# facebookresearch/sylph-few-shot-detection

Hardware: AMD Instinct MI355X
Metric: query images/sec, R50-FPN 5-way 5-shot 800x1333 (whole job) (higher is better)
Workload: dtype bf16

## Files before the change

### include/sylph_hip.h

```cpp
#ifndef SYLPH_HIP_H
#define SYLPH_HIP_H

#include <stdint.h>

#ifdef __cplusplus
extern "C" {
#endif

typedef struct sylph_ctx sylph_ctx;

enum { SYLPH_F32 = 0, SYLPH_BF16 = 1, SYLPH_F32S = 2 };

typedef struct sylph_config {
  int resnet_depth;
  int stride_in_1x1;
  int num_cls_convs;
  int num_box_convs;
  int nlevels;
  int strides[8];
  float pixel_mean[3];
  float pixel_std[3];
  int size_divisibility;
  int use_scale;
  int cond_use_bias;
  float pre_nms_thresh;
  int pre_nms_topk;
  float nms_thresh;
  int post_nms_topk;
  int thresh_with_ctr;
  int quality_mode;
  int cg_tower_layers;
  int cg_has_bias;
  int cg_bias_l2_norm;
  int cg_post_norm;
  int cg_conv_l2_norm;
  int cg_use_weight_scale;
  float prior_prob;
  int cand_cap;
  int cg_type;
  int tok_num_conv;
  int tok_num_fc;
  int enc_layers;
  int head_num_fc;
  int head_fc_dim;
  int cg_meta_bias;
  int cg_has_weight;
  int cg_has_scale;
  int num_share_convs;
  int tower_norm;
  int cg_tower_gn_mask;
  int cg_tower_relu_mask;
  int tower_deformable;
  int num_groups;
  int width_per_group;
  int cg_code_ksize;
} sylph_config;

void sylph_config_default(sylph_config* cfg);

int sylph_ctx_create(int device_id, int dtype, sylph_ctx** out);
void sylph_ctx_destroy(sylph_ctx* ctx);
const char* sylph_last_error(void);
int sylph_set_stream(sylph_ctx* ctx, void* hip_stream);
int sylph_set_config(sylph_ctx* ctx, const sylph_config* cfg);

int sylph_load_weight(sylph_ctx* ctx, const char* name, const float* data_host, const int64_t* shape, int ndim);
int sylph_finalize_weights(sylph_ctx* ctx);

int sylph_preprocess(sylph_ctx* ctx, int B, const float* const* images_dev, const int* heights, const int* widths,
                     int* padded_h, int* padded_w);

int sylph_preprocess_u8(sylph_ctx* ctx, int B, const unsigned char* const* images_dev, const int* heights, const int* widths,
                        const int* new_heights, const int* new_widths, int rgb_input, int* padded_h, int* padded_w);
int sylph_export_input(sylph_ctx* ctx, float* out_nchw_dev);

int sylph_backbone_fpn(sylph_ctx* ctx);

int sylph_import_pyramid(sylph_ctx* ctx, int B, int padded_h, int padded_w, const int* heights, const int* widths,
                         const float* const* levels_nchw_dev);
int sylph_export_pyramid(sylph_ctx* ctx, int level, float* out_nchw_dev);

int sylph_fcos_head(sylph_ctx* ctx, const float* cls_conv_dev, const float* cls_bias_dev, int N);
int sylph_fcos_head_episodes(sylph_ctx* ctx, int E, const float* cls_conv_dev, const float* cls_bias_dev, const int* n_classes,
                             const int* image_episode);
int sylph_fcos_head_codesets(sylph_ctx* ctx, int G, const float* cls_conv_dev, const float* cls_bias_dev, const int* n_classes);
int sylph_fcos_head_pretrained(sylph_ctx* ctx, int* num_classes);
int sylph_export_head(sylph_ctx* ctx, int level, float* logits_nchw_dev, float* reg_nchw_dev, float* ctr_nchw_dev,
                      float* iou_nchw_dev);

int sylph_import_head(sylph_ctx* ctx, int N, int level, const float* logits_nchw_dev, const float* reg_nchw_dev,
                      const float* ctr_nchw_dev, const float* iou_nchw_dev);

int sylph_decode_nms(sylph_ctx* ctx, const int* out_heights, const int* out_widths, int max_out, float* boxes_dev,
                     float* scores_dev, int* classes_dev, int* levels_dev, float* locations_dev, int* cand_dev,
                     int* counts_dev, int* status_dev);
int sylph_decode_nms_codesets(sylph_ctx* ctx, int G, const int* out_heights, const int* out_widths, int max_out, float* boxes_dev,
                              float* scores_dev, int* classes_dev, int* levels_dev, float* locations_dev, int* cand_dev,
                              int* counts_dev, int* status_dev);

int sylph_codegen(sylph_ctx* ctx, const float* boxes_dev, float* code_out_dev);
int sylph_codegen_classes(sylph_ctx* ctx, const float* boxes_dev, int shots, float* codes_out_dev);
int sylph_codegen_rois(sylph_ctx* ctx, int R, const float* boxes_dev, const int* roi_image, int n_seg, const int* seg_len,
                       float* codes_out_dev);
int sylph_roi_table_uploads(sylph_ctx* ctx, int64_t* n_out);
int sylph_codegen_weight_norm(sylph_ctx* ctx, float* weight_norm_out_dev);

int sylph_roi_align(sylph_ctx* ctx, const float* boxes_dev, float* out_nchw_dev);
int sylph_roi_align_rois(sylph_ctx* ctx, int R, const float* boxes_dev, const int* roi_image, float* out_nchw_dev);

int sylph_normalize_codes(sylph_ctx* ctx, float* codes_dev, int n, const float* weight_norm_dev);

int sylph_reduce_codes(sylph_ctx* ctx, const float* rows_dev, int n, int row_ld, float* out_dev, int num_classes,
                       int divide_by_acc);

int sylph_allgather_codes(sylph_ctx* ctx, void* comm, const float* local_dev, int n_local, int capacity, float* out_dev);
int sylph_comm_unique_id(char* id_out_128);
int sylph_comm_init_rank(sylph_ctx* ctx, const char* id_128, int nranks, int rank, void** comm_out);
int sylph_comm_destroy(void* comm);

int sylph_conv2d(sylph_ctx* ctx, const float* x_nchw_dev, int B, int C, int H, int W, const float* w_host, int Cout,
                 int KH, int KW, int stride, int pad, const float* scale_host, const float* shift_host, int relu,
                 const float* residual_nchw_dev, float* y_nchw_dev);
int sylph_group_norm(sylph_ctx* ctx, const float* x_nchw_dev, int B, int H, int W, const float* gamma_host,
                     const float* beta_host, int relu, float* y_nchw_dev);

int sylph_stem_maxpool(sylph_ctx* ctx, const float* x_nchw_dev, int B, int H, int W, const float* w_host,
                       const float* scale_host, const float* shift_host, float* stem_out_nchw_dev, float* pool_out_nchw_dev);

int sylph_set_debug_taps(sylph_ctx* ctx, int on);
int sylph_export_stage(sylph_ctx* ctx, int stage, float* out_nchw_dev);
int sylph_export_tower(sylph_ctx* ctx, int tower, int layer, int level, float* y_nchw_dev, float* coef_dev);

#define SYLPH_SUP_ROI 0
#define SYLPH_SUP_GN_Y 1
#define SYLPH_SUP_GN_COEF 2
#define SYLPH_SUP_LAYER_OUT 3
#define SYLPH_SUP_CONV_OUT 4
#define SYLPH_SUP_CONTEXT 5
#define SYLPH_SUP_MSCAM 6
#define SYLPH_SUP_TOKENS 7
#define SYLPH_SUP_CLS_TOKENS 8
int sylph_support_tap_numel(sylph_ctx* ctx, int stage, int index, int64_t* numel);
int sylph_export_support(sylph_ctx* ctx, int stage, int index, float* out_dev);

int sylph_bottleneck(sylph_ctx* ctx, const float* x_nchw_dev, int B, int Cin, int H, int W, int stride, int mid, int cout,
                     const float* const* w_host, const float* const* scale_host, const float* const* shift_host,
                     float* y_nchw_dev);
int sylph_bottleneck_even(sylph_ctx* ctx, const float* x_nchw_dev, int B, int Cin, int H, int W, int mid, int cout,
                          const float* const* w_host, const float* const* scale_host, const float* const* shift_host,
                          float* y_nchw_dev);

int sylph_fpn_lateral(sylph_ctx* ctx, const float* x_nchw_dev, int B, int C, int H, int W, const float* w_host, const float* bias_host,
                      const float* top_nchw_dev, float* y_nchw_dev);

int sylph_group_conv(sylph_ctx* ctx, const float* x_nchw_dev, int B, int C, int H, int W, int groups, int stride, const float* w_host,
                     const float* scale_host, const float* shift_host, int relu, float* y_nchw_dev);
int sylph_conv3x3_c64(sylph_ctx* ctx, const float* x_nchw_dev, int B, int H, int W, const float* w_host, const float* scale_host,
                      const float* shift_host, int relu, const float* residual_nchw_dev, float* y_nchw_dev);
int sylph_basic_block(sylph_ctx* ctx, const float* x_nchw_dev, int B, int Cin, int H, int W, int stride, int cout,
                      const float* const* w_host, const float* const* scale_host, const float* const* shift_host, float* y_nchw_dev);
int sylph_bottleneck_grouped(sylph_ctx* ctx, const float* x_nchw_dev, int B, int Cin, int H, int W, int stride, int mid, int cout,
                             int groups, const float* const* w_host, const float* const* scale_host, const float* const* shift_host,
                             float* y_nchw_dev);

int64_t sylph_device_bytes(sylph_ctx* ctx);

int sylph_profile_enable(sylph_ctx* ctx, int on);
int sylph_bench_conv(sylph_ctx* ctx, int B, int H, int W, int Cin, int Cout, int K, int stride, int pad, int has_res,
                     int relu, int with_gn, int iters, float* ms_out, double* flops_out);
int sylph_profile_read(sylph_ctx* ctx, double* conv_ms, double* conv_flops, int64_t* conv_launches);
int sylph_profile_read_kernels(sylph_ctx* ctx, int max_kernels, char* names_out, double* ms_out, double* flops_out,
                               int64_t* launches_out, int* n_out);
int sylph_conv_routes_read(sylph_ctx* ctx, int max_routes, char* names_out, int* n_out);

#ifdef __cplusplus
}
#endif
#endif
```

### sylph-few-shot-detection_amd/csrc/api_backbone.hip

```cpp
#include "api_internal.h"

namespace sylph_host {

std::shared_ptr<PilCoeffs> pil_bilinear_coeffs(int in_size, int out_size) {
  auto pc = std::make_shared<PilCoeffs>();
  const double scale = (double)in_size / (double)out_size;
  double filterscale = scale;
  if (filterscale < 1.0) filterscale = 1.0;
  const double support = 1.0 * filterscale;
  const int ksize = (int)ceil(support) * 2 + 1;
  pc->ksize = ksize;
  pc->bounds.assign((size_t)out_size * 2, 0);
  pc->kk.assign((size_t)out_size * ksize, 0);
  std::vector<double> k((size_t)ksize);
  for (int xx = 0; xx < out_size; ++xx) {
    const double center = (xx + 0.5) * scale;
    const double ss = 1.0 / filterscale;
    int xmin = (int)(center - support + 0.5);
    if (xmin < 0) xmin = 0;
    int xmax = (int)(center + support + 0.5);
    if (xmax > in_size) xmax = in_size;
    xmax -= xmin;
    double ww = 0.0;
    for (int x = 0; x < xmax; ++x) {
      double a = (x + xmin - center + 0.5) * ss;
      if (a < 0.0) a = -a;
      const double w = a < 1.0 ? 1.0 - a : 0.0;
      k[x] = w;
      ww += w;
    }
    for (int x = 0; x < xmax; ++x) {
      if (ww != 0.0) k[x] /= ww;
      pc->kk[(size_t)xx * ksize + x] = k[x] < 0 ? (int)(-0.5 + k[x] * (double)(1 << 22)) : (int)(0.5 + k[x] * (double)(1 << 22));
    }
    pc->bounds[2 * xx] = xmin;
    pc->bounds[2 * xx + 1] = xmax;
  }
  return pc;
}

int ensure_pyramid(sylph_ctx* c, Plan* P) {
  if (!P->F) RET(c->dalloc(&P->F, (size_t)P->B * P->Ltot * 256 * c->esz()));
  return 0;
}

template <typename Args>
static int add_patch_kernel(sylph_ctx* c, std::vector<OpFn>& ops, const char* kern, double flops, int (*launch)(const Args&, hipStream_t), Args a,
                            int B, int H, int W, int ph, int pw, int even_rp = 0) {
  std::vector<BkTile> bt;
  for (int b = 0; b < B; ++b) {
    if (even_rp) {
      for (int yy = 0; yy < H / 2; yy += ph)
        for (int xx = 0; xx < W / 2; xx += pw)
          bt.push_back(BkTile{b * H * W, H, W, (yy << 16) | xx, ph | (even_rp << 16), pw, (65536u + pw - 1) / pw, (65536u + 2 * pw) / (2 * pw + 1)});
      continue;
    }
    for (int yy = 0; yy < H; yy += ph)
      for (int xx = 0; xx < W; xx += pw)
        bt.push_back(BkTile{b * H * W, H, W, (yy << 16) | xx, ph, pw, (65536u + pw - 1) / pw, (65536u + pw + 2 - 1) / (pw + 2)});
  }
  void* btd = nullptr;
  RET(upload(c, &btd, bt.data(), bt.size() * sizeof(BkTile)));
  a.bk = (const BkTile*)btd;
  a.n_tiles = (int)bt.size();
  ops.push_back([=](hipStream_t s) { return timed_op(c, kern, flops, s, [=](hipStream_t st) { return launch(a, st); }); });
  return 0;
}

static const long RW64_MIN_PATCHES = 2048;

Conv3Route pick_conv3_route(const sylph_ctx* c, const ConvLayer& L, int B, int H, int W, int stride) {
  Conv3Route r;
  if (c->dt != DT_BF16 || L.groups != 1 || L.KH != 3 || L.KW != 3 || stride != 1 || !L.scale || !L.shift) return r;
  const size_t pos = (size_t)B * H * W;
  int ph = 0, pw = 0;
  if (const int on = knob::conv_rw3(); on && L.Cin == 128 && L.Cout == 128 && L.Cout_pad == 128 &&
      pos * 256 < ((size_t)1 << 31) &&
      (on == 2 || pos >= (size_t)256 * 120)) {
    pick_patch(H, W, 128, 184, 2, &ph, &pw);
    if (conv_rw3_patch_ok(ph, pw)) { r.kind = Conv3Kind::rw3; r.ph = ph; r.pw = pw; }
    return r;
  }
  if (const int on = knob::conv_rw64(); on && L.Cin == 64 && L.Cout == 64 && L.Cout_pad == 64 && W < 65536 &&
      pos * 128 <= 0xff000000u) {
    pick_patch(H, W, 256, 352, 2, &ph, &pw);
    const long n = (long)B * ((H + ph - 1) / ph) * ((W + pw - 1) / pw);
    if (conv_rw64_patch_ok(ph, pw) && (on == 2 || n >= RW64_MIN_PATCHES)) { r.kind = Conv3Kind::rw64; r.ph = ph; r.pw = pw; }
  }
  return r;
}

static int add_conv3x3(sylph_ctx* c, std::vector<OpFn>& ops, const ConvLayer& L, const Conv3Route& r, int B, int H, int W, int stride, const void* x,
                       const void* res, void* y, int relu) {
  switch (r.kind) {
    case Conv3Kind::rw3: {
      if (res || !relu) return fail("internal: conv_rw3 is conv + FrozenBN + ReLU");
      BottleneckArgs ba;
      memset(&ba, 0, sizeof(ba));
      ba.x = x; ba.y = y;
      ba.w2 = (const __bf16*)L.w; ba.s2 = L.scale; ba.b2 = L.shift;
      return add_patch_kernel(c, ops, "conv_rw3_kernel", 2.0 * (double)B * H * W * 128.0 * 1152.0, launch_conv_rw3, ba, B, H, W, r.ph, r.pw);
    }
    case Conv3Kind::rw64: {
      ConvRw64Args ra;
      memset(&ra, 0, sizeof(ra));
      ra.x = x; ra.y = y; ra.res = res; ra.w = (const __bf16*)L.w; ra.scale = L.scale; ra.shift = L.shift;
      ra.bytes = (unsigned)((size_t)B * H * W * 128); ra.relu = relu ? 1 : 0;
      return add_patch_kernel(c, ops, "conv_rw64_kernel", 2.0 * (double)B * H * W * 64.0 * 576.0, launch_conv_rw64, ra, B, H, W, r.ph, r.pw);
    }
    case Conv3Kind::generic: break;
  }
  const int Ho = (H - 1) / stride + 1, Wo = (W - 1) / stride + 1;
  ConvOpts o; o.stride = stride; o.pad = 1; o.relu_nch = relu ? (1 << 30) : 0;
  if (res) { o.res = res; o.res_ld = L.Cout; o.res_mode = 1; }
  return add_conv(c, ops, L, x, L.Cin, y, L.Cout, image_segs(B, H, W, Ho, Wo), o);
}

int add_conv3x3_c64(sylph_ctx* c, std::vector<OpFn>& ops, const ConvLayer& L, int B, int H, int W, const void* x, const void* res, void* y, int relu) {
  return add_conv3x3(c, ops, L, pick_conv3_route(c, L, B, H, W, 1), B, H, W, 1, x, res, y, relu);
}

BlockRoute pick_block_route(const sylph_ctx* c, const sylph_ctx::Block& blk, int B, int Cin, int Hin, int Win, int stride, int mid, int cout, int flags) {
  BlockRoute r;
  r.chunk = B;
  r.s1 = c->cfg.stride_in_1x1 ? stride : 1; r.s3 = c->cfg.stride_in_1x1 ? 1 : stride;
  r.H1 = (Hin - 1) / r.s1 + 1; r.W1 = (Win - 1) / r.s1 + 1;
  r.Ho = (Hin - 1) / stride + 1; r.Wo = (Win - 1) / stride + 1;
  const bool dense2 = blk.c2.groups == 1;
  const bool fused64 = knob::fuse_bottleneck() && dense2 && c->dt == DT_BF16 && stride == 1 && mid == 64 && cout == 256 && blk.c1.Cout_pad == 64 &&
                       blk.c2.Cout_pad == 64 && (size_t)Hin * Win * 512 < ((size_t)1 << 32) && (size_t)B * Hin * Win < ((size_t)1 << 31);
  const bool fuse_id = fused64 && !blk.has_sc && Cin == 256 && blk.c3.Cout_pad == 256;
  const bool fuse_pr = fused64 && blk.fused_sc && Cin == 64 && blk.c3sc.Cout_pad == 256 && blk.c3sc.Cin == 128 && !blk.c3sc.scale;
  r.tail_ok = fuse_id && (Hin & 1) == 0 && (Win & 1) == 0;
  if ((flags & BK_EVEN_OUT) && !r.tail_ok) {
    r.refuse = "the stride-2-output bottleneck is the fused bf16 identity block (C 256, mid 64) on a map of even height and width";
    return r;
  }
  if (!dense2) {
    const long per_img = std::max({(long)Hin * Win * Cin, (long)r.H1 * r.W1 * mid, (long)r.Ho * r.Wo * mid, (long)r.Ho * r.Wo * cout});
    const int nb = (int)std::min<long>(B, ((1L << 31) - 1) / per_img);
    if (nb < 1) {
      r.refuse = "image too large for the ResNeXt block kernels: " + std::to_string(per_img) + " elements per image";
      return r;
    }
    if (nb < B) {
      const int nch = (B + nb - 1) / nb;
      r.chunk = (B + nch - 1) / nch;
      return r;
    }
  }
  if (fuse_id || fuse_pr) {
    r.form = fuse_pr ? BlockForm::fused_proj : (flags & BK_EVEN_OUT) ? BlockForm::fused_id_even : BlockForm::fused_id;
    return r;
  }
  r.form = BlockForm::chain;
  r.fused_sc = blk.fused_sc;
  if (!dense2) {
    const int cpg = mid / blk.c2.groups;
    r.conv2 = Conv2Form::grouped;
    if (blk.c2.Cin != mid || blk.c2.Cout != mid || mid % 64 != 0 || cpg < 4 || cpg > 64 || (cpg & (cpg - 1)) != 0)
      r.refuse = "internal: grouped conv2 shape";
    else if ((long)r.H1 * r.W1 * mid >= (1L << 31))
      r.refuse = "image too large for conv_group: " + std::to_string((long)r.H1 * r.W1 * mid) + " elements per image exceed its 31-bit offsets";
    return r;
  }
  const Conv3Route r2 = pick_conv3_route(c, blk.c2, B, r.H1, r.W1, r.s3);
  if (r2.kind == Conv3Kind::rw3) { r.conv2 = Conv2Form::rw3; r.ph = r2.ph; r.pw = r2.pw; }
  return r;
}

int add_bottleneck(sylph_ctx* c, std::vector<OpFn>& ops, const sylph_ctx::Block& blk, int B, const void* X, int Cin, int Hin, int Win,
                          int stride, int mid, int cout, void* Y, const BkScratch& scr, int flags) {
  const BlockRoute r = pick_block_route(c, blk, B, Cin, Hin, Win, stride, mid, cout, flags);
  if (!r.refuse.empty()) return fail(r.refuse);
  const DType dt = c->dt;
  const int H1 = r.H1, W1 = r.W1, Ho = r.Ho, Wo = r.Wo;
  void *t1 = scr.t1, *t2 = scr.t2, *sc = scr.sc;
  if (r.chunk < B) {
    const size_t e = c->esz();
    for (int b0 = 0; b0 < B; b0 += r.chunk) {
      const int n = std::min(r.chunk, B - b0);
      BkScratch sub{(char*)t1 + (size_t)b0 * H1 * W1 * mid * e, (char*)t2 + (size_t)b0 * Ho * Wo * mid * e,
                    (char*)sc + (size_t)b0 * Ho * Wo * cout * e, scr.trash};
      RET(add_bottleneck(c, ops, blk, n, (const char*)X + (size_t)b0 * Hin * Win * Cin * e, Cin, Hin, Win, stride, mid, cout,
                         (char*)Y + (size_t)b0 * Ho * Wo * cout * e, sub, flags));
    }
    return 0;
  }
  if (r.form != BlockForm::chain) {
    const bool id = r.form != BlockForm::fused_proj;
    BottleneckArgs ba;
    memset(&ba, 0, sizeof(ba));
    ba.x = X; ba.y = Y;
    ba.w1 = (const __bf16*)blk.c1.w; ba.w2 = (const __bf16*)blk.c2.w; ba.w3 = (const __bf16*)(id ? blk.c3.w : blk.c3sc.w);
    ba.s1 = blk.c1.scale; ba.b1 = blk.c1.shift; ba.s2 = blk.c2.scale; ba.b2 = blk.c2.shift;
    ba.s3 = id ? blk.c3.scale : nullptr; ba.b3 = id ? blk.c3.shift : blk.c3sc.shift;
    ba.zeros = c->zeros;
    if (!*scr.trash) RET(c->dalloc(scr.trash, (size_t)1024 * 256 * 128));
    ba.trash = *scr.trash;
    int ph, pw;
    if (r.form == BlockForm::fused_id_even) {
      int rp;
      bottleneck64_even_patch(Hin, Win, &ph, &pw, &rp);
      const double fl = 2.0 * (double)B * ((double)Hin * Win * 256.0 * 64 + (double)(Hin / 2) * (Win / 2) * (64.0 * 576 + 64.0 * 256));
      return add_patch_kernel(c, ops, "bottleneck64_kernel", fl, launch_bottleneck64_even, ba, B, Hin, Win, ph, pw, rp);
    }
    pick_patch(Hin, Win, 128, 184, 2, &ph, &pw);
    const double fl = 2.0 * (double)B * Hin * Win * (id ? (256.0 * 64 + 64.0 * 576 + 64.0 * 256) : (64.0 * 64 + 64.0 * 576 + 128.0 * 256));
    if (id) return add_patch_kernel(c, ops, "bottleneck64_kernel", fl, launch_bottleneck64, ba, B, Hin, Win, ph, pw);
    return add_patch_kernel(c, ops, "bottleneck64p_kernel", fl, launch_bottleneck64p, ba, B, Hin, Win, ph, pw);
  }
  const int route_stride = (flags & BK_IN_COMPACT) ? 2 : 0;
  ConvOpts o1; o1.stride = r.s1; o1.relu_nch = 1 << 30; o1.route_stride = route_stride;
  RET(add_conv(c, ops, blk.c1, X, Cin, t1, mid, image_segs(B, Hin, Win, H1, W1), o1));
  switch (r.conv2) {
    case Conv2Form::grouped: {
      GroupConvArgs ga;
      memset(&ga, 0, sizeof(ga));
      ga.x = t1; ga.y = t2; ga.wt = blk.c2.w; ga.scale = blk.c2.scale; ga.shift = blk.c2.shift;
      ga.B = B; ga.C = mid; ga.cpg = mid / blk.c2.groups; ga.Hin = H1; ga.Win = W1; ga.Ho = Ho; ga.Wo = Wo; ga.stride = r.s3; ga.relu = 1;
      const double fl = 2.0 * (double)B * Ho * Wo * mid * 9.0 * ga.cpg;
      ops.push_back([=](hipStream_t s) { return timed_op(c, "conv_group_kernel", fl, s, [=](hipStream_t st) { return launch_conv_group(dt, ga, st); }); });
      break;
    }
    case Conv2Form::rw3:
      RET(add_conv3x3(c, ops, blk.c2, Conv3Route{Conv3Kind::rw3, r.ph, r.pw}, B, H1, W1, r.s3, t1, nullptr, t2, 1));
      break;
    case Conv2Form::generic:
      RET(add_conv3x3(c, ops, blk.c2, Conv3Route{}, B, H1, W1, r.s3, t1, nullptr, t2, 1));
      break;
  }
  if (r.fused_sc) {
    std::vector<SegDesc> sg = image_segs(B, Ho, Wo, Ho, Wo);
    for (int b = 0; b < B; ++b) { sg[b].in2_row0 = b * Hin * Win; sg[b].in2_W = Win; }
    ConvOpts o3; o3.relu_nch = 1 << 30; o3.in2 = X; o3.in2_ld = Cin; o3.Cin2 = Cin; o3.stride2 = stride;
    RET(add_conv(c, ops, blk.c3sc, t2, mid, Y, cout, sg, o3));
  } else {
    const void* resid = X;
    if (blk.has_sc) {
      ConvOpts os; os.stride = stride; os.route_stride = route_stride;
      RET(add_conv(c, ops, blk.sc, X, Cin, sc, cout, image_segs(B, Hin, Win, Ho, Wo), os));
      resid = sc;
    }
    ConvOpts o3; o3.relu_nch = 1 << 30; o3.res = resid; o3.res_ld = cout; o3.res_mode = 1;
    RET(add_conv(c, ops, blk.c3, t2, mid, Y, cout, image_segs(B, Ho, Wo, Ho, Wo), o3));
  }
  return 0;
}

int add_basic_block(sylph_ctx* c, std::vector<OpFn>& ops, const sylph_ctx::Block& blk, int B, const void* X, int Cin, int Hin, int Win,
                    int stride, int cout, void* Y, const BkScratch& scr) {
  const int Ho = (Hin - 1) / stride + 1, Wo = (Win - 1) / stride + 1;
  void *t = scr.t1, *sc = scr.sc;
  if (!blk.has_sc && (Cin != cout || stride != 1)) return fail("internal: BasicBlock without a shortcut must keep its shape");
  if (blk.c1.Cin != Cin || blk.c1.Cout != cout || blk.c2.Cin != cout || blk.c2.Cout != cout || blk.c1.KH != 3 || blk.c2.KH != 3)
    return fail("internal: BasicBlock shape");
  RET(add_conv3x3(c, ops, blk.c1, pick_conv3_route(c, blk.c1, B, Hin, Win, stride), B, Hin, Win, stride, X, nullptr, t, 1));
  const void* resid = X;
  if (blk.has_sc) {
    ConvOpts os; os.stride = stride;
    RET(add_conv(c, ops, blk.sc, X, Cin, sc, cout, image_segs(B, Hin, Win, Ho, Wo), os));
    resid = sc;
  }
  const bool c64 = Cin == 64 && cout == 64 && stride == 1;
  return add_conv3x3(c, ops, blk.c2, c64 ? pick_conv3_route(c, blk.c2, B, Ho, Wo, 1) : Conv3Route{}, B, Ho, Wo, 1, t, resid, Y, 1);
}

StemRoute pick_stem_route(const sylph_ctx* c) {
  if (c->dt != DT_BF16 || !c->stem_wp || !knob::stem_kernel()) return StemRoute::igemm;
  return knob::fuse_stem_pool() ? StemRoute::fused_pool : StemRoute::stem_conv;
}

int build_backbone(sylph_ctx* c, Plan* P) {
  if (P->backbone_built) return 0;
  if (!c->has_backbone) return fail("backbone weights were not loaded");
  const int B = P->B, H = P->H, W = P->W;
  const size_t e = c->esz();
  RET(ensure_pyramid(c, P));
  RET(c->dalloc(&P->x0, (size_t)B * H * W * 4 * e));
  const int H2 = (H - 1) / 2 + 1, W2 = (W - 1) / 2 + 1;
  const int H4 = (H2 - 1) / 2 + 1, W4 = (W2 - 1) / 2 + 1;
  RET(c->dalloc(&P->stem_out, (size_t)B * H2 * W2 * 64 * e));
  RET(c->dalloc(&P->pool_out, (size_t)B * H4 * W4 * 64 * e));
  RET(c->dalloc((void**)&P->img_desc_dev, sizeof(ImageDesc) * B));
  HIPCHK(hipHostMalloc((void**)&P->img_desc_host, sizeof(ImageDesc) * B));
  auto& ops = P->backbone_ops;
  const DType dt = c->dt;
  {
    void *so = P->stem_out, *po = P->pool_out;
    ConvOpts os; os.stem = 1; os.relu_nch = 1 << 30;
    os.flops = 2.0 * (double)B * H2 * W2 * 64.0 * 147.0;
    const void *x0 = P->x0, *wp = c->stem_wp;
    const float *scl = c->stem.scale, *shf = c->stem.shift;
    const double fl = os.flops;
    switch (pick_stem_route(c)) {
      case StemRoute::fused_pool: {
        void* trash = nullptr;
        RET(c->dalloc(&trash, (size_t)512 * 256 * 16));
        const Plan* PP = P;
        ops.push_back([=](hipStream_t s) {
          return timed_op(c, "stem_pool_kernel", fl, s, [=](hipStream_t st) {
            if (PP->raw_input)
              return launch_stem_pool_raw(PP->img_desc_dev, c->cfg.pixel_mean, c->cfg.pixel_std, wp, scl, shf, po, trash, B, H, W, H2, W2, H4, W4, st);
            return launch_stem_pool(x0, wp, scl, shf, po, trash, B, H, W, H2, W2, H4, W4, st);
          });
        });
        P->stem_takes_raw = B <= STEM_RAW_MAX_BATCH;
        break;
      }
      case StemRoute::stem_conv:
        ops.push_back([=](hipStream_t s) {
          return timed_op(c, "stem_conv_kernel", fl, s, [=](hipStream_t st) { return launch_stem_conv(x0, wp, scl, shf, so, B, H, W, H2, W2, st); });
        });
        ops.push_back([=](hipStream_t s) { return launch_maxpool(dt, so, po, B, H2, W2, 64, H4, W4, s); });
        break;
      case StemRoute::igemm:
        RET(add_conv(c, ops, c->stem, P->x0, 4, so, 64, image_segs(B, H, W, H2, W2), os));
        ops.push_back([=](hipStream_t s) { return launch_maxpool(dt, so, po, B, H2, W2, 64, H4, W4, s); });
        break;
    }
  }
  const void* X = P->pool_out;
  int Hin = H4, Win = W4, Cin = 64;
  const void* stage_out[4] = {nullptr, nullptr, nullptr, nullptr};
  int stage_h[4], stage_w[4];
  const bool basic = !c->stages[0].empty() && c->stages[0][0].basic;
  int stage_c[4];
  bool in_compact = false;
  for (int si = 0; si < 4; ++si) {
    const int mid = (c->cfg.num_groups * c->cfg.width_per_group) << si, cout = (basic ? 64 : 256) << si;
    const int first_stride = si == 0 ? 1 : in_compact ? 1 : 2;
    const int Hs = (Hin - 1) / first_stride + 1, Ws = (Win - 1) / first_stride + 1;
    void *t1, *t2 = nullptr, *sc, *Ya, *Yb;
    RET(c->dalloc(&t1, basic ? (size_t)B * Hs * Ws * cout * e : (size_t)B * Hin * Win * mid * e));
    if (!basic) RET(c->dalloc(&t2, (size_t)B * Hs * Ws * mid * e));
    RET(c->dalloc(&sc, (size_t)B * Hs * Ws * cout * e));
    RET(c->dalloc(&Ya, (size_t)B * Hs * Ws * cout * e));
    RET(c->dalloc(&Yb, (size_t)B * Hs * Ws * cout * e));
    auto& blocks = c->stages[si];
    void* Y = nullptr;
    BkScratch scr{t1, t2, sc, &P->bk_trash};
    for (size_t bi = 0; bi < blocks.size(); ++bi) {
      const int stride = bi == 0 ? first_stride : 1;
      Y = (Y == Ya) ? Yb : Ya;
      const bool fpn_input = si >= 1;
      const bool even_tail = knob::bk_strided_tail() && !basic && bi > 0 && bi + 1 == blocks.size() && !fpn_input && si + 1 < 4 && c->cfg.stride_in_1x1 &&
                             !c->stages[si + 1].empty() && !c->stages[si + 1][0].basic &&
                             pick_block_route(c, blocks[bi], B, Cin, Hin, Win, stride, mid, cout, 0).tail_ok;
      if (basic) RET(add_basic_block(c, ops, blocks[bi], B, X, Cin, Hin, Win, stride, cout, Y, scr));
      else RET(add_bottleneck(c, ops, blocks[bi], B, X, Cin, Hin, Win, stride, mid, cout, Y, scr,
                              even_tail ? BK_EVEN_OUT : (bi == 0 && in_compact) ? BK_IN_COMPACT : 0));
      if (bi == 0) in_compact = false;
      if (even_tail) {
        P->tail_even = true; P->tail_x = X;
        P->stage_h[si] = Hin; P->stage_w[si] = Win; P->stage_c[si] = cout;
        in_compact = true;
        X = Y; Hin /= 2; Win /= 2; Cin = cout;
        continue;
      }
      X = Y; Hin = (Hin - 1) / stride + 1; Win = (Win - 1) / stride + 1; Cin = cout;
    }
    stage_out[si] = X; stage_h[si] = Hin; stage_w[si] = Win; stage_c[si] = cout;
    if (in_compact) continue;
    P->stage_out[si] = X; P->stage_h[si] = Hin; P->stage_w[si] = Win; P->stage_c[si] = cout;
  }
  const int fpn_two_on = knob::head_streams();
  const bool fpn_two = fpn_two_on == 2 || (fpn_two_on == 1 && (size_t)B * P->Ltot <= (size_t)32 * 22400);
  if (fpn_two) RET(ensure_side_stream(c));
  std::vector<OpFn> side_ops;
  void* lat[3] = {nullptr, nullptr, nullptr};
  for (int k = 2; k >= 0; --k) {
    const int si = k + 1, h = stage_h[si], w = stage_w[si], cin = stage_c[si];
    if (h != P->hl[k] || w != P->wl[k]) return fail("internal: level geometry mismatch");
    RET(c->dalloc(&lat[k], (size_t)B * h * w * 256 * e));
    ConvOpts ol;
    std::vector<SegDesc> segs = image_segs(B, h, w, h, w);
    if (k < 2) {
      ol.res = lat[k + 1]; ol.res_ld = 256; ol.res_mode = 2;
      segs = image_segs(B, h, w, h, w, stage_h[si + 1], stage_w[si + 1]);
      if (h != 2 * stage_h[si + 1] || w != 2 * stage_w[si + 1]) return fail("FPN needs exact 2x level sizes");
    }
    RET(add_conv(c, ops, c->fpn_lat[k], stage_out[si], cin, lat[k], 256, segs, ol));
    if (k == 2 && fpn_two) ops.push_back(side_fork_op(c));
    std::vector<SegDesc> so = image_segs(B, h, w, h, w);
    for (int b = 0; b < B; ++b) so[b].out_row0 = b * P->Ltot + P->off[k];
    ConvOpts oo; oo.pad = 1; oo.stream_slot = (k == 2 && fpn_two) ? 1 : 0;
    RET(add_conv(c, (k == 2 && fpn_two) ? side_ops : ops, c->fpn_out[k], lat[k], 256, P->F, 256, so, oo));
  }
  std::vector<OpFn>& top_ops = fpn_two ? side_ops : ops;
  for (int k = 3; k < c->cfg.nlevels && k < 5; ++k) {
    std::vector<SegDesc> sg = image_segs(B, P->hl[k - 1], P->wl[k - 1], P->hl[k], P->wl[k]);
    for (int b = 0; b < B; ++b) {
      sg[b].in_row0 = b * P->Ltot + P->off[k - 1];
      sg[b].out_row0 = b * P->Ltot + P->off[k];
    }
    ConvOpts op; op.stride = 2; op.pad = 1; op.stream_slot = fpn_two ? 1 : 0;
    const void* src = P->F;
    if (k == 4) {
      const int n6 = P->hl[3] * P->wl[3];
      void* p6r;
      RET(c->dalloc(&p6r, (size_t)B * n6 * 256 * e));
      std::vector<CopySeg> cs;
      for (int b = 0; b < B; ++b) {
        cs.push_back(CopySeg{b * P->Ltot + P->off[3], b * n6, n6});
        sg[b].in_row0 = b * n6;
      }
      CopySeg* csd;
      RET(upload(c, (void**)&csd, cs.data(), cs.size() * sizeof(CopySeg)));
      const void* F = P->F;
      top_ops.push_back([=](hipStream_t s) { return launch_relu_rows(dt, F, p6r, 256, csd, B, n6, s); });
      src = p6r;
    }
    RET(add_conv(c, top_ops, k == 3 ? c->p6 : c->p7, src, 256, P->F, 256, sg, op));
  }
  if (fpn_two) {
    for (const OpFn& op : side_ops) ops.push_back(on_side_stream(c, op));
    ops.push_back(side_join_op(c));
  }
  P->backbone_built = true;
  return 0;
}

}

extern "C" {

int sylph_preprocess(sylph_ctx* c, int B, const float* const* images, const int* hs, const int* ws, int* ph, int* pw) {
  if (!c->finalized) return fail("weights not finalized");
  if (B <= 0) return fail("empty batch");
  HIPCHK(hipSetDevice(c->device));
  int mh = 0, mw = 0;
  for (int b = 0; b < B; ++b) { mh = hs[b] > mh ? hs[b] : mh; mw = ws[b] > mw ? ws[b] : mw; }
  const int d = c->cfg.size_divisibility;
  if (d > 1) { mh = (mh + d - 1) / d * d; mw = (mw + d - 1) / d * d; }
  Plan* P = get_plan(c, B, mh, mw);
  OwnerScope own(c, P);
  BUILD(build_backbone(c, P), P);
  std::vector<ImageDesc> tab((size_t)B);
  for (int b = 0; b < B; ++b) {
    tab[b].ptr = images[b]; tab[b].h = hs[b]; tab[b].w = ws[b];
    P->img_h[b] = hs[b]; P->img_w[b] = ws[b];
  }
  if (!P->img_desc_ev || P->img_desc_kind != 1 || P->img_desc_last.size() != tab.size() ||
      memcmp(P->img_desc_last.data(), tab.data(), tab.size() * sizeof(ImageDesc)) != 0) {
    if (P->img_desc_ev) HIPCHK(hipEventSynchronize(P->img_desc_ev));
    else HIPCHK(hipEventCreateWithFlags(&P->img_desc_ev, hipEventDisableTiming));
    memcpy(P->img_desc_host, tab.data(), tab.size() * sizeof(ImageDesc));
    HIPCHK(hipMemcpyAsync(P->img_desc_dev, P->img_desc_host, sizeof(ImageDesc) * B, hipMemcpyHostToDevice, c->stream));
    HIPCHK(hipEventRecord(P->img_desc_ev, c->stream));
    P->img_desc_last = tab;
    P->img_desc_kind = 1;
  }
  P->raw_input = knob::fuse_preprocess() && P->stem_takes_raw;
  if (!P->raw_input)
    KCHK(launch_preprocess(c->dt, P->img_desc_dev, P->x0, B, mh, mw, c->cfg.pixel_mean, c->cfg.pixel_std, c->stream),
         "preprocess");
  c->cur = P;
  if (ph) *ph = mh;
  if (pw) *pw = mw;
  return 0;
}

int sylph_preprocess_u8(sylph_ctx* c, int B, const unsigned char* const* images, const int* hs, const int* ws, const int* nhs,
                        const int* nws, int rgb_input, int* ph, int* pw) {
  if (!c->finalized) return fail("weights not finalized");
  if (B <= 0) return fail("empty batch");
  HIPCHK(hipSetDevice(c->device));
  int mh = 0, mw = 0;
  for (int b = 0; b < B; ++b) {
    if (hs[b] <= 0 || ws[b] <= 0 || nhs[b] <= 0 || nws[b] <= 0) return fail("sylph_preprocess_u8: bad image size");
    mh = nhs[b] > mh ? nhs[b] : mh; mw = nws[b] > mw ? nws[b] : mw;
  }
  const int d = c->cfg.size_divisibility;
  if (d > 1) { mh = (mh + d - 1) / d * d; mw = (mw + d - 1) / d * d; }
  Plan* P = get_plan(c, B, mh, mw);
  OwnerScope own(c, P);
  BUILD(build_backbone(c, P), P);
  std::vector<std::shared_ptr<PilCoeffs>> hc((size_t)B), vc((size_t)B);
  size_t nint = 0;
  for (int b = 0; b < B; ++b) {
    for (int pass = 0; pass < 2; ++pass) {
      const std::pair<int, int> key = pass == 0 ? std::make_pair(ws[b], nws[b]) : std::make_pair(hs[b], nhs[b]);
      auto it = c->pil_cache.find(key);
      if (it == c->pil_cache.end()) {
        if (c->pil_cache.size() > 256) c->pil_cache.clear();
        it = c->pil_cache.emplace(key, pil_bilinear_coeffs(key.first, key.second)).first;
      }
      (pass == 0 ? hc : vc)[b] = it->second;
      nint += it->second->bounds.size() + it->second->kk.size();
    }
  }
  if (P->img_desc_ev) HIPCHK(hipEventSynchronize(P->img_desc_ev));
  else HIPCHK(hipEventCreateWithFlags(&P->img_desc_ev, hipEventDisableTiming));
  const size_t need = sizeof(ResizeDesc) * B + nint * sizeof(int);
  if (need > P->rz_tab_cap) {
    if (P->rz_host) (void)hipHostFree(P->rz_host);
    if (P->rz_desc_dev) c->dfree(P->rz_desc_dev);
    P->rz_host = nullptr; P->rz_desc_dev = nullptr; P->rz_tab_cap = 0;
    const size_t cap = need + need / 2;
    HIPCHK(hipHostMalloc((void**)&P->rz_host, cap));
    RET(c->dalloc((void**)&P->rz_desc_dev, cap));
    P->rz_tab_cap = cap;
  }
  ResizeDesc* dh = reinterpret_cast<ResizeDesc*>(P->rz_host);
  int* th = reinterpret_cast<int*>(P->rz_host + sizeof(ResizeDesc) * B);
  size_t off = 0;
  for (int b = 0; b < B; ++b) {
    ResizeDesc& r = dh[b];
    r.src = images[b]; r.h = hs[b]; r.w = ws[b]; r.new_h = nhs[b]; r.new_w = nws[b];
    r.ksh = hc[b]->ksize; r.ksv = vc[b]->ksize;
    r.hb_off = (int)off; memcpy(th + off, hc[b]->bounds.data(), hc[b]->bounds.size() * sizeof(int)); off += hc[b]->bounds.size();
    r.hk_off = (int)off; memcpy(th + off, hc[b]->kk.data(), hc[b]->kk.size() * sizeof(int)); off += hc[b]->kk.size();
    r.vb_off = (int)off; memcpy(th + off, vc[b]->bounds.data(), vc[b]->bounds.size() * sizeof(int)); off += vc[b]->bounds.size();
    r.vk_off = (int)off; memcpy(th + off, vc[b]->kk.data(), vc[b]->kk.size() * sizeof(int)); off += vc[b]->kk.size();
    P->img_h[b] = nhs[b]; P->img_w[b] = nws[b];
  }
  HIPCHK(hipMemcpyAsync(P->rz_desc_dev, P->rz_host, need, hipMemcpyHostToDevice, c->stream));
  HIPCHK(hipEventRecord(P->img_desc_ev, c->stream));
  const int* tab_dev = reinterpret_cast<const int*>(reinterpret_cast<const char*>(P->rz_desc_dev) + sizeof(ResizeDesc) * B);
  P->raw_input = false;
  KCHK(launch_resize_preprocess(c->dt, P->rz_desc_dev, tab_dev, P->x0, B, mh, mw, c->cfg.pixel_mean, c->cfg.pixel_std, rgb_input,
                                c->stream), "resize_preprocess");
  c->cur = P;
  if (ph) *ph = mh;
  if (pw) *pw = mw;
  return 0;
}

int sylph_export_input(sylph_ctx* c, float* out) {
  Plan* P = c->cur;
  if (!P || !P->x0) return fail("sylph_preprocess must be called first");
  if (P->raw_input)
    KCHK(launch_preprocess(c->dt, P->img_desc_dev, P->x0, P->B, P->H, P->W, c->cfg.pixel_mean, c->cfg.pixel_std, c->stream), "preprocess");
  KCHK(launch_export_input(c->dt, P->x0, out, P->B, P->H, P->W, c->stream), "export_input");
  return 0;
}

int sylph_backbone_fpn(sylph_ctx* c) {
  if (!c->cur || !c->cur->backbone_built) return fail("sylph_preprocess must be called first");
  return run_ops(c, c->cur->backbone_ops, "backbone_fpn");
}

int sylph_import_pyramid(sylph_ctx* c, int B, int H, int W, const int* hs, const int* ws, const float* const* levels) {
  if (!c->finalized) return fail("weights not finalized");
  HIPCHK(hipSetDevice(c->device));
  Plan* P = get_plan(c, B, H, W);
  OwnerScope own(c, P);
  BUILD(ensure_pyramid(c, P), P);
  for (int b = 0; b < B; ++b) { P->img_h[b] = hs ? hs[b] : H; P->img_w[b] = ws ? ws[b] : W; }
  for (int l = 0; l < c->cfg.nlevels; ++l) {
    const int hw = P->hl[l] * P->wl[l];
    for (int b = 0; b < B; ++b)
      KCHK(launch_import_nchw(c->dt, levels[l] + (size_t)b * 256 * hw, P->F, 256, hw, b * P->Ltot + P->off[l], 256,
                              c->stream),
           "import_pyramid");
  }
  c->cur = P;
  return 0;
}

int sylph_export_pyramid(sylph_ctx* c, int level, float* out) {
  Plan* P = c->cur;
  if (!P || !P->F) return fail("no current batch");
  if (level < 0 || level >= c->cfg.nlevels) return fail("bad level");
  const int hw = P->hl[level] * P->wl[level];
  for (int b = 0; b < P->B; ++b)
    KCHK(launch_export_nchw(c->dt, P->F, out + (size_t)b * 256 * hw, 256, hw, b * P->Ltot + P->off[level], 256,
                            c->stream),
         "export_pyramid");
  return 0;
}

}
```

### sylph-few-shot-detection_amd/csrc/api_internal.h

```cpp
#pragma once
#include <hip/hip_runtime.h>
#include <limits.h>
#include <math.h>
#include <stdio.h>
#include <stdlib.h>
#include <string.h>

#include <functional>
#include <map>
#include <memory>
#include <string>
#include <tuple>
#include <vector>

#include "../../include/sylph_hip.h"
#include "common.h"
#include "kernels.h"

using namespace sylph;
namespace sylph_host {
int fail(const std::string& m);
}
using sylph_host::fail;
hipStream_t sylph_internal_stream(sylph_ctx* c);
int sylph_internal_fail(const std::string& m);
int sylph_internal_code_ksize(sylph_ctx* c);
#define HIPCHK(x)                                                                                  \
  do {                                                                                             \
    hipError_t e_ = (x);                                                                           \
    if (e_ != hipSuccess) return fail(std::string(#x) + ": " + hipGetErrorString(e_));             \
  } while (0)
#define RET(x)                     \
  do {                             \
    int r_ = (x);                  \
    if (r_ != 0) return r_;        \
  } while (0)
#define BUILD(x, P)                                  \
  do {                                               \
    int r_ = (x);                                    \
    if (r_ != 0) { drop_plan(c, (P)); return r_; }   \
  } while (0)
#define KCHK(x, what)                                                                              \
  do {                                                                                             \
    int r_ = (x);                                                                                  \
    if (r_ != 0) return fail(std::string(what) + ": launch failed (" + std::to_string(r_) + ")");  \
  } while (0)

static inline uint16_t f2bf_host(float f) {
  uint32_t u;
  memcpy(&u, &f, 4);
  if ((u & 0x7fffffffu) > 0x7f800000u) return (uint16_t)((u >> 16) | 0x40);
  u += 0x7fffu + ((u >> 16) & 1u);
  return (uint16_t)(u >> 16);
}

namespace sylph_host {
long knob_env(const char* name, long dflt);
namespace knob {
#define SYLPH_KNOB_ONCE(fn, name, dflt) inline int fn() { static const int v = (int)knob_env(name, dflt); return v; }
#define SYLPH_KNOB_LIVE(fn, name, dflt) inline int fn() { return (int)knob_env(name, dflt); }
SYLPH_KNOB_ONCE(conv_hpipe, "SYLPH_CONV_HPIPE", 1)
SYLPH_KNOB_ONCE(conv_halo, "SYLPH_CONV_HALO", 1)
SYLPH_KNOB_ONCE(conv_pw, "SYLPH_CONV_PW", 1)
SYLPH_KNOB_ONCE(conv_spw, "SYLPH_CONV_SPW", 1)
SYLPH_KNOB_ONCE(conv_nbuf2, "SYLPH_CONV_NBUF2", 1)
SYLPH_KNOB_ONCE(conv_nbuf3_max, "SYLPH_CONV_NBUF3_MAX", 400)
SYLPH_KNOB_ONCE(split_k, "SYLPH_SPLIT_K", 1)
SYLPH_KNOB_ONCE(split_t1, "SYLPH_SPLIT_T1", 64)
SYLPH_KNOB_ONCE(split_t2, "SYLPH_SPLIT_T2", 64)
SYLPH_KNOB_ONCE(conv_rw3, "SYLPH_CONV_RW3", 1)
SYLPH_KNOB_LIVE(conv_rw64, "SYLPH_CONV_RW64", 1)
SYLPH_KNOB_ONCE(fuse_bottleneck, "SYLPH_FUSE_BOTTLENECK", 1)
SYLPH_KNOB_ONCE(bk_strided_tail, "SYLPH_BK_STRIDED_TAIL", 1)
SYLPH_KNOB_ONCE(stem_kernel, "SYLPH_STEM_KERNEL", 1)
SYLPH_KNOB_ONCE(fuse_stem_pool, "SYLPH_FUSE_STEM_POOL", 1)
SYLPH_KNOB_ONCE(head_streams, "SYLPH_HEAD_STREAMS", 1)
SYLPH_KNOB_ONCE(gn_fuse, "SYLPH_GN_FUSE", 1)
SYLPH_KNOB_ONCE(fuse_gn_logits, "SYLPH_FUSE_GN_LOGITS", 1)
SYLPH_KNOB_LIVE(gn_cond3x3, "SYLPH_GN_COND3X3", 0)
SYLPH_KNOB_ONCE(fuse_scan, "SYLPH_FUSE_SCAN", 1)
SYLPH_KNOB_LIVE(fuse_preprocess, "SYLPH_FUSE_PREPROCESS", 1)
SYLPH_KNOB_LIVE(fuse_shortcut, "SYLPH_FUSE_SHORTCUT", 1)
SYLPH_KNOB_LIVE(max_plans, "SYLPH_MAX_PLANS", 32)
inline long plan_bytes_mb() { return knob_env("SYLPH_PLAN_BYTES_MB", LONG_MIN); }
#undef SYLPH_KNOB_ONCE
#undef SYLPH_KNOB_LIVE
}
}

typedef std::function<int(hipStream_t)> OpFn;

struct HostTensor {
  std::vector<float> data;
  std::vector<int64_t> shape;
};

struct ConvLayer {
  void* w = nullptr;
  float* scale = nullptr;
  float* shift = nullptr;
  int Cin = 0, Cout = 0, Cout_pad = 0, KH = 1, KW = 1;
  int groups = 1;
};
struct GNLayer {
  float* gamma = nullptr;
  float* beta = nullptr;
};

struct Plan;

struct PilCoeffs {
  int ksize = 0;
  std::vector<int> bounds;
  std::vector<int> kk;
};


struct sylph_ctx {
  int device = 0;
  DType dt = DT_BF16;
  hipStream_t stream = nullptr;
  sylph_config cfg;
  bool finalized = false;
  int64_t bytes = 0;
  std::vector<void*> allocs;
  std::map<std::string, HostTensor> host_w;
  ConvLayer stem;
  void* stem_wp = nullptr;
  struct Block {
    ConvLayer c1, c2, c3, sc, c3sc;
    bool has_sc = false, fused_sc = false;
    bool basic = false;
  };
  std::vector<std::vector<Block>> stages;
  ConvLayer fpn_lat[3], fpn_out[3], p6, p7;
  std::vector<ConvLayer> cls_tower, box_tower, share_tower;
  std::vector<GNLayer> share_gn;
  std::vector<GNLayer> cls_gn, box_gn;
  ConvLayer cls_off, box_off;
  ConvLayer pred;
  ConvLayer cls_logits;
  bool has_cls_logits = false;
  void* pred_taps = nullptr;
  std::vector<float> level_scales;
  std::vector<ConvLayer> cg_tower;
  std::vector<GNLayer> cg_gn;
  ConvLayer cg_cls, cg_bias;
  int cg_naux = 0, cg_ib = -1, cg_iw = -1, cg_is = -1;
  GNLayer cg_post;
  float cg_conv_scale = 1.f, cg_bias_scale = 1.f;
  float cg_bias_prior = 0.f;
  struct Lin { float* W = nullptr; float* b = nullptr; int K = 0, O = 0; };
  struct EncLayer { Lin attn, l1, l2; GNLayer n1, n2; };
  struct RoiEnc {
    ConvLayer pool_conv; GNLayer pool_gn;
    MsCamWeights cam;
    std::vector<ConvLayer> tok_conv; std::vector<GNLayer> tok_gn;
    std::vector<Lin> tok_fc, wh, bh;
    std::vector<EncLayer> layers;
  } re;
  bool has_backbone = false, has_head = false, has_codegen = false, has_roienc = false;
  std::map<std::tuple<int, int, int>, std::unique_ptr<Plan>> plans;
  std::map<std::pair<int, int>, std::shared_ptr<struct PilCoeffs>> pil_cache;
  std::map<const void*, void*> hp_weights;
  std::map<const void*, std::pair<void*, float*>> pw_weights;
  void* pw_trash = nullptr;
  Plan* cur = nullptr;
  void* zeros = nullptr;
  hipStream_t side_stream = nullptr;
  hipEvent_t ev_fork = nullptr, ev_join = nullptr;
  int build_slot = 0;
  bool prof = false;
  struct ProfRec { hipEvent_t a, b; double flops; const char* kern; };
  std::vector<ProfRec> prof_recs;
  std::vector<std::pair<hipEvent_t, hipEvent_t>> prof_free;
  std::vector<std::string> route_recs;

  Plan* alloc_owner = nullptr;
  int64_t roi_table_uploads = 0;
  bool debug_taps = false;
  uint64_t use_clock = 0;
  size_t max_plans = 32;
  int64_t plan_byte_budget = 0;
  int dalloc(void** p, size_t n);
  void dfree_nosync(void* p) {
    if (!p) return;
    for (size_t i = 0; i < allocs.size(); ++i)
      if (allocs[i] == p) { allocs[i] = allocs.back(); allocs.pop_back(); break; }
    auto it = alloc_bytes.find(p);
    if (it != alloc_bytes.end()) { bytes -= (int64_t)it->second; alloc_bytes.erase(it); }
    (void)hipFree(p);
  }
  std::map<void*, size_t> alloc_bytes;
  void dfree(void* p);
  size_t esz() const { return dt == DT_BF16 ? 2 : 4; }
};

struct SupportPass {
  int S = 0;
  bool built = false;
  std::vector<OpFn> ops;
  void *roi = nullptr, *cgA = nullptr, *cgB = nullptr;
  float *cg_conv_out = nullptr, *cg_bias_out = nullptr, *cg_wnorm = nullptr;
  float *re_ctx = nullptr, *re_tok = nullptr, *re_tmp = nullptr, *re_hid = nullptr, *re_cls = nullptr, *re_h = nullptr;
  struct SupTap {
    const void* p = nullptr;
    bool f32 = true;
    int n = 0, npos = 49, C = 256, ld = 256;
    const float2* stats = nullptr;
    const float *gamma = nullptr, *beta = nullptr;
  };
  std::map<std::pair<int, int>, SupTap> taps;
  const float* cur_boxes = nullptr;
  int n_seg = 0;
  float* cur_code_out = nullptr;
  std::vector<int> roi_image, seg_len;
  int max_len = 0;
  int* roi_image_dev = nullptr;
  int2* seg_dev = nullptr;
};

struct HeadOut {
  enum Src { none, cond, episodes, pretrained, imported, codesets } src = none;
  enum Cand { cand_none, cand_all, cand_scanned } cand = cand_none;
  bool has_bias = false;
  bool logits_missing = false;
  int ncls = 0, logits_ld = 0;
  int nsets = 0;
};

struct PackedCodes {
  void* w = nullptr;
  float* bias = nullptr;
  int* src_row = nullptr;
  int rows = 0, cap = 0;
};

struct DecodeSlots {
  DecodeBuffers buf{};
  int slots_cap = 0, cand_cap = 0;
};

struct Plan {
  std::vector<void*> allocs;
  int64_t bytes = 0;
  uint64_t last_use = 0;
  int B = 0, H = 0, W = 0;
  int hl[8], wl[8], off[8], Ltot = 0;
  std::vector<int> img_h, img_w;
  void *x0 = nullptr, *stem_out = nullptr, *pool_out = nullptr;
  void* F = nullptr;
  void* bk_trash = nullptr;
  float* splitk_scratch[2] = {nullptr, nullptr};
  size_t splitk_bytes[2] = {0, 0};
  const void* stage_out[4] = {nullptr, nullptr, nullptr, nullptr};
  bool tail_even = false;
  const void* tail_x = nullptr;
  void* tail_dense = nullptr;
  std::vector<OpFn> tail_dense_ops;
  int stage_h[4] = {0, 0, 0, 0}, stage_w[4] = {0, 0, 0, 0}, stage_c[4] = {0, 0, 0, 0};
  std::vector<const void*> tap_out[2];
  std::vector<const float2*> tap_coef[2];
  std::vector<OpFn> backbone_ops, head_ops;
  bool backbone_built = false, head_built = false;
  ImageDesc* img_desc_dev = nullptr;
  ImageDesc* img_desc_host = nullptr;
  std::vector<ImageDesc> img_desc_last;
  int img_desc_kind = 0;
  hipEvent_t img_desc_ev = nullptr;
  ResizeDesc* rz_desc_dev = nullptr;
  char* rz_host = nullptr;
  int* rz_tab_dev = nullptr;
  size_t rz_tab_cap = 0;
  void *tA = nullptr, *tB = nullptr, *tC = nullptr, *tD = nullptr;
  void* cls_feat = nullptr;
  const float2* cls_coef = nullptr;
  std::function<int(hipStream_t)> cls_apply;
  float* pred = nullptr;
  float* logits = nullptr;
  int logits_cap_ld = 0;
  HeadOut out;
  PackedCodes codes;
  void* code_wf = nullptr;
  int code_wf_cap = 0;
  PackedCodes codes3;
  std::map<std::pair<int, int>, std::vector<OpFn>> cond3_ops;
  const void* cond3_for[3] = {nullptr, nullptr, nullptr};
  const SegDesc* head_segs = nullptr;
  const int2 *head_tiles = nullptr, *head_tiles32 = nullptr;
  int head_mtiles = 0, head_BM = 128, head_mtiles32 = 0;
  RowSeg* head_rowsegs = nullptr;
  float* gn_partial = nullptr;
  float2* gn_stats = nullptr;
  DecodeSeg* dsegs = nullptr;
  DecodeSlots dec, dec_cs;
  bool cand_dirty = false;
  bool decode_built = false;
  std::vector<OpFn> cls_logits_ops;
  const float* cls_logits_dst = nullptr;
  int pool_cap = 0;
  bool stem_takes_raw = false;
  bool raw_input = false;
  struct Episodes {
    PackedCodes codes;
    std::vector<int> n, image;
    std::vector<int> row0;
    std::vector<int2> tiles32, tilesBM;
    int* seg_row0 = nullptr;
    int2* tiles_dev = nullptr;
    DecodeSeg* dsegs = nullptr;
  } ep;
  struct CodeSets {
    PackedCodes codes;
    std::vector<int> n, col0;
    int hot_blocks = 0, hot_width = 0, ld = 0;
    DecodeSeg* dsegs = nullptr;
    int dsegs_cap = 0;
  } cs;
  ImageOut* img_out_dev = nullptr;
  ImageOut* img_out_host = nullptr;
  std::vector<ImageOut> img_out_last;
  hipEvent_t img_out_ev = nullptr;
  LevelDesc* lv_dev = nullptr;
  std::map<int, std::unique_ptr<SupportPass>> sup;
  SupportPass* sup_last = nullptr;
};

struct OwnerScope {
  sylph_ctx* c; Plan* prev;
  OwnerScope(sylph_ctx* c_, Plan* P) : c(c_), prev(c_->alloc_owner) { c->alloc_owner = P; }
  ~OwnerScope() { c->alloc_owner = prev; }
};

struct Geom {
  const SegDesc* segs;
  const int2* tiles;
  int n_mtiles;
  std::vector<int2> seg_tiles;
  float* gn_partial = nullptr;
};

struct ConvOpts {
  int stride = 1, pad = 0;
  int relu_nch = 0, mul_nch = 0;
  const void* res = nullptr;
  int res_ld = 0, res_mode = 0;
  bool out_f32 = false;
  int cout_override = -1;
  int stem = 0;
  int want_gn = 0;
  const void* in2 = nullptr;
  int in2_ld = 0, Cin2 = 0, stride2 = 1;
  double flops = -1.0;
  const float2* gn_coef = nullptr;
  int gn_relu = 0;
  int segs_per_image = 1;
  int stream_slot = 0;
  int route_stride = 0;
};

enum class ConvKind { hpipe, igemm_halo, pw, spw, igemm_splitk, igemm };
struct ConvRoute {
  ConvKind kind = ConvKind::igemm;
  int BM = 0, BN = 0;
  int nbuf = 0;
  int ksplit = 1;
};

enum class Conv3Kind { rw3, rw64, generic };
struct Conv3Route {
  Conv3Kind kind = Conv3Kind::generic;
  int ph = 0, pw = 0;
};

enum class BlockForm { fused_id, fused_id_even, fused_proj, chain };
enum class Conv2Form { grouped, rw3, generic };
struct BlockRoute {
  std::string refuse;
  int chunk = 0;
  BlockForm form = BlockForm::chain;
  Conv2Form conv2 = Conv2Form::generic;
  int ph = 0, pw = 0;
  bool fused_sc = false;
  bool tail_ok = false;
  int s1 = 1, s3 = 1, H1 = 0, W1 = 0, Ho = 0, Wo = 0;
};

enum class StemRoute { fused_pool, stem_conv, igemm };

struct BkScratch { void *t1, *t2, *sc; void** trash; };
enum { BK_EVEN_OUT = 1, BK_IN_COMPACT = 2 };

namespace sylph_host {
std::shared_ptr<PilCoeffs> pil_bilinear_coeffs(int in_size, int out_size);
void free_plan(sylph_ctx* c, Plan* P);
int upload(sylph_ctx* c, void** dev, const void* host, size_t n);
void evict_plans(sylph_ctx* c, const Plan* keep);
void drop_plan(sylph_ctx* c, Plan* P);
Plan* get_plan(sylph_ctx* c, int B, int H, int W);
int run_ops(sylph_ctx* c, const std::vector<OpFn>& ops, const char* what);
int ensure_side_stream(sylph_ctx* c);
OpFn side_fork_op(sylph_ctx* c);
OpFn side_join_op(sylph_ctx* c);
OpFn on_side_stream(sylph_ctx* c, const OpFn& op);
const HostTensor* find_w(sylph_ctx* c, const std::string& k);
int pack_conv(sylph_ctx* c, const std::vector<const HostTensor*>& ws, ConvLayer* L);
int upload_vec(sylph_ctx* c, float** dev, const std::vector<float>& v, int pad_to);
int make_conv_bn(sylph_ctx* c, const std::string& name, ConvLayer* L);
int pack_conv_grouped(sylph_ctx* c, const HostTensor& w, const std::string& key, int C, int groups, const float* scale, const float* shift,
                      ConvLayer* L);
int make_conv_bias(sylph_ctx* c, const std::vector<std::string>& names, ConvLayer* L);
int make_c3sc(sylph_ctx* c, const HostTensor& w3, const float* s3, const float* h3, const HostTensor& ws, const float* ss, const float* hs, ConvLayer* L);
int make_gn(sylph_ctx* c, const std::string& name, GNLayer* G);
int upload_f32(sylph_ctx* c, const float** dev, const HostTensor* t, const std::string& what, size_t expect = 0);
int make_lin(sylph_ctx* c, const std::string& name, sylph_ctx::Lin* L);
int make_ln(sylph_ctx* c, const std::string& name, GNLayer* G);
bool has_prefix(sylph_ctx* c, const std::string& p);
void level_dims(const sylph_config& cfg, int H, int W, int* hl, int* wl, int* off, int* Ltot);
int make_geom(sylph_ctx* c, const std::vector<SegDesc>& segs, int BM, Geom* g);
void pick_patch(int H, int W, int max_pos, int halo_rows, int xpad, int* ph_out, int* pw_out);
void set_patch(SegDesc* s, int ph, int pw, int xpad);
int make_geom_patch(sylph_ctx* c, std::vector<SegDesc> segs, int max_pos, int halo_rows, int xpad, bool pair, Geom* g, int group = 1);
long patch_count(const std::vector<SegDesc>& segs, int max_pos, int halo_rows, int xpad);
int timed_op(sylph_ctx* c, const char* kern, double flops, hipStream_t s, const std::function<int(hipStream_t)>& fn);
ConvRoute pick_conv_route(const sylph_ctx* c, const ConvLayer& L, int in_ld, const std::vector<SegDesc>& segs, const ConvOpts& o);
std::string conv_route_name(const ConvRoute& r);
void adopt_records(sylph_ctx* c, sylph_ctx* tmp);
int add_conv(sylph_ctx* c, std::vector<OpFn>& ops, const ConvLayer& L, const void* in, int in_ld, void* out, int out_ld, const std::vector<SegDesc>& segs, const ConvOpts& o, Geom* geom_out = nullptr);
int add_conv_gn(sylph_ctx* c, std::vector<OpFn>& ops, const ConvLayer& L, const void* in, int in_ld, void* out, const std::vector<SegDesc>& segs, ConvOpts o, const GNLayer& G, int relu, const float2** coef_out = nullptr, OpFn* apply_out = nullptr);
int add_gn_from_partials(sylph_ctx* c, std::vector<OpFn>& ops, void* out, int ld, const std::vector<SegDesc>& segs, const Geom& g, const GNLayer& G, int relu,
                         const float2** coef_out, OpFn* apply_out, const float2** stats_out = nullptr);
int add_conv_deform(sylph_ctx* c, std::vector<OpFn>& ops, const ConvLayer& off, const ConvLayer& L, const void* in, void* out,
                    const std::vector<SegDesc>& segs, int segs_per_image, const GNLayer* G, int relu, const float2** coef_out = nullptr,
                    OpFn* apply_out = nullptr);
std::vector<SegDesc> image_segs(int B, int Hin, int Win, int Hout, int Wout, int resH = 0, int resW = 0);
int ensure_pyramid(sylph_ctx* c, Plan* P);
Conv3Route pick_conv3_route(const sylph_ctx* c, const ConvLayer& L, int B, int H, int W, int stride);
BlockRoute pick_block_route(const sylph_ctx* c, const sylph_ctx::Block& blk, int B, int Cin, int Hin, int Win, int stride, int mid, int cout, int flags);
StemRoute pick_stem_route(const sylph_ctx* c);
int add_bottleneck(sylph_ctx* c, std::vector<OpFn>& ops, const sylph_ctx::Block& blk, int B, const void* X, int Cin, int Hin, int Win, int stride, int mid, int cout, void* Y, const BkScratch& scr, int flags = 0);
int add_conv3x3_c64(sylph_ctx* c, std::vector<OpFn>& ops, const ConvLayer& L, int B, int H, int W, const void* x, const void* res, void* y, int relu);
int add_basic_block(sylph_ctx* c, std::vector<OpFn>& ops, const sylph_ctx::Block& blk, int B, const void* X, int Cin, int Hin, int Win, int stride, int cout, void* Y, const BkScratch& scr);
int build_backbone(sylph_ctx* c, Plan* P);
std::vector<SegDesc> pyramid_segs(sylph_ctx* c, Plan* P);
int add_gn(sylph_ctx* c, Plan* P, std::vector<OpFn>& ops, void* x, const RowSeg* segs_dev, int nseg, int max_rows, const GNLayer& G, int relu);
int ensure_gn_ws(sylph_ctx* c, Plan* P, int nseg, int max_rows);
int build_head(sylph_ctx* c, Plan* P);
int build_support(sylph_ctx* c, Plan* P, SupportPass* Q);
int build_support_roienc(sylph_ctx* c, Plan* P, SupportPass* Q);
}
using namespace sylph_host;
```

### sylph-few-shot-detection_amd/csrc/api_parity.hip

```cpp
#include "api_internal.h"

namespace {

int import_nchw(sylph_ctx* c, const float* src, void* dst, int B, int C, int hw, const char* what = "import") {
  for (int b = 0; b < B; ++b) KCHK(launch_import_nchw(c->dt, src + (size_t)b * C * hw, dst, C, hw, b * hw, C, c->stream), what);
  return 0;
}
int export_nchw(sylph_ctx* c, const void* src, float* dst, int B, int C, int hw, const char* what = "export") {
  for (int b = 0; b < B; ++b) KCHK(launch_export_nchw(c->dt, src, dst + (size_t)b * C * hw, C, hw, b * hw, C, c->stream), what);
  return 0;
}

enum class Records { to_caller, none };
struct Scratch : sylph_ctx {
  sylph_ctx* const caller;
  Scratch(sylph_ctx* c, Records rec) : caller(c) {
    device = c->device; dt = c->dt; stream = c->stream; zeros = c->zeros; cfg = c->cfg;
    if (rec == Records::to_caller) prof = c->prof;
  }
  Scratch(const Scratch&) = delete;
  ~Scratch() {
    (void)hipStreamSynchronize(stream);
    for (void* p : allocs) (void)hipFree(p);
  }
  void hand_records() { adopt_records(caller, this); }
};

}

extern "C" {

int sylph_conv2d(sylph_ctx* c, const float* x, int B, int C, int H, int W, const float* w_host, int Cout, int KH, int KW,
                 int stride, int pad, const float* scale_host, const float* shift_host, int relu, const float* residual,
                 float* y) {
  HIPCHK(hipSetDevice(c->device));
  const int bk = c->dt == DT_BF16 ? 64 : 32;
  if (C % bk != 0) return fail("sylph_conv2d: Cin must be a multiple of " + std::to_string(bk));
  const int Ho = (H + 2 * pad - KH) / stride + 1, Wo = (W + 2 * pad - KW) / stride + 1;
  Scratch tmp(c, Records::to_caller);
  HostTensor hw;
  hw.shape = {Cout, C, KH, KW};
  hw.data.assign(w_host, w_host + (size_t)Cout * C * KH * KW);
  ConvLayer L;
  RET(pack_conv(&tmp, {&hw}, &L));
  if (scale_host) RET(upload_vec(&tmp, &L.scale, std::vector<float>(scale_host, scale_host + Cout), L.Cout_pad));
  if (shift_host) RET(upload_vec(&tmp, &L.shift, std::vector<float>(shift_host, shift_host + Cout), L.Cout_pad));
  void *xin, *yout, *res = nullptr;
  RET(tmp.dalloc(&xin, (size_t)B * H * W * C * tmp.esz()));
  RET(tmp.dalloc(&yout, (size_t)B * Ho * Wo * Cout * tmp.esz()));
  RET(import_nchw(&tmp, x, xin, B, C, H * W));
  ConvOpts o; o.stride = stride; o.pad = pad; o.relu_nch = relu ? (1 << 30) : 0;
  if (residual) {
    RET(tmp.dalloc(&res, (size_t)B * Ho * Wo * Cout * tmp.esz()));
    RET(import_nchw(&tmp, residual, res, B, Cout, Ho * Wo));
    o.res = res; o.res_ld = Cout; o.res_mode = 1;
  }
  std::vector<OpFn> ops;
  RET(add_conv(&tmp, ops, L, xin, C, yout, Cout, image_segs(B, H, W, Ho, Wo), o));
  RET(run_ops(c, ops, "conv2d"));
  tmp.hand_records();
  return export_nchw(&tmp, yout, y, B, Cout, Ho * Wo);
}

int sylph_set_debug_taps(sylph_ctx* c, int on) {
  c->debug_taps = on != 0;
  return 0;
}

int sylph_export_stage(sylph_ctx* c, int stage, float* out) {
  Plan* P = c->cur;
  if (!P || !P->backbone_built) return fail("no backbone pass on the current batch");
  const bool on_demand = stage == 2 && P->tail_even;
  if (stage < 2 || stage > 5 || (!P->stage_out[stage - 2] && !on_demand)) return fail("bad stage");
  HIPCHK(hipSetDevice(c->device));
  const int si = stage - 2, C = P->stage_c[si], hw = P->stage_h[si] * P->stage_w[si];
  const void* src = P->stage_out[si];
  if (on_demand) {
    if (!P->tail_dense) {
      OwnerScope own(c, P);
      RET(c->dalloc(&P->tail_dense, (size_t)P->B * hw * C * c->esz()));
      BkScratch scr{nullptr, nullptr, nullptr, &P->bk_trash};
      const int rc = add_bottleneck(c, P->tail_dense_ops, c->stages[0].back(), P->B, P->tail_x, C, P->stage_h[si], P->stage_w[si], 1, 64, C, P->tail_dense, scr);
      if (rc != 0) { P->tail_dense_ops.clear(); return rc; }
    }
    RET(run_ops(c, P->tail_dense_ops, "res2 tap"));
    src = P->tail_dense;
  }
  return export_nchw(c, src, out, P->B, C, hw, "export stage");
}

int sylph_export_tower(sylph_ctx* c, int tower, int layer, int level, float* y, float* coef) {
  Plan* P = c->cur;
  if (!P || !P->head_built) return fail("no head pass on the current batch");
  if (tower < 0 || tower > 1 || layer < 0 || layer >= (int)P->tap_out[tower].size()) return fail("bad tower / layer");
  if (level < 0 || level >= c->cfg.nlevels) return fail("bad level");
  if (!c->debug_taps && layer + 1 != (int)P->tap_out[tower].size()) return fail("intermediate tower layers need sylph_set_debug_taps(1) before the first head call");
  HIPCHK(hipSetDevice(c->device));
  const int hw = P->hl[level] * P->wl[level], L = c->cfg.nlevels;
  for (int b = 0; b < P->B; ++b) {
    if (y) KCHK(launch_export_nchw(c->dt, P->tap_out[tower][layer], y + (size_t)b * 256 * hw, 256, hw, b * P->Ltot + P->off[level], 256, c->stream), "export tower");
    if (coef) {
      if (!P->tap_coef[tower][layer]) return fail("this layer's GroupNorm was applied in place (no coefficient table)");
      HIPCHK(hipMemcpyAsync(coef + (size_t)b * 512, P->tap_coef[tower][layer] + (size_t)(b * L + level) * 256, 512 * sizeof(float),
                            hipMemcpyDeviceToDevice, c->stream));
    }
  }
  return 0;
}

static int bottleneck_entry(sylph_ctx* c, const float* x, int B, int Cin, int H, int W, int stride, int mid, int cout, int groups,
                            const float* const* w_host, const float* const* scale_host, const float* const* shift_host, float* y, bool even_out = false) {
  HIPCHK(hipSetDevice(c->device));
  const int bk = c->dt == DT_BF16 ? 64 : 32;
  if (Cin % bk != 0 || mid % bk != 0) return fail("sylph_bottleneck: channel counts must be multiples of " + std::to_string(bk));
  const bool has_sc = w_host[3] != nullptr;
  if (!has_sc && (Cin != cout || stride != 1)) return fail("sylph_bottleneck: an identity block needs Cin == cout and stride 1");
  Scratch tmp(c, Records::to_caller);
  sylph_ctx::Block blk;
  const int cins[4] = {Cin, mid, mid, Cin}, couts[4] = {mid, mid, cout, cout}, ks[4] = {1, 3, 1, 1};
  ConvLayer* Ls[4] = {&blk.c1, &blk.c2, &blk.c3, &blk.sc};
  HostTensor hw[4];
  for (int i = 0; i < (has_sc ? 4 : 3); ++i) {
    const int cin_w = i == 1 ? cins[i] / groups : cins[i];
    hw[i].shape = {couts[i], cin_w, ks[i], ks[i]};
    hw[i].data.assign(w_host[i], w_host[i] + (size_t)couts[i] * cin_w * ks[i] * ks[i]);
    if (i == 1 && groups > 1) {
      RET(pack_conv_grouped(&tmp, hw[i], "conv2.weight", mid, groups, scale_host[i], shift_host[i], Ls[i]));
      continue;
    }
    RET(pack_conv(&tmp, {&hw[i]}, Ls[i]));
    RET(upload_vec(&tmp, &Ls[i]->scale, std::vector<float>(scale_host[i], scale_host[i] + couts[i]), Ls[i]->Cout_pad));
    RET(upload_vec(&tmp, &Ls[i]->shift, std::vector<float>(shift_host[i], shift_host[i] + couts[i]), Ls[i]->Cout_pad));
  }
  blk.has_sc = has_sc;
  if (has_sc && knob::fuse_shortcut()) {
    RET(make_c3sc(&tmp, hw[2], scale_host[2], shift_host[2], hw[3], scale_host[3], shift_host[3], &blk.c3sc));
    blk.fused_sc = true;
  }
  const size_t e = tmp.esz();
  const int Ho = even_out ? H / 2 : (H - 1) / stride + 1, Wo = even_out ? W / 2 : (W - 1) / stride + 1;
  void *xin, *yout, *t1, *t2, *sc, *trash = nullptr;
  RET(tmp.dalloc(&xin, (size_t)B * H * W * Cin * e));
  RET(tmp.dalloc(&yout, (size_t)B * Ho * Wo * cout * e));
  RET(tmp.dalloc(&t1, (size_t)B * H * W * mid * e));
  RET(tmp.dalloc(&t2, (size_t)B * Ho * Wo * mid * e));
  RET(tmp.dalloc(&sc, (size_t)B * Ho * Wo * cout * e));
  RET(import_nchw(&tmp, x, xin, B, Cin, H * W));
  std::vector<OpFn> ops;
  BkScratch scr{t1, t2, sc, &trash};
  RET(add_bottleneck(&tmp, ops, blk, B, xin, Cin, H, W, stride, mid, cout, yout, scr, even_out ? BK_EVEN_OUT : 0));
  RET(run_ops(c, ops, "bottleneck"));
  tmp.hand_records();
  return export_nchw(&tmp, yout, y, B, cout, Ho * Wo);
}

int sylph_bottleneck(sylph_ctx* c, const float* x, int B, int Cin, int H, int W, int stride, int mid, int cout, const float* const* w_host,
                     const float* const* scale_host, const float* const* shift_host, float* y) {
  return bottleneck_entry(c, x, B, Cin, H, W, stride, mid, cout, 1, w_host, scale_host, shift_host, y);
}

int sylph_bottleneck_even(sylph_ctx* c, const float* x, int B, int Cin, int H, int W, int mid, int cout, const float* const* w_host,
                          const float* const* scale_host, const float* const* shift_host, float* y) {
  if (B < 1 || H < 2 || W < 2 || (H & 1) || (W & 1)) return fail("sylph_bottleneck_even: H and W must be even");
  if (Cin != 256 || mid != 64 || cout != 256 || c->dt != DT_BF16) return fail("sylph_bottleneck_even: the fused identity block is C 256, mid 64, bf16");
  if (!w_host[0] || !w_host[1] || !w_host[2] || w_host[3]) return fail("sylph_bottleneck_even: an identity block has three convs and no shortcut");
  return bottleneck_entry(c, x, B, Cin, H, W, 1, mid, cout, 1, w_host, scale_host, shift_host, y, true);
}

int sylph_bottleneck_grouped(sylph_ctx* c, const float* x, int B, int Cin, int H, int W, int stride, int mid, int cout, int groups,
                             const float* const* w_host, const float* const* scale_host, const float* const* shift_host, float* y) {
  if (groups < 1 || mid % groups != 0) return fail("sylph_bottleneck_grouped: mid must be a multiple of groups");
  return bottleneck_entry(c, x, B, Cin, H, W, stride, mid, cout, groups, w_host, scale_host, shift_host, y);
}

int sylph_group_conv(sylph_ctx* c, const float* x, int B, int C, int H, int W, int groups, int stride, const float* w_host,
                     const float* scale_host, const float* shift_host, int relu, float* y) {
  HIPCHK(hipSetDevice(c->device));
  if (groups < 1 || C % groups != 0 || (stride != 1 && stride != 2) || B < 1) return fail("sylph_group_conv: bad arguments");
  Scratch tmp(c, Records::to_caller);
  HostTensor hw;
  hw.shape = {C, C / groups, 3, 3};
  hw.data.assign(w_host, w_host + (size_t)C * (C / groups) * 9);
  ConvLayer L;
  RET(pack_conv_grouped(&tmp, hw, "sylph_group_conv weight", C, groups, scale_host, shift_host, &L));
  const size_t e = tmp.esz();
  const int Ho = (H - 1) / stride + 1, Wo = (W - 1) / stride + 1;
  void *xin, *yout;
  RET(tmp.dalloc(&xin, (size_t)B * H * W * C * e));
  RET(tmp.dalloc(&yout, (size_t)B * Ho * Wo * C * e));
  RET(import_nchw(&tmp, x, xin, B, C, H * W));
  GroupConvArgs ga;
  memset(&ga, 0, sizeof(ga));
  ga.x = xin; ga.y = yout; ga.wt = L.w; ga.scale = L.scale; ga.shift = L.shift;
  ga.B = B; ga.C = C; ga.cpg = C / groups; ga.Hin = H; ga.Win = W; ga.Ho = Ho; ga.Wo = Wo; ga.stride = stride; ga.relu = relu ? 1 : 0;
  const double fl = 2.0 * (double)B * Ho * Wo * C * 9.0 * (C / groups);
  const DType dt = c->dt;
  KCHK(timed_op(&tmp, "conv_group_kernel", fl, c->stream, [=](hipStream_t st) { return launch_conv_group(dt, ga, st); }), "conv_group");
  tmp.hand_records();
  return export_nchw(&tmp, yout, y, B, C, Ho * Wo);
}

int sylph_conv3x3_c64(sylph_ctx* c, const float* x, int B, int H, int W, const float* w_host, const float* scale_host,
                      const float* shift_host, int relu, const float* residual, float* y) {
  HIPCHK(hipSetDevice(c->device));
  if (B < 1 || H < 1 || W < 1 || !w_host || !scale_host || !shift_host) return fail("sylph_conv3x3_c64: bad arguments");
  Scratch tmp(c, Records::to_caller);
  HostTensor hw;
  hw.shape = {64, 64, 3, 3};
  hw.data.assign(w_host, w_host + (size_t)64 * 64 * 9);
  ConvLayer L;
  RET(pack_conv(&tmp, {&hw}, &L));
  RET(upload_vec(&tmp, &L.scale, std::vector<float>(scale_host, scale_host + 64), L.Cout_pad));
  RET(upload_vec(&tmp, &L.shift, std::vector<float>(shift_host, shift_host + 64), L.Cout_pad));
  const size_t n = (size_t)B * H * W * 64 * tmp.esz();
  void *xin, *yout, *res = nullptr;
  RET(tmp.dalloc(&xin, n));
  RET(tmp.dalloc(&yout, n));
  if (residual) RET(tmp.dalloc(&res, n));
  RET(import_nchw(&tmp, x, xin, B, 64, H * W));
  if (residual) RET(import_nchw(&tmp, residual, res, B, 64, H * W));
  std::vector<OpFn> ops;
  RET(add_conv3x3_c64(&tmp, ops, L, B, H, W, xin, res, yout, relu));
  RET(run_ops(c, ops, "conv3x3_c64"));
  tmp.hand_records();
  return export_nchw(&tmp, yout, y, B, 64, H * W);
}

int sylph_basic_block(sylph_ctx* c, const float* x, int B, int Cin, int H, int W, int stride, int cout, const float* const* w_host,
                      const float* const* scale_host, const float* const* shift_host, float* y) {
  HIPCHK(hipSetDevice(c->device));
  const int bk = c->dt == DT_BF16 ? 64 : 32;
  if (Cin % bk != 0 || cout % bk != 0) return fail("sylph_basic_block: channel counts must be multiples of " + std::to_string(bk));
  if (stride != 1 && stride != 2) return fail("sylph_basic_block: stride must be 1 or 2");
  const bool has_sc = w_host[2] != nullptr;
  if (!has_sc && (Cin != cout || stride != 1)) return fail("sylph_basic_block: an identity block needs Cin == cout and stride 1");
  Scratch tmp(c, Records::to_caller);
  sylph_ctx::Block blk;
  blk.basic = true; blk.has_sc = has_sc;
  const int cins[3] = {Cin, cout, Cin}, ks[3] = {3, 3, 1};
  ConvLayer* Ls[3] = {&blk.c1, &blk.c2, &blk.sc};
  HostTensor hw[3];
  for (int i = 0; i < (has_sc ? 3 : 2); ++i) {
    hw[i].shape = {cout, cins[i], ks[i], ks[i]};
    hw[i].data.assign(w_host[i], w_host[i] + (size_t)cout * cins[i] * ks[i] * ks[i]);
    RET(pack_conv(&tmp, {&hw[i]}, Ls[i]));
    RET(upload_vec(&tmp, &Ls[i]->scale, std::vector<float>(scale_host[i], scale_host[i] + cout), Ls[i]->Cout_pad));
    RET(upload_vec(&tmp, &Ls[i]->shift, std::vector<float>(shift_host[i], shift_host[i] + cout), Ls[i]->Cout_pad));
  }
  const size_t e = tmp.esz();
  const int Ho = (H - 1) / stride + 1, Wo = (W - 1) / stride + 1;
  void *xin, *yout, *t1, *sc, *trash = nullptr;
  RET(tmp.dalloc(&xin, (size_t)B * H * W * Cin * e));
  RET(tmp.dalloc(&yout, (size_t)B * Ho * Wo * cout * e));
  RET(tmp.dalloc(&t1, (size_t)B * Ho * Wo * cout * e));
  RET(tmp.dalloc(&sc, (size_t)B * Ho * Wo * cout * e));
  RET(import_nchw(&tmp, x, xin, B, Cin, H * W));
  std::vector<OpFn> ops;
  BkScratch scr{t1, nullptr, sc, &trash};
  RET(add_basic_block(&tmp, ops, blk, B, xin, Cin, H, W, stride, cout, yout, scr));
  RET(run_ops(c, ops, "basic_block"));
  tmp.hand_records();
  return export_nchw(&tmp, yout, y, B, cout, Ho * Wo);
}

int sylph_fpn_lateral(sylph_ctx* c, const float* x, int B, int C, int H, int W, const float* w_host, const float* bias_host, const float* top,
                      float* y) {
  HIPCHK(hipSetDevice(c->device));
  const int bk = c->dt == DT_BF16 ? 64 : 32;
  if (C % bk != 0) return fail("sylph_fpn_lateral: Cin must be a multiple of " + std::to_string(bk));
  if (top && ((H & 1) || (W & 1))) return fail("sylph_fpn_lateral: the top-down input is half the size: H and W must be even");
  Scratch tmp(c, Records::to_caller);
  HostTensor hw;
  hw.shape = {256, C, 1, 1};
  hw.data.assign(w_host, w_host + (size_t)256 * C);
  ConvLayer L;
  RET(pack_conv(&tmp, {&hw}, &L));
  RET(upload_vec(&tmp, &L.shift, std::vector<float>(bias_host, bias_host + 256), L.Cout_pad));
  const size_t e = tmp.esz();
  void *xin, *yout, *tp = nullptr;
  RET(tmp.dalloc(&xin, (size_t)B * H * W * C * e));
  RET(tmp.dalloc(&yout, (size_t)B * H * W * 256 * e));
  RET(import_nchw(&tmp, x, xin, B, C, H * W));
  ConvOpts o;
  std::vector<SegDesc> segs = image_segs(B, H, W, H, W);
  if (top) {
    const int h2 = H / 2, w2 = W / 2;
    RET(tmp.dalloc(&tp, (size_t)B * h2 * w2 * 256 * e));
    RET(import_nchw(&tmp, top, tp, B, 256, h2 * w2));
    o.res = tp; o.res_ld = 256; o.res_mode = 2;
    segs = image_segs(B, H, W, H, W, h2, w2);
  }
  std::vector<OpFn> ops;
  RET(add_conv(&tmp, ops, L, xin, C, yout, 256, segs, o));
  RET(run_ops(c, ops, "fpn_lateral"));
  tmp.hand_records();
  return export_nchw(&tmp, yout, y, B, 256, H * W);
}

int sylph_group_norm(sylph_ctx* c, const float* x, int B, int H, int W, const float* gamma_host, const float* beta_host,
                     int relu, float* y) {
  HIPCHK(hipSetDevice(c->device));
  Scratch tmp(c, Records::none);
  const int HW = H * W;
  void* buf;
  RET(tmp.dalloc(&buf, (size_t)B * HW * 256 * tmp.esz()));
  RET(import_nchw(&tmp, x, buf, B, 256, HW));
  std::vector<RowSeg> rs;
  for (int b = 0; b < B; ++b) rs.push_back(RowSeg{b * HW, HW});
  RowSeg* rsd;
  RET(upload(&tmp, (void**)&rsd, rs.data(), rs.size() * sizeof(RowSeg)));
  float *ga, *be, *partial;
  float2* stats;
  RET(upload_vec(&tmp, &ga, std::vector<float>(gamma_host, gamma_host + 256), 256));
  RET(upload_vec(&tmp, &be, std::vector<float>(beta_host, beta_host + 256), 256));
  const int max_chunks = (HW + GN_ROWS_PER_CHUNK - 1) / GN_ROWS_PER_CHUNK;
  RET(tmp.dalloc((void**)&partial, (size_t)B * max_chunks * 32 * 3 * 4));
  RET(tmp.dalloc((void**)&stats, (size_t)B * 32 * sizeof(float2)));
  KCHK(launch_groupnorm(c->dt, buf, rsd, B, HW, 256, ga, be, 1e-5f, relu, partial, stats, c->stream), "group_norm");
  return export_nchw(&tmp, buf, y, B, 256, HW);
}

int sylph_stem_maxpool(sylph_ctx* c, const float* x, int B, int H, int W, const float* w_host, const float* scale_host,
                       const float* shift_host, float* stem_out, float* pool_out) {
  if (c->dt != DT_BF16) return fail("sylph_stem_maxpool: the dedicated stem kernels exist in bf16 mode only");
  HIPCHK(hipSetDevice(c->device));
  Scratch tmp(c, Records::none);
  const int H2 = (H - 1) / 2 + 1, W2 = (W - 1) / 2 + 1, H4 = (H2 - 1) / 2 + 1, W4 = (W2 - 1) / 2 + 1;
  std::vector<bf16_t> wp((size_t)64 * 224);
  for (int n = 0; n < 64; ++n)
    for (int kh = 0; kh < 7; ++kh)
      for (int px = 0; px < 8; ++px)
        for (int ch = 0; ch < 4; ++ch)
          wp[(size_t)n * 224 + kh * 32 + px * 4 + ch] = (bf16_t)((px < 7 && ch < 3) ? w_host[((n * 3 + ch) * 7 + kh) * 7 + px] : 0.f);
  void *wpd, *x0, *so, *po;
  float *scd, *shd;
  ImageDesc* idd;
  RET(upload(&tmp, &wpd, wp.data(), wp.size() * sizeof(bf16_t)));
  RET(upload_vec(&tmp, &scd, std::vector<float>(scale_host, scale_host + 64), 64));
  RET(upload_vec(&tmp, &shd, std::vector<float>(shift_host, shift_host + 64), 64));
  std::vector<ImageDesc> id((size_t)B);
  for (int b = 0; b < B; ++b) { id[b].ptr = x + (size_t)b * 3 * H * W; id[b].h = H; id[b].w = W; }
  RET(upload(&tmp, (void**)&idd, id.data(), id.size() * sizeof(ImageDesc)));
  RET(tmp.dalloc(&x0, (size_t)B * H * W * 4 * 2));
  RET(tmp.dalloc(&so, (size_t)B * H2 * W2 * 64 * 2));
  RET(tmp.dalloc(&po, (size_t)B * H4 * W4 * 64 * 2));
  const float mean0[3] = {0.f, 0.f, 0.f}, std1[3] = {1.f, 1.f, 1.f};
  KCHK(launch_preprocess(c->dt, idd, x0, B, H, W, mean0, std1, c->stream), "preprocess");
  KCHK(launch_stem_conv(x0, wpd, scd, shd, so, B, H, W, H2, W2, c->stream), "stem_conv");
  if (knob::fuse_stem_pool()) {
    void* trash;
    RET(tmp.dalloc(&trash, (size_t)512 * 256 * 16));
    KCHK(launch_stem_pool(x0, wpd, scd, shd, po, trash, B, H, W, H2, W2, H4, W4, c->stream), "stem_pool");
  } else {
    KCHK(launch_maxpool(c->dt, so, po, B, H2, W2, 64, H4, W4, c->stream), "maxpool");
  }
  if (stem_out) RET(export_nchw(&tmp, so, stem_out, B, 64, H2 * W2));
  if (pool_out) RET(export_nchw(&tmp, po, pool_out, B, 64, H4 * W4));
  return 0;
}

int sylph_bench_conv(sylph_ctx* c, int B, int H, int W, int Cin, int Cout, int K, int stride, int pad, int has_res,
                     int relu, int with_gn, int iters, float* ms_out, double* flops_out) {
  HIPCHK(hipSetDevice(c->device));
  const int bk = c->dt == DT_BF16 ? 64 : 32;
  if (Cin % bk != 0) return fail("sylph_bench_conv: Cin must be a multiple of " + std::to_string(bk));
  const int Ho = (H + 2 * pad - K) / stride + 1, Wo = (W + 2 * pad - K) / stride + 1;
  Scratch tmp(c, Records::none);
  HostTensor hw;
  hw.shape = {Cout, Cin, K, K};
  hw.data.resize((size_t)Cout * Cin * K * K);
  unsigned st = 12345u;
  const float wsc = 1.0f / sqrtf((float)(Cin * K * K));
  for (auto& v : hw.data) { st = st * 1664525u + 1013904223u; v = ((float)(st >> 8) * (2.0f / 16777216.0f) - 1.0f) * wsc; }
  ConvLayer L;
  RET(pack_conv(&tmp, {&hw}, &L));
  RET(upload_vec(&tmp, &L.scale, std::vector<float>((size_t)Cout, 1.0f), L.Cout_pad));
  RET(upload_vec(&tmp, &L.shift, std::vector<float>((size_t)Cout, 0.1f), L.Cout_pad));
  void *xin, *yout, *res = nullptr;
  const size_t nin = (size_t)B * H * W * Cin, nout = (size_t)B * Ho * Wo * Cout;
  RET(tmp.dalloc(&xin, nin * tmp.esz()));
  RET(tmp.dalloc(&yout, nout * tmp.esz()));
  KCHK(launch_fill_random(c->dt, xin, nin, 1u, c->stream), "fill");
  ConvOpts o; o.stride = stride; o.pad = pad; o.relu_nch = relu ? (1 << 30) : 0;
  if (has_res) {
    RET(tmp.dalloc(&res, nout * tmp.esz()));
    KCHK(launch_fill_random(c->dt, res, nout, 2u, c->stream), "fill");
    o.res = res; o.res_ld = Cout; o.res_mode = 1;
  }
  o.want_gn = with_gn & 1;
  if (with_gn & 2) {
    float2* coef;
    RET(tmp.dalloc((void**)&coef, (size_t)B * Cin * sizeof(float2)));
    KCHK(launch_fill_random(DT_F32, coef, (size_t)B * Cin * 2, 3u, c->stream), "fill");
    o.gn_coef = coef; o.gn_relu = 1;
  }
  std::vector<OpFn> ops;
  RET(add_conv(&tmp, ops, L, xin, Cin, yout, Cout, image_segs(B, H, W, Ho, Wo), o));
  for (int i = 0; i < 2; ++i) RET(run_ops(c, ops, "bench_conv"));
  hipEvent_t e0, e1;
  HIPCHK(hipEventCreate(&e0)); HIPCHK(hipEventCreate(&e1));
  HIPCHK(hipEventRecord(e0, c->stream));
  for (int i = 0; i < iters; ++i) RET(run_ops(c, ops, "bench_conv"));
  HIPCHK(hipEventRecord(e1, c->stream));
  HIPCHK(hipEventSynchronize(e1));
  float ms = 0.f;
  HIPCHK(hipEventElapsedTime(&ms, e0, e1));
  (void)hipEventDestroy(e0); (void)hipEventDestroy(e1);
  if (ms_out) *ms_out = ms / (float)iters;
  if (flops_out) *flops_out = 2.0 * (double)B * Ho * Wo * Cout * K * K * Cin;
  return 0;
}

}
```

### sylph-few-shot-detection_amd/csrc/common.h

```cpp
#pragma once
#include <hip/hip_runtime.h>
#include <stdint.h>

#include <atomic>

namespace sylph {

typedef __bf16 bf16_t;
typedef __attribute__((ext_vector_type(8))) __bf16 bf16x8;
typedef __attribute__((ext_vector_type(16))) float f32x16;
typedef __attribute__((ext_vector_type(4))) float f32x4;

enum DType { DT_F32 = 0, DT_BF16 = 1, DT_F32S = 2 };

struct SegDesc {
  int in_row0, in_H, in_W;
  int out_row0, out_H, out_W;
  int res_row0, res_H, res_W;
  float mul;
  int in2_row0, in2_W;
  int ph, pw;
  int hpitch;
  unsigned inv_pw, inv_hw2;
};

struct ConvArgs {
  const void* in;
  const void* wt;
  void* out;
  const void* res;
  const float* scale;
  const float* shift;
  const void* in2;
  const void* zeros;
  const SegDesc* segs;
  const int2* tiles;
  int n_mtiles, n_ntiles;
  int Cin, Cout, KH, KW, stride, pad;
  int in_ld, out_ld, res_ld;
  int Cin2, in2_ld, stride2;
  int relu_nch;
  int mul_nch;
  int res_mode;
  float* gn_partial;
  int halo;
  int ss_padded_host;
  int ss_padded;
  int stem;
  int tap_dy;
  const float2* gn_coef;
  int gn_relu;
  void* trash;
  const struct PwDesc* pw_desc;
  const float* pw_table;
  int pw_rot_mask;
  int ksplit;
  long long split_stride;
  int nbuf2;
};

struct SplitSeg { int src_row0, dst_row0, res_row0, nrows; };

struct PwDesc { int row0, seg_rows, out_W, out_row0, in_row0, in_W, in2_row0, in2_W, res_row0, res_W, pad[6]; };

struct BkTile { int row0, H, W, yx, ph, pw; unsigned inv_pw, inv_hw2; };
struct BottleneckArgs {
  const void* x;
  void* y;
  const __bf16 *w1, *w2, *w3;
  const float *s1, *b1, *s2, *b2, *s3, *b3;
  const void* zeros;
  void* trash;
  const BkTile* bk;
  int n_tiles;
};

struct ConvRw64Args {
  const void* x;
  void* y;
  const void* res;
  const __bf16* w;
  const float *scale, *shift;
  const BkTile* bk;
  int n_tiles;
  unsigned bytes;
  int relu;
};

template <typename T> struct Cvt;
template <> struct Cvt<float> {
  static __device__ __forceinline__ float to_f(float v) { return v; }
  static __device__ __forceinline__ float from_f(float v) { return v; }
};
template <> struct Cvt<bf16_t> {
  static __device__ __forceinline__ float to_f(bf16_t v) { return (float)v; }
  static __device__ __forceinline__ bf16_t from_f(float v) { return (bf16_t)v; }
};

__device__ __forceinline__ float bf16_bits_to_f(uint32_t hi16) { return __uint_as_float(hi16 << 16); }

template <typename T> __device__ __forceinline__ void load8(const T* p, float (&v)[8]);
template <> __device__ __forceinline__ void load8<float>(const float* p, float (&v)[8]) {
  const float4 a = *reinterpret_cast<const float4*>(p);
  const float4 b = *reinterpret_cast<const float4*>(p + 4);
  v[0] = a.x; v[1] = a.y; v[2] = a.z; v[3] = a.w; v[4] = b.x; v[5] = b.y; v[6] = b.z; v[7] = b.w;
}
template <> __device__ __forceinline__ void load8<bf16_t>(const bf16_t* p, float (&v)[8]) {
  const uint4 a = *reinterpret_cast<const uint4*>(p);
  v[0] = __uint_as_float(a.x << 16); v[1] = __uint_as_float(a.x & 0xffff0000u);
  v[2] = __uint_as_float(a.y << 16); v[3] = __uint_as_float(a.y & 0xffff0000u);
  v[4] = __uint_as_float(a.z << 16); v[5] = __uint_as_float(a.z & 0xffff0000u);
  v[6] = __uint_as_float(a.w << 16); v[7] = __uint_as_float(a.w & 0xffff0000u);
}
template <typename T> __device__ __forceinline__ void store8(T* p, const float (&v)[8]);
template <> __device__ __forceinline__ void store8<float>(float* p, const float (&v)[8]) {
  *reinterpret_cast<float4*>(p) = make_float4(v[0], v[1], v[2], v[3]);
  *reinterpret_cast<float4*>(p + 4) = make_float4(v[4], v[5], v[6], v[7]);
}
template <> __device__ __forceinline__ void store8<bf16_t>(bf16_t* p, const float (&v)[8]) {
  bf16x8 o;
#pragma unroll
  for (int i = 0; i < 8; ++i) o[i] = (bf16_t)v[i];
  *reinterpret_cast<bf16x8*>(p) = o;
}

inline int current_device() {
  int dev = 0;
  return (hipGetDevice(&dev) == hipSuccess && dev >= 0 && dev < 64) ? dev : 0;
}
inline int device_cu_count(int dev) {
  static std::atomic<int> cus[64];
  int n = cus[dev].load(std::memory_order_relaxed);
  if (n == 0) {
    hipDeviceProp_t p;
    n = (hipGetDeviceProperties(&p, dev) == hipSuccess && p.multiProcessorCount > 0) ? p.multiProcessorCount : 256;
    cus[dev].store(n, std::memory_order_relaxed);
  }
  return n;
}
struct PerDeviceOnce {
  std::atomic<unsigned long long> done{0};
  template <typename F> bool run(int dev, F&& f) {
    const unsigned long long bit = 1ull << dev;
    if (done.load(std::memory_order_acquire) & bit) return true;
    if (!f()) return false;
    done.fetch_or(bit, std::memory_order_release);
    return true;
  }
};

int launch_conv(DType dt, bool out_f32, const ConvArgs& a, int BM, int BN, hipStream_t s);
void conv_pick_tile(int rows_total, int cout, int ntaps, int* BM, int* BN);
int launch_splitk_finish(const float* partial, int ksplit, size_t plane, int ld, int Cout, const SplitSeg* segs_dev, int nseg, int max_rows,
                         const float* scale, const float* shift, const void* res, int res_ld, int relu_nch, void* out, int out_ld, hipStream_t s);
bool conv_hpipe_ok(DType dt, bool out_f32, const ConvArgs& a);
int launch_conv_hpipe(const ConvArgs& a, hipStream_t s);
int launch_hpipe_pack_weights(const void* w_igemm, void* w_hpipe, int Cout, int Cin, hipStream_t s);
int launch_bottleneck64(const BottleneckArgs& a, hipStream_t s);
int launch_bottleneck64_even(const BottleneckArgs& a, hipStream_t s);
void bottleneck64_even_patch(int H, int W, int* ph_out, int* pw_out, int* rp_out);
int launch_bottleneck64p(const BottleneckArgs& a, hipStream_t s);
int launch_conv_rw3(const BottleneckArgs& a, hipStream_t s);
bool conv_rw3_patch_ok(int ph, int pw);
int launch_conv_rw64(const ConvRw64Args& a, hipStream_t s);
bool conv_rw64_patch_ok(int ph, int pw);
bool conv_pw_tile(int cout, int k_total, bool has_res, int* BM, int* BN);
bool conv_pw_ok(DType dt, bool out_f32, const ConvArgs& a);
int launch_conv_pw(const ConvArgs& a, int BM, int BN, hipStream_t s);
int launch_pw_pack_weights(const void* w_igemm, void* w_pw, int Cout, int K, int BN, hipStream_t s);
bool conv_spw_ok(DType dt, bool out_f32, const ConvArgs& a);
int launch_conv_spw(const ConvArgs& a, hipStream_t s);
int launch_pw_pack_table(const float* scale, const float* shift, float* out, int Cout, int BN, hipStream_t s);

}
```

### sylph-few-shot-detection_amd/sylph_amd/_lib.py

```python
import ctypes
import os
from ctypes import POINTER, Structure, c_char_p, c_float, c_int, c_int64, c_void_p

import torch

_HERE = os.path.dirname(os.path.abspath(__file__))
LIB_PATH = os.environ.get("SYLPH_LIB_PATH") or os.path.join(os.path.dirname(_HERE), "lib", "libsylph_hip.so")

SYLPH_F32 = 0
SYLPH_BF16 = 1
SYLPH_F32S = 2


class SylphConfig(Structure):
    _fields_ = [
        ("resnet_depth", c_int), ("stride_in_1x1", c_int), ("num_cls_convs", c_int), ("num_box_convs", c_int),
        ("nlevels", c_int), ("strides", c_int * 8), ("pixel_mean", c_float * 3), ("pixel_std", c_float * 3),
        ("size_divisibility", c_int), ("use_scale", c_int), ("cond_use_bias", c_int),
        ("pre_nms_thresh", c_float), ("pre_nms_topk", c_int), ("nms_thresh", c_float), ("post_nms_topk", c_int),
        ("thresh_with_ctr", c_int), ("quality_mode", c_int),
        ("cg_tower_layers", c_int), ("cg_has_bias", c_int), ("cg_bias_l2_norm", c_int), ("cg_post_norm", c_int),
        ("cg_conv_l2_norm", c_int), ("cg_use_weight_scale", c_int), ("prior_prob", c_float), ("cand_cap", c_int),
        ("cg_type", c_int), ("tok_num_conv", c_int), ("tok_num_fc", c_int), ("enc_layers", c_int),
        ("head_num_fc", c_int), ("head_fc_dim", c_int), ("cg_meta_bias", c_int), ("cg_has_weight", c_int), ("cg_has_scale", c_int),
        ("num_share_convs", c_int), ("tower_norm", c_int), ("cg_tower_gn_mask", c_int), ("cg_tower_relu_mask", c_int),
        ("tower_deformable", c_int), ("num_groups", c_int), ("width_per_group", c_int),
        ("cg_code_ksize", c_int),
    ]


PROTOTYPES = {
    "sylph_config_default": (None, [POINTER(SylphConfig)]),
    "sylph_ctx_create": (c_int, [c_int, c_int, POINTER(c_void_p)]),
    "sylph_ctx_destroy": (None, [c_void_p]),
    "sylph_last_error": (c_char_p, []),
    "sylph_set_stream": (c_int, [c_void_p, c_void_p]),
    "sylph_set_config": (c_int, [c_void_p, POINTER(SylphConfig)]),
    "sylph_load_weight": (c_int, [c_void_p, c_char_p, c_void_p, POINTER(c_int64), c_int]),
    "sylph_finalize_weights": (c_int, [c_void_p]),
    "sylph_preprocess": (c_int, [c_void_p, c_int, POINTER(c_void_p), POINTER(c_int), POINTER(c_int),
                                 POINTER(c_int), POINTER(c_int)]),
    "sylph_preprocess_u8": (c_int, [c_void_p, c_int, POINTER(c_void_p), POINTER(c_int), POINTER(c_int), POINTER(c_int),
                                    POINTER(c_int), c_int, POINTER(c_int), POINTER(c_int)]),
    "sylph_export_input": (c_int, [c_void_p, c_void_p]),
    "sylph_backbone_fpn": (c_int, [c_void_p]),
    "sylph_import_pyramid": (c_int, [c_void_p, c_int, c_int, c_int, POINTER(c_int), POINTER(c_int),
                                     POINTER(c_void_p)]),
    "sylph_export_pyramid": (c_int, [c_void_p, c_int, c_void_p]),
    "sylph_fcos_head": (c_int, [c_void_p, c_void_p, c_void_p, c_int]),
    "sylph_fcos_head_episodes": (c_int, [c_void_p, c_int, c_void_p, c_void_p, POINTER(c_int), POINTER(c_int)]),
    "sylph_fcos_head_codesets": (c_int, [c_void_p, c_int, c_void_p, c_void_p, POINTER(c_int)]),
    "sylph_fcos_head_pretrained": (c_int, [c_void_p, POINTER(c_int)]),
    "sylph_export_head": (c_int, [c_void_p, c_int, c_void_p, c_void_p, c_void_p, c_void_p]),
    "sylph_import_head": (c_int, [c_void_p, c_int, c_int, c_void_p, c_void_p, c_void_p, c_void_p]),
    "sylph_roi_align": (c_int, [c_void_p, c_void_p, c_void_p]),
    "sylph_roi_align_rois": (c_int, [c_void_p, c_int, c_void_p, POINTER(c_int), c_void_p]),
    "sylph_decode_nms": (c_int, [c_void_p, POINTER(c_int), POINTER(c_int), c_int, c_void_p, c_void_p, c_void_p,
                                 c_void_p, c_void_p, c_void_p, c_void_p, c_void_p]),
    "sylph_decode_nms_codesets": (c_int, [c_void_p, c_int, POINTER(c_int), POINTER(c_int), c_int, c_void_p, c_void_p, c_void_p,
                                          c_void_p, c_void_p, c_void_p, c_void_p, c_void_p]),
    "sylph_codegen": (c_int, [c_void_p, c_void_p, c_void_p]),
    "sylph_codegen_classes": (c_int, [c_void_p, c_void_p, c_int, c_void_p]),
    "sylph_codegen_rois": (c_int, [c_void_p, c_int, c_void_p, POINTER(c_int), c_int, POINTER(c_int), c_void_p]),
    "sylph_roi_table_uploads": (c_int, [c_void_p, POINTER(c_int64)]),
    "sylph_codegen_weight_norm": (c_int, [c_void_p, c_void_p]),
    "sylph_normalize_codes": (c_int, [c_void_p, c_void_p, c_int, c_void_p]),
    "sylph_reduce_codes": (c_int, [c_void_p, c_void_p, c_int, c_int, c_void_p, c_int, c_int]),
    "sylph_conv2d": (c_int, [c_void_p, c_void_p, c_int, c_int, c_int, c_int, c_void_p, c_int, c_int, c_int, c_int,
                             c_int, c_void_p, c_void_p, c_int, c_void_p, c_void_p]),
    "sylph_group_norm": (c_int, [c_void_p, c_void_p, c_int, c_int, c_int, c_void_p, c_void_p, c_int, c_void_p]),
    "sylph_stem_maxpool": (c_int, [c_void_p, c_void_p, c_int, c_int, c_int, c_void_p, c_void_p, c_void_p, c_void_p, c_void_p]),
    "sylph_set_debug_taps": (c_int, [c_void_p, c_int]),
    "sylph_export_stage": (c_int, [c_void_p, c_int, c_void_p]),
    "sylph_export_tower": (c_int, [c_void_p, c_int, c_int, c_int, c_void_p, c_void_p]),
    "sylph_support_tap_numel": (c_int, [c_void_p, c_int, c_int, POINTER(c_int64)]),
    "sylph_export_support": (c_int, [c_void_p, c_int, c_int, c_void_p]),
    "sylph_bottleneck": (c_int, [c_void_p, c_void_p, c_int, c_int, c_int, c_int, c_int, c_int, c_int, POINTER(c_void_p),
                                 POINTER(c_void_p), POINTER(c_void_p), c_void_p]),
    "sylph_bottleneck_even": (c_int, [c_void_p, c_void_p, c_int, c_int, c_int, c_int, c_int, c_int, POINTER(c_void_p),
                                      POINTER(c_void_p), POINTER(c_void_p), c_void_p]),
    "sylph_allgather_codes": (c_int, [c_void_p, c_void_p, c_void_p, c_int, c_int, c_void_p]),
    "sylph_comm_unique_id": (c_int, [ctypes.c_char_p]),
    "sylph_comm_init_rank": (c_int, [c_void_p, ctypes.c_char_p, c_int, c_int, POINTER(c_void_p)]),
    "sylph_comm_destroy": (c_int, [c_void_p]),
    "sylph_fpn_lateral": (c_int, [c_void_p, c_void_p, c_int, c_int, c_int, c_int, c_void_p, c_void_p, c_void_p, c_void_p]),
    "sylph_group_conv": (c_int, [c_void_p, c_void_p] + [c_int] * 6 + [c_void_p, c_void_p, c_void_p, c_int, c_void_p]),
    "sylph_bottleneck_grouped": (c_int, [c_void_p, c_void_p] + [c_int] * 8 + [POINTER(c_void_p), POINTER(c_void_p), POINTER(c_void_p),
                                                                            c_void_p]),
    "sylph_conv3x3_c64": (c_int, [c_void_p, c_void_p, c_int, c_int, c_int, c_void_p, c_void_p, c_void_p, c_int, c_void_p, c_void_p]),
    "sylph_basic_block": (c_int, [c_void_p, c_void_p] + [c_int] * 6 + [POINTER(c_void_p), POINTER(c_void_p), POINTER(c_void_p), c_void_p]),
    "sylph_device_bytes": (c_int64, [c_void_p]),
    "sylph_profile_enable": (c_int, [c_void_p, c_int]),
    "sylph_bench_conv": (c_int, [c_void_p] + [c_int] * 12 + [POINTER(c_float), POINTER(ctypes.c_double)]),
    "sylph_profile_read": (c_int, [c_void_p, POINTER(ctypes.c_double), POINTER(ctypes.c_double), POINTER(c_int64)]),
    "sylph_profile_read_kernels": (c_int, [c_void_p, c_int, ctypes.c_char_p, POINTER(ctypes.c_double), POINTER(ctypes.c_double),
                                           POINTER(c_int64), POINTER(c_int)]),
    "sylph_conv_routes_read": (c_int, [c_void_p, c_int, ctypes.c_char_p, POINTER(c_int)]),
}

_LIB = None


def lib():
    global _LIB
    if _LIB is None:
        if not os.path.exists(LIB_PATH):
            raise RuntimeError(
                f"{LIB_PATH} is missing: build the HIP extension first (python -c 'import __graft_entry__ as g; "
                "g.build()' or make -C sylph-few-shot-detection_amd/csrc).  There is no CPU fallback.")
        _LIB = ctypes.CDLL(LIB_PATH)
        for name, (res, args) in PROTOTYPES.items():
            fn = getattr(_LIB, name)
            fn.restype = res
            fn.argtypes = args
    return _LIB


def check(rc: int, what: str = ""):
    if rc != 0:
        msg = lib().sylph_last_error().decode("utf-8", "replace")
        raise RuntimeError(f"libsylph_hip {what}: {msg}")
```

### sylph-few-shot-detection_amd/sylph_amd/engine.py

```python
import ctypes
from ctypes import c_int, c_int64, c_void_p
from typing import Dict, List, Optional, Sequence, Tuple

import torch

from . import _lib
from ._lib import SylphConfig, check


def _ptr(t: Optional[torch.Tensor]):
    return c_void_p(t.data_ptr()) if t is not None else c_void_p(0)


def _iarr(v: Sequence[int]):
    return (c_int * len(v))(*[int(x) for x in v])


def config_from_cfg(cfg) -> SylphConfig:
    L = _lib.lib()
    sc = SylphConfig()
    L.sylph_config_default(ctypes.byref(sc))
    if cfg is None:
        return sc
    m = cfg.MODEL
    f = m.FCOS
    sc.resnet_depth = int(m.RESNETS.DEPTH)
    sc.stride_in_1x1 = int(bool(m.RESNETS.get("STRIDE_IN_1X1", True)))
    sc.num_cls_convs = int(f.NUM_CLS_CONVS)
    sc.num_box_convs = int(f.NUM_BOX_CONVS)
    sc.num_share_convs = int(f.NUM_SHARE_CONVS)
    sc.tower_deformable = int(bool(f.get("USE_DEFORMABLE", False)))
    r = m.RESNETS
    ng, wpg = int(r.get("NUM_GROUPS", 1)), int(r.get("WIDTH_PER_GROUP", 64))
    basic = sc.resnet_depth in (18, 34)
    if sc.resnet_depth not in (18, 34, 50, 101, 152):
        raise NotImplementedError(f"MODEL.RESNETS.DEPTH {sc.resnet_depth}: 18, 34 (BasicBlock) and 50, 101, 152 (bottleneck) are supported")
    if ng != 1 or wpg != 64:
        if sc.resnet_depth not in (50, 101, 152):
            raise NotImplementedError(f"MODEL.RESNETS.DEPTH {sc.resnet_depth}: ResNeXt needs DEPTH 50, 101 or 152")
        widths = [wpg << s for s in range(4)]
        if ng < 1 or wpg < 1 or any(w < 4 or w > 64 or (w & (w - 1)) for w in widths) or (ng * wpg) % 64 != 0:
            raise NotImplementedError(
                f"MODEL.RESNETS.NUM_GROUPS {ng} / WIDTH_PER_GROUP {wpg}: the grouped conv needs a per-group width WIDTH_PER_GROUP << s "
                f"that is a power of two in [4, 64] at every stage (here {widths}) and NUM_GROUPS * WIDTH_PER_GROUP a multiple of 64")
    sc.num_groups, sc.width_per_group = ng, wpg
    if any(bool(v) for v in r.get("DEFORM_ON_PER_STAGE", [False] * 4)):
        raise NotImplementedError("MODEL.RESNETS.DEFORM_ON_PER_STAGE: deformable bottleneck convs are not supported")
    if int(r.get("RES5_DILATION", 1)) != 1:
        raise NotImplementedError("MODEL.RESNETS.RES5_DILATION != 1 is not supported")
    res2_out = int(r.get("RES2_OUT_CHANNELS", 256))
    if basic and res2_out != 64:
        raise NotImplementedError(f"MODEL.RESNETS.RES2_OUT_CHANNELS {res2_out}: DEPTH {sc.resnet_depth} (BasicBlock) needs RES2_OUT_CHANNELS 64")
    if not basic and res2_out == 64:
        raise NotImplementedError(f"MODEL.RESNETS.RES2_OUT_CHANNELS 64 belongs to DEPTH 18 / 34 (BasicBlock); DEPTH {sc.resnet_depth} needs 256")
    if res2_out != (64 if basic else 256) or int(r.get("STEM_OUT_CHANNELS", 64)) != 64:
        raise NotImplementedError("MODEL.RESNETS.RES2_OUT_CHANNELS / STEM_OUT_CHANNELS: only 256 (64 for DEPTH 18 / 34) / 64 are supported")
    if str(r.get("NORM", "FrozenBN")) != "FrozenBN":
        raise NotImplementedError(f"MODEL.RESNETS.NORM {r.NORM!r}: only FrozenBN (inference) is supported")
    fpn = m.get("FPN", None)
    if fpn is not None:
        if str(fpn.get("FUSE_TYPE", "sum")) != "sum":
            raise NotImplementedError(f"MODEL.FPN.FUSE_TYPE {fpn.FUSE_TYPE!r}: only 'sum' is supported")
        if str(fpn.get("NORM", "") or "") != "":
            raise NotImplementedError(f"MODEL.FPN.NORM {fpn.NORM!r}: only '' (bias convs) is supported")
        if int(fpn.get("OUT_CHANNELS", 256)) != 256:
            raise NotImplementedError("MODEL.FPN.OUT_CHANNELS: only 256 is supported")
    norm = "" if f.NORM is None else str(f.NORM)
    if norm in ("GN", "NaiveGN"):
        sc.tower_norm = 0
    elif norm in ("none", ""):
        sc.tower_norm = 1
    else:
        raise NotImplementedError(f"MODEL.FCOS.NORM {norm!r}: 'GN', 'NaiveGN' and 'none' are supported (the per-level BatchNorm variants are not)")
    strides = list(f.FPN_STRIDES)
    sc.nlevels = len(strides)
    for i, s in enumerate(strides):
        sc.strides[i] = int(s)
    for i in range(3):
        sc.pixel_mean[i] = float(m.PIXEL_MEAN[i])
        sc.pixel_std[i] = float(m.PIXEL_STD[i])
    sc.use_scale = int(bool(f.USE_SCALE))
    sc.pre_nms_thresh = float(f.INFERENCE_TH_TEST)
    sc.pre_nms_topk = int(f.PRE_NMS_TOPK_TEST)
    sc.nms_thresh = float(f.NMS_TH)
    sc.post_nms_topk = int(f.POST_NMS_TOPK_TEST)
    sc.thresh_with_ctr = int(bool(f.THRESH_WITH_CTR) or bool(m.PROPOSAL_GENERATOR.get("OWD", False)))
    bq = sorted(list(f.BOX_QUALITY))
    if bq == ["ctrness"]:
        sc.quality_mode = 0
    elif bq == ["iou"]:
        sc.quality_mode = 1
    elif bq == ["ctrness", "iou"]:
        sc.quality_mode = 2
    else:
        raise NotImplementedError(f"MODEL.FCOS.BOX_QUALITY {bq}")
    sc.prior_prob = float(f.PRIOR_PROB)
    if int(m.RESNETS.get("RES5_DILATION", 1)) != 1:
        raise NotImplementedError("MODEL.RESNETS.RES5_DILATION != 1 is not supported")
    if not bool(m.META_LEARN.EPISODIC_LEARNING):
        if int(f.get("CLS_LOGITS_KERNEL_SIZE", 3)) not in (1, 3):
            raise NotImplementedError("base-detector inference needs MODEL.FCOS.CLS_LOGITS_KERNEL_SIZE 1 or 3")
        sc.cond_use_bias = 1
        return sc
    cg = m.META_LEARN.CODE_GENERATOR
    if int(m.RESNETS.get("RES5_DILATION", 1)) != 1:
        raise NotImplementedError("MODEL.RESNETS.RES5_DILATION != 1 is not supported")
    if bool(cg.ROI_BOX.get("FPN_MULTILEVEL_FEATURE", False)):
        raise NotImplementedError("CODE_GENERATOR.ROI_BOX.FPN_MULTILEVEL_FEATURE is not supported (it fails in the reference too)")
    for knob in ("ALL_MASK", "USE_DEFORMABLE", "META_WEIGHT"):
        if bool(cg.get(knob, False)):
            raise NotImplementedError(f"CODE_GENERATOR.{knob} is not supported")
    if str(cg.ROI_BOX.get("POOLER_TYPE", "ROIAlignV2")) != "ROIAlignV2":
        raise NotImplementedError("CODE_GENERATOR.ROI_BOX.POOLER_TYPE must be ROIAlignV2")
    sc.cg_meta_bias = int(bool(cg.get("META_BIAS", False)))
    sc.cond_use_bias = int(bool(cg.USE_BIAS))
    cg_name = str(cg.NAME)
    if cg_name not in ("CodeGenerator", "ROIEncoder"):
        from .modeling import CODE_GENERATOR_REGISTRY
        comp = CODE_GENERATOR_REGISTRY.get(cg_name) if cg_name in CODE_GENERATOR_REGISTRY else None
        cg_name = getattr(comp, "engine_generator", None) or cg_name
    if cg_name == "ROIEncoder":
        sc.cg_type = 1
        tk, te, hd = cg.TOKENIZER, cg.TRANSFORMER_ENCODER, cg.HEAD
        if int(tk.CONV_DIM) != 256 or int(tk.FC_DIM) != 256 or int(hd.OUTPUT_DIM) != 256:
            raise NotImplementedError("ROIEncoder: TOKENIZER.CONV_DIM / FC_DIM and HEAD.OUTPUT_DIM must be 256")
        if int(tk.NUM_CONV) > 0 and str(tk.NORM) != "GN":
            raise NotImplementedError("ROIEncoder: TOKENIZER.NORM must be 'GN'")
        if int(cg.ROI_BOX.POOLER_RESOLUTION) != 7:
            raise NotImplementedError("ROI_BOX.POOLER_RESOLUTION must be 7")
        sc.tok_num_conv, sc.tok_num_fc = int(tk.NUM_CONV), int(tk.NUM_FC)
        sc.enc_layers, sc.head_num_fc, sc.head_fc_dim = int(te.LAYERS), int(hd.NUM_FC), int(hd.FC_DIM)
        sc.cond_use_bias = 1
        return sc
    if cg_name != "CodeGenerator":
        raise NotImplementedError(f"{cg.NAME} is not implemented")
    tl = list(cg.TOWER_LAYERS)
    sc.cg_tower_layers = len(tl)
    sc.cg_tower_gn_mask = sc.cg_tower_relu_mask = 0
    for i, layer in enumerate(tl):
        norm, act = (list(layer) + ["", ""])[:2]
        norm, act = ("" if norm is None else str(norm)), ("" if act is None else str(act))
        if norm in ("GN", "NaiveGN"):
            sc.cg_tower_gn_mask |= 1 << i
        elif norm not in ("", "none"):
            raise NotImplementedError(f"CODE_GENERATOR.TOWER_LAYERS entry {layer}: norm must be 'GN' or '' (LN / BN / IN are not supported)")
        if act == "ReLU":
            sc.cg_tower_relu_mask |= 1 << i
        elif act != "":
            raise NotImplementedError(f"CODE_GENERATOR.TOWER_LAYERS entry {layer}: activation must be 'ReLU' or ''")
    if len(tl) > 30:
        raise NotImplementedError("more than 30 CODE_GENERATOR.TOWER_LAYERS")
    cl = list(cg.CLS_LAYER)
    if len(cl) != 3 or cl[0] not in ("", "none") or cl[1] != "" or int(cl[2]) not in (1, 3):
        raise NotImplementedError(f"CODE_GENERATOR.CLS_LAYER {cl} (only ['', '', 1] and ['', '', 3]: no norm, no activation, a 1x1 or 3x3 class code)")
    sc.cg_code_ksize = int(cl[2])
    bl = list(cg.BIAS_LAYER)
    sc.cg_has_bias = int(len(bl) != 0)
    if len(bl) and (len(bl) != 3 or bl[0] not in ("", "none") or bl[1] != "" or int(bl[2]) != 1):
        raise NotImplementedError(f"CODE_GENERATOR.BIAS_LAYER {bl} (only [] or ['', '', 1]: no norm, no ReLU, one conv)")
    for knob, field in (("WEIGHT_LAYER", "cg_has_weight"), ("SCALE_LAYER", "cg_has_scale")):
        lay = list(cg.get(knob, []))
        if len(lay) and (len(lay) != 3 or lay[0] not in ("", "none")):
            raise NotImplementedError(f"CODE_GENERATOR.{knob} {lay} (only [] or ['', '', 1])")
        setattr(sc, field, int(len(lay) != 0))
    if bool(cg.COMPRESS_CODE_W_MAX) or bool(cg.CLS_REWEIGHT) or bool(cg.BOX_ON):
        raise NotImplementedError("COMPRESS_CODE_W_MAX / CLS_REWEIGHT / BOX_ON are not supported")
    sc.cg_bias_l2_norm = int(bool(cg.BIAS_L2_NORM))
    sc.cg_post_norm = int(str(cg.POST_NORM) != "")
    if sc.cg_post_norm and str(cg.POST_NORM) != "GN":
        raise NotImplementedError("CODE_GENERATOR.POST_NORM must be '' or 'GN'")
    sc.cg_conv_l2_norm = int(bool(cg.CONV_L2_NORM))
    sc.cg_use_weight_scale = int(bool(cg.USE_WEIGHT_SCALE))
    return sc


def code_set_offsets(n_classes: Sequence[int]) -> List[int]:
    off = [0]
    for g, n in enumerate(n_classes):
        if int(n) < 1:
            raise ValueError(f"code set {g} is empty (N_g = {int(n)}): every set needs at least one class")
        off.append(off[-1] + int(n))
    return off


def check_code_sets(codes, code_ksize: int = 1) -> List[int]:
    if code_ksize != 1:
        raise NotImplementedError(f"head_code_sets runs 1x1 class codes only: CODE_GENERATOR.CLS_LAYER kernel size {code_ksize} is not "
                                  "supported here (call head once per code set)")
    codes = list(codes)
    if len(codes) == 0:
        raise ValueError("head_code_sets needs at least one code set (G = 0)")
    n = []
    for g, (w, b) in enumerate(codes):
        if w.dim() != 4:
            raise ValueError(f"code set {g}: Weight has dimension: {w.dim()}")
        if w.size(2) != 1 or w.size(3) != 1:
            raise ValueError(f"code set {g}: class code of spatial size {w.size(2)}x{w.size(3)}: cls_conv must be (N, 256 k, 1, 1)")
        if w.size(1) < 256 or w.size(1) % 256 != 0:
            raise ValueError(f"code set {g}: weight has wrong shape, {tuple(w.shape)}: 256 channels (or a multiple, ROIEncoder) expected")
        if b is not None and b.numel() != w.size(0):
            raise ValueError(f"code set {g}: {b.numel()} biases for {w.size(0)} classes")
        n.append(int(w.size(0)))
    code_set_offsets(n)
    if len({b is None for _, b in codes}) != 1:
        raise ValueError("cls_bias must be given for every code set or for none")
    return n


class Engine:

    def __init__(self, cfg=None, dtype: str = "bf16", device: int = 0, cand_cap: int = 0):
        if not torch.cuda.is_available():
            raise RuntimeError("sylph_amd.Engine needs a ROCm GPU (torch.cuda.is_available() is False); "
                               "there is no CPU fallback")
        self.L = _lib.lib()
        self.device = torch.device("cuda", device)
        self.dtype = dtype
        self._ctx = c_void_p(0)
        dt = {"bf16": _lib.SYLPH_BF16, "f32": _lib.SYLPH_F32, "fp32": _lib.SYLPH_F32, "f32s": _lib.SYLPH_F32S}[dtype]
        check(self.L.sylph_ctx_create(device, dt, ctypes.byref(self._ctx)), "ctx_create")
        self.sc = config_from_cfg(cfg)
        if cand_cap:
            self.sc.cand_cap = cand_cap
        check(self.L.sylph_set_config(self._ctx, ctypes.byref(self.sc)), "set_config")
        self.nlevels = self.sc.nlevels
        self.is_roi_encoder = int(self.sc.cg_type) == 1
        self.code_ksize = 1 if self.is_roi_encoder else max(1, int(self.sc.cg_code_ksize))
        self.code_len = 256 * self.code_ksize ** 2 + 1
        self.cond_scale = 1.0
        self.cond_scales = [1.0]
        self._cond_scales_loaded = False
        self.owd = bool(cfg.MODEL.PROPOSAL_GENERATOR.get("OWD", False)) if cfg is not None else False
        self._batch = None
        self._sup_rows = None
        self._ncls = 0
        self._keep = []
        self._lib_writes = 0

    def close(self):
        if self._ctx:
            self.L.sylph_ctx_destroy(self._ctx)
            self._ctx = c_void_p(0)

    def __del__(self):
        try:
            self.close()
        except Exception:
            pass

    def _stream(self):
        check(self.L.sylph_set_stream(self._ctx, c_void_p(torch.cuda.current_stream(self.device).cuda_stream)))

    def load_state_dict(self, sd: Dict[str, torch.Tensor]):
        for k, v in sd.items():
            if not torch.is_tensor(v) or not v.is_floating_point():
                continue
            if ".fcos_head.cond_cls_logits.scales." in k and k.endswith(".scale"):
                i = int(k.split(".scales.")[1].split(".")[0])
                while len(self.cond_scales) <= i:
                    self.cond_scales.append(1.0)
                self.cond_scales[i] = float(v.reshape(-1)[0])
                self._cond_scales_loaded = True
                if i == 0:
                    self.cond_scale = self.cond_scales[0]
            t = v.detach().to("cpu", torch.float32).contiguous()
            shape = (c_int64 * max(t.dim(), 1))(*(list(t.shape) if t.dim() else [1]))
            check(self.L.sylph_load_weight(self._ctx, k.encode(), c_void_p(t.data_ptr()), shape, max(t.dim(), 1)),
                  f"load_weight({k})")
        check(self.L.sylph_finalize_weights(self._ctx), "finalize_weights")
        self._codes_key = None

    def level_shapes(self, H: int, W: int) -> List[Tuple[int, int]]:
        h, w = H // 8, W // 8
        out = []
        for _ in range(self.nlevels):
            out.append((h, w))
            h, w = (h - 1) // 2 + 1, (w - 1) // 2 + 1
        return out

    def preprocess(self, images: List[torch.Tensor]) -> Tuple[int, int]:
        self._stream()
        imgs = [im.to(self.device, torch.float32).contiguous() for im in images]
        B = len(imgs)
        ptrs = (c_void_p * B)(*[im.data_ptr() for im in imgs])
        hs, ws = _iarr([im.shape[1] for im in imgs]), _iarr([im.shape[2] for im in imgs])
        ph, pw = c_int(0), c_int(0)
        check(self.L.sylph_preprocess(self._ctx, B, ptrs, hs, ws, ctypes.byref(ph), ctypes.byref(pw)), "preprocess")
        self._keep = imgs
        self._batch = (B, ph.value, pw.value, [(int(im.shape[1]), int(im.shape[2])) for im in imgs])
        return ph.value, pw.value

    def preprocess_u8(self, images: List[torch.Tensor], new_sizes: List[Tuple[int, int]], rgb_input: bool = False) -> Tuple[int, int]:
        self._stream()
        imgs = [im.to(self.device, non_blocking=True).contiguous() for im in images]
        for im in imgs:
            assert im.dtype == torch.uint8 and im.dim() == 3 and im.shape[2] == 3, "uint8 HWC images expected"
        B = len(imgs)
        ptrs = (c_void_p * B)(*[im.data_ptr() for im in imgs])
        ph, pw = c_int(0), c_int(0)
        check(self.L.sylph_preprocess_u8(self._ctx, B, ptrs, _iarr([im.shape[0] for im in imgs]), _iarr([im.shape[1] for im in imgs]),
                                         _iarr([s[0] for s in new_sizes]), _iarr([s[1] for s in new_sizes]), int(rgb_input),
                                         ctypes.byref(ph), ctypes.byref(pw)), "preprocess_u8")
        self._keep = imgs
        self._batch = (B, ph.value, pw.value, [(int(s[0]), int(s[1])) for s in new_sizes])
        return ph.value, pw.value

    def export_input(self) -> torch.Tensor:
        self._stream()
        B, H, W, _ = self._batch
        out = torch.empty(B, 3, H, W, device=self.device)
        check(self.L.sylph_export_input(self._ctx, _ptr(out)), "export_input")
        return out

    def backbone(self):
        self._stream()
        check(self.L.sylph_backbone_fpn(self._ctx), "backbone_fpn")

    def import_pyramid(self, levels: List[torch.Tensor], padded_hw: Tuple[int, int],
                       image_sizes: Optional[List[Tuple[int, int]]] = None):
        self._stream()
        B = levels[0].shape[0]
        H, W = padded_hw
        lv = [t.to(self.device, torch.float32).contiguous() for t in levels]
        exp = self.level_shapes(H, W)
        for t, (h, w) in zip(lv, exp):
            assert tuple(t.shape) == (B, 256, h, w), f"level shape {tuple(t.shape)} != {(B, 256, h, w)}"
        sizes = image_sizes or [(H, W)] * B
        ptrs = (c_void_p * len(lv))(*[t.data_ptr() for t in lv])
        check(self.L.sylph_import_pyramid(self._ctx, B, H, W, _iarr([s[0] for s in sizes]),
                                          _iarr([s[1] for s in sizes]), ptrs), "import_pyramid")
        self._keep = lv
        self._batch = (B, H, W, list(sizes))

    def export_pyramid(self) -> List[torch.Tensor]:
        self._stream()
        B, H, W, _ = self._batch
        out = []
        for l, (h, w) in enumerate(self.level_shapes(H, W)):
            t = torch.empty(B, 256, h, w, device=self.device, dtype=torch.float32)
            check(self.L.sylph_export_pyramid(self._ctx, l, _ptr(t)), "export_pyramid")
            out.append(t)
        return out

    def _fold_codes(self, cls_conv: torch.Tensor, cls_bias: Optional[torch.Tensor], raw: bool = False):
        k = cls_conv.size(1) // 256
        assert cls_conv.size(1) == 256 * k and k >= 1, f"weight has wrong shape, {tuple(cls_conv.shape)}"
        assert k == 1 or (self.is_roi_encoder and not raw), "feature.size(1) != weight.size(1)"
        w = cls_conv.to(self.device, torch.float32).reshape(cls_conv.size(0), -1)
        b = cls_bias.to(self.device, torch.float32).reshape(-1).contiguous() if cls_bias is not None else None
        if self.is_roi_encoder and not raw:
            if not self._cond_scales_loaded:
                sc = [1.0 / k] * k
            else:
                if len(self.cond_scales) < max(k - 1, 1):
                    raise ValueError(f"the checkpoint has {len(self.cond_scales)} cond_cls_logits scales; a {256 * k}-channel class "
                                     f"code needs {max(k - 1, 1)}")
                sc = list(self.cond_scales)
            per_chunk = [sc[0]] + [sc[i] for i in range(k - 1)]
            w = sum(s_ * w[:, 256 * i:256 * (i + 1)] for i, s_ in enumerate(per_chunk))
            b = b * float(sum(per_chunk)) if b is not None else None
        w = w.contiguous()
        if b is not None:
            assert b.numel() == w.size(0)
        return w, b

    def head(self, cls_conv: torch.Tensor, cls_bias: Optional[torch.Tensor], raw: bool = False):
        self._stream()
        assert cls_conv.dim() == 4, f"Weight has dimension: {cls_conv.dim()}"
        k = self.code_ksize
        if cls_conv.size(2) != k or cls_conv.size(3) != k:
            raise ValueError(f"class code of spatial size {cls_conv.size(2)}x{cls_conv.size(3)} on an engine configured for {k}x{k} codes "
                             f"(CODE_GENERATOR.CLS_LAYER kernel size {k}): cls_conv must be (N, 256, {k}, {k})")
        if self.owd:
            if getattr(self, "_owd_codes", None) is None:
                self._owd_codes = (torch.zeros(1, 256 * k * k, device=self.device), torch.full((1,), 40.0, device=self.device))
            w1, b1 = self._owd_codes
            self._ncls = 1
            check(self.L.sylph_fcos_head(self._ctx, _ptr(w1), _ptr(b1), 1), "fcos_head (OWD)")
            return
        key = (id(cls_conv), cls_conv._version, id(cls_bias), None if cls_bias is None else cls_bias._version, bool(raw),
               tuple(self.cond_scales), self._cond_scales_loaded, self._lib_writes)
        cached = getattr(self, "_codes_key", None) == key
        if not cached:
            self._codes = self._fold_codes(cls_conv, cls_bias, raw)
            self._codes_src = (cls_conv, cls_bias)
            self._codes_key = key
        w, b = self._codes
        self._ncls = w.size(0)
        check(self.L.sylph_fcos_head(self._ctx, _ptr(w), _ptr(b), self._ncls), "fcos_head")

    def head_episodes(self, codes, image_episode):
        self._stream()
        if self.code_ksize != 1:
            raise NotImplementedError(f"head_episodes runs 1x1 class codes only: CODE_GENERATOR.CLS_LAYER kernel size {self.code_ksize} is not "
                                      "supported here (call head once per episode)")
        codes = [(w, b) for w, b in codes]
        image_episode = [int(e) for e in image_episode]
        if len(codes) == 0:
            raise ValueError("head_episodes needs at least one episode")
        if len(image_episode) != self._batch[0]:
            raise ValueError(f"image_episode has {len(image_episode)} entries for a batch of {self._batch[0]} images")
        if any(e < 0 or e >= len(codes) for e in image_episode):
            raise ValueError(f"image_episode entries must be in [0, {len(codes)})")
        for w, _ in codes:
            assert w.dim() == 4, f"Weight has dimension: {w.dim()}"
            assert w.size(2) == 1 and w.size(3) == 1
        if self.owd:
            return self.head(*codes[0])
        if len({b is None for _, b in codes}) != 1:
            raise ValueError("cls_bias must be given for every episode or for none")
        key = (tuple((id(w), w._version, id(b), None if b is None else b._version) for w, b in codes),
               tuple(self.cond_scales), self._cond_scales_loaded, self._lib_writes)
        if getattr(self, "_ep_codes_key", None) != key:
            folded = [self._fold_codes(w, b) for w, b in codes]
            W = torch.cat([w for w, _ in folded]).contiguous()
            Bv = torch.cat([b for _, b in folded]).contiguous() if folded[0][1] is not None else None
            self._ep_codes = (W, Bv, [int(w.size(0)) for w, _ in folded])
            self._ep_codes_src = codes
            self._ep_codes_key = key
        W, Bv, n = self._ep_codes
        self._ncls = max(n)
        check(self.L.sylph_fcos_head_episodes(self._ctx, len(n), _ptr(W), _ptr(Bv), _iarr(n), _iarr(image_episode)), "fcos_head_episodes")

    def head_code_sets(self, codes):
        self._stream()
        codes = [(w, b) for w, b in codes]
        check_code_sets(codes, self.code_ksize)
        if self.owd:
            if getattr(self, "_owd_codes", None) is None:
                self._owd_codes = (torch.zeros(1, 256, device=self.device), torch.full((1,), 40.0, device=self.device))
            w1, b1 = self._owd_codes
            key, folded = ("owd", len(codes)), [(w1, b1)] * len(codes)
        else:
            for w, _ in codes:
                if w.size(1) != 256 and not self.is_roi_encoder:
                    raise ValueError(f"weight has wrong shape, {tuple(w.shape)}: feature.size(1) != weight.size(1) (256 channels expected)")
            key = (tuple((id(w), w._version, id(b), None if b is None else b._version) for w, b in codes),
                   tuple(self.cond_scales), self._cond_scales_loaded, self._lib_writes)
            folded = None
        if getattr(self, "_cs_codes_key", None) != key:
            if folded is None:
                folded = [self._fold_codes(w, b) for w, b in codes]
            W = torch.cat([w.reshape(w.size(0), -1) for w, _ in folded]).contiguous()
            Bv = torch.cat([b for _, b in folded]).contiguous() if folded[0][1] is not None else None
            self._cs_codes = (W, Bv, [int(w.size(0)) for w, _ in folded])
            self._cs_codes_src = codes
            self._cs_codes_key = key
        W, Bv, n = self._cs_codes
        self._ncls = sum(n)
        self._cs_n = list(n)
        check(self.L.sylph_fcos_head_codesets(self._ctx, len(n), _ptr(W), _ptr(Bv), _iarr(n)), "fcos_head_codesets")

    def decode_code_sets(self, out_sizes: Optional[List[Tuple[int, int]]] = None, max_out: Optional[int] = None):
        self._stream()
        B = self._batch[0]
        G = len(getattr(self, "_cs_n", None) or [0])
        S = G * B
        if max_out is None:
            max_out = self.default_max_out()
        dev = self.device
        boxes = torch.empty(S, max_out, 4, device=dev)
        scores = torch.empty(S, max_out, device=dev)
        ints = torch.empty(3, S, max_out, device=dev, dtype=torch.int32)
        locs = torch.empty(S, max_out, 2, device=dev)
        counts = torch.empty(S + 1, device=dev, dtype=torch.int32)
        oh = _iarr([s[0] for s in out_sizes]) if out_sizes is not None else None
        ow = _iarr([s[1] for s in out_sizes]) if out_sizes is not None else None
        check(self.L.sylph_decode_nms_codesets(self._ctx, G, oh, ow, max_out, _ptr(boxes), _ptr(scores), _ptr(ints[0]), _ptr(ints[1]),
                                               _ptr(locs), _ptr(ints[2]), _ptr(counts), c_void_p(counts.data_ptr() + 4 * S)),
              "decode_nms_codesets")
        slot = self.__dict__.setdefault("_count_ring", {}).setdefault(("code sets", S), {"bufs": [], "next": 0})
        if len(slot["bufs"]) < 8:
            slot["bufs"].append(torch.empty(S + 1, dtype=torch.int32, pin_memory=True))
            host_counts = slot["bufs"][-1]
        else:
            host_counts = slot["bufs"][slot["next"] % 8]
            slot["next"] += 1
        host_counts.copy_(counts, non_blocking=True)
        done = torch.cuda.Event()
        done.record(torch.cuda.current_stream(dev))
        flat = self.decode_fetch((S, boxes, scores, ints, None, locs, None, host_counts, done, torch.cuda.current_stream(dev)))
        return [flat[g * B:(g + 1) * B] for g in range(G)]

    def head_pretrained(self) -> int:
        self._stream()
        n = c_int(0)
        check(self.L.sylph_fcos_head_pretrained(self._ctx, ctypes.byref(n)), "fcos_head_pretrained")
        self._ncls = n.value
        return n.value

    def export_head(self):
        self._stream()
        B, H, W, _ = self._batch
        lo, rg, ct, io = [], [], [], []
        for l, (h, w) in enumerate(self.level_shapes(H, W)):
            a = torch.empty(B, self._ncls, h, w, device=self.device)
            r = torch.empty(B, 4, h, w, device=self.device)
            c = torch.empty(B, 1, h, w, device=self.device)
            q = torch.empty(B, 1, h, w, device=self.device)
            check(self.L.sylph_export_head(self._ctx, l, _ptr(a), _ptr(r), _ptr(c), _ptr(q)), "export_head")
            lo.append(a); rg.append(r); ct.append(c); io.append(q)
        return lo, rg, ct, io

    def import_head(self, logits: List[torch.Tensor], reg: List[torch.Tensor], ctr: List[torch.Tensor],
                    iou: Optional[List[torch.Tensor]] = None):
        self._stream()
        N = int(logits[0].shape[1])
        keep = []
        for l in range(self.nlevels):
            ts = [t[l].to(self.device, torch.float32).contiguous() if t is not None else None for t in (logits, reg, ctr, iou)]
            keep.append(ts)
            check(self.L.sylph_import_head(self._ctx, N, l, _ptr(ts[0]), _ptr(ts[1]), _ptr(ts[2]), _ptr(ts[3])), "import_head")
        self._keep_head = keep
        self._ncls = N

    def roi_align(self, boxes: torch.Tensor) -> torch.Tensor:
        self._stream()
        B = self._batch[0]
        bx = boxes.to(self.device, torch.float32).reshape(-1, 4).contiguous()
        assert bx.shape[0] == B
        out = torch.empty(B, 256, 7, 7, device=self.device)
        check(self.L.sylph_roi_align(self._ctx, _ptr(bx), _ptr(out)), "roi_align")
        return out

    def _check_rois(self, boxes: torch.Tensor, roi_image) -> Tuple[torch.Tensor, List[int]]:
        if getattr(self, "_batch", None) is None:
            raise ValueError("no current batch")
        if boxes is None or roi_image is None:
            raise ValueError("boxes and roi_image must be given")
        B = self._batch[0]
        ri = [int(i) for i in (roi_image.tolist() if torch.is_tensor(roi_image) else roi_image)]
        R = len(ri)
        if R < 1:
            raise ValueError("the ROI list is empty (R < 1)")
        if boxes.numel() != 4 * R:
            raise ValueError(f"boxes has {boxes.numel()} values for {R} ROIs: (R, 4) expected")
        for r, i in enumerate(ri):
            if i < 0 or i >= B:
                raise ValueError(f"roi_image[{r}] = {i} is outside the batch of {B} images")
        return boxes.to(self.device, torch.float32).reshape(R, 4).contiguous(), ri

    def roi_align_rois(self, boxes: torch.Tensor, roi_image) -> torch.Tensor:
        self._stream()
        bx, ri = self._check_rois(boxes, roi_image)
        out = torch.empty(len(ri), 256, 7, 7, device=self.device)
        check(self.L.sylph_roi_align_rois(self._ctx, len(ri), _ptr(bx), _iarr(ri), _ptr(out)), "roi_align_rois")
        return out

    def decode(self, out_sizes: Optional[List[Tuple[int, int]]] = None, max_out: Optional[int] = None):
        return self.decode_fetch(self.decode_launch(out_sizes, max_out))

    def default_max_out(self) -> int:
        K = int(self.sc.post_nms_topk)
        return 2 * K if K > 0 else int(self.sc.pre_nms_topk) * self.nlevels

    def decode_launch(self, out_sizes: Optional[List[Tuple[int, int]]] = None, max_out: Optional[int] = None):
        self._stream()
        B = self._batch[0]
        if max_out is None:
            max_out = self.default_max_out()
        dev = self.device
        boxes = torch.empty(B, max_out, 4, device=dev)
        scores = torch.empty(B, max_out, device=dev)
        ints = torch.empty(3, B, max_out, device=dev, dtype=torch.int32)
        classes, levels, cand = ints[0], ints[1], ints[2]
        locs = torch.empty(B, max_out, 2, device=dev)
        counts = torch.empty(B + 1, device=dev, dtype=torch.int32)
        oh = _iarr([s[0] for s in out_sizes]) if out_sizes is not None else None
        ow = _iarr([s[1] for s in out_sizes]) if out_sizes is not None else None
        check(self.L.sylph_decode_nms(self._ctx, oh, ow, max_out, _ptr(boxes), _ptr(scores), _ptr(classes),
                                      _ptr(levels), _ptr(locs), _ptr(cand), _ptr(counts),
                                      c_void_p(counts.data_ptr() + 4 * B)), "decode_nms")
        ring = self.__dict__.setdefault("_count_ring", {})
        slot = ring.setdefault(B, {"bufs": [], "next": 0})
        if len(slot["bufs"]) < 8:
            slot["bufs"].append(torch.empty(B + 1, dtype=torch.int32, pin_memory=True))
            host_counts = slot["bufs"][-1]
        else:
            host_counts = slot["bufs"][slot["next"] % 8]
            slot["next"] += 1
        host_counts.copy_(counts, non_blocking=True)
        done = torch.cuda.Event()
        done.record(torch.cuda.current_stream(dev))
        return (B, boxes, scores, ints, None, locs, None, host_counts, done, torch.cuda.current_stream(dev))

    def decode_fetch(self, handle):
        B, boxes, scores, ints, _, locs, _, host_counts, done, stream = handle
        done.synchronize()
        cnt = host_counts.tolist()
        status = cnt[B]
        if status & 1:
            raise RuntimeError("sylph decode: per-level candidate capacity exceeded (raise cand_cap)")
        if status & 2:
            raise RuntimeError("sylph decode: more tied detections than max_out")
        with torch.cuda.stream(stream):
            wide = ints.long()
            classes, levels, cand = wide[0], wide[1], wide[2]
        cur = torch.cuda.current_stream(self.device)
        if cur != stream:
            cur.wait_stream(stream)
        nar = torch.Tensor.narrow
        cols = [[nar(r, 0, 0, n) for r, n in zip(t.unbind(0), cnt)] for t in (boxes, scores, classes, levels, locs, cand)]
        keys = ("pred_boxes", "scores", "pred_classes", "fpn_levels", "locations", "cand_index")
        return [dict(zip(keys, vals)) for vals in zip(*cols)]

    def _image_boxes(self, boxes: torch.Tensor) -> torch.Tensor:
        bx = boxes.to(self.device, torch.float32).reshape(-1, 4).contiguous()
        B = self._batch[0]
        assert bx.shape[0] == B, f"pooled_features.shape[0] {bx.shape[0]} Vs batch_size * num_shots {B}"
        return bx

    def _run_codegen(self, what: str, bx: torch.Tensor, n_codes: Optional[int], *args) -> torch.Tensor:
        self._stream()
        out = torch.empty(*(() if n_codes is None else (n_codes,)), self.code_len, device=self.device)
        self._keep_boxes = bx
        check(getattr(self.L, "sylph_" + what)(self._ctx, *args, _ptr(out)), what)
        self._sup_rows = bx.shape[0]
        return out

    def codegen(self, boxes: torch.Tensor) -> torch.Tensor:
        bx = self._image_boxes(boxes)
        B = bx.shape[0]
        if B > 64:
            raise ValueError(f"{B} support images of one class in one call: the code generator's shot reduction handles at most 64 "
                             "(split the class into chunks and reduce them, as the base-class path does)")
        return self._run_codegen("codegen", bx, None, _ptr(bx))

    def codegen_classes(self, boxes: torch.Tensor, shots: int) -> torch.Tensor:
        bx = self._image_boxes(boxes)
        B = bx.shape[0]
        assert B % shots == 0, f"pooled_features.shape[0] {B} Vs batch_size * num_shots {B}"
        if shots > 64:
            raise ValueError(f"{shots} shots per class in one call: the code generator's shot reduction handles at most 64 (split the "
                             "class into chunks and reduce them, as the base-class path does)")
        return self._run_codegen("codegen_classes", bx, B // shots, _ptr(bx), int(shots))

    def codegen_rois(self, boxes: torch.Tensor, roi_image, seg_len) -> torch.Tensor:
        bx, ri = self._check_rois(boxes, roi_image)
        if seg_len is None:
            raise ValueError("seg_len must be given")
        sl = [int(n) for n in (seg_len.tolist() if torch.is_tensor(seg_len) else seg_len)]
        if len(sl) < 1:
            raise ValueError("the ROI list has no segment (n_seg < 1)")
        for j, n in enumerate(sl):
            if n < 1:
                raise ValueError(f"seg_len[{j}] = {n}: a segment needs at least one ROI")
        if sum(sl) != len(ri):
            raise ValueError(f"the segment lengths sum to {sum(sl)}, not to R = {len(ri)}")
        return self._run_codegen("codegen_rois", bx, len(sl), len(ri), _ptr(bx), _iarr(ri), len(sl), _iarr(sl))

    def roi_table_uploads(self) -> int:
        n = c_int64(0)
        check(self.L.sylph_roi_table_uploads(self._ctx, ctypes.byref(n)), "roi_table_uploads")
        return n.value

    def codegen_weight_norm(self, n_classes: int = 1) -> torch.Tensor:
        self._stream()
        out = torch.empty(n_classes, device=self.device)
        check(self.L.sylph_codegen_weight_norm(self._ctx, _ptr(out)), "codegen_weight_norm")
        return out

    def normalize_codes(self, codes: torch.Tensor, weight_norm: Optional[torch.Tensor] = None) -> torch.Tensor:
        self._stream()
        assert codes.is_cuda and codes.dtype == torch.float32 and codes.is_contiguous()
        if codes.shape[-1] != self.code_len:
            raise ValueError(f"normalize_codes: rows of {codes.shape[-1]} floats on an engine whose codes are {self.code_ksize}x{self.code_ksize} "
                             f"({self.code_len} floats per row; CODE_GENERATOR.CLS_LAYER kernel size {self.code_ksize})")
        wn = None
        if weight_norm is not None:
            wn = weight_norm.to(self.device, torch.float32).reshape(-1).contiguous()
            assert wn.numel() == codes.shape[0]
        check(self.L.sylph_normalize_codes(self._ctx, _ptr(codes), codes.shape[0], _ptr(wn)), "normalize_codes")
        self._lib_writes += 1
        return codes

    def reduce_codes(self, rows: torch.Tensor, num_classes: int, divide_by_acc: bool = True) -> torch.Tensor:
        self._stream()
        assert rows.is_cuda and rows.dtype == torch.float32 and rows.dim() == 2 and rows.is_contiguous()
        out = torch.empty(num_classes, rows.shape[1], device=self.device)
        check(self.L.sylph_reduce_codes(self._ctx, _ptr(rows), rows.shape[0], rows.shape[1], _ptr(out), num_classes,
                                        int(divide_by_acc)), "reduce_codes")
        return out

    def conv2d(self, x, w, scale=None, shift=None, stride=1, pad=0, relu=False, residual=None):
        self._stream()
        x = x.to(self.device, torch.float32).contiguous()
        B, C, H, W = x.shape
        wh = w.detach().cpu().float().contiguous()
        Cout, _, KH, KW = wh.shape
        Ho, Wo = (H + 2 * pad - KH) // stride + 1, (W + 2 * pad - KW) // stride + 1
        y = torch.empty(B, Cout, Ho, Wo, device=self.device)
        sc = scale.detach().cpu().float().contiguous() if scale is not None else None
        sh = shift.detach().cpu().float().contiguous() if shift is not None else None
        rs = residual.to(self.device, torch.float32).contiguous() if residual is not None else None
        check(self.L.sylph_conv2d(self._ctx, _ptr(x), B, C, H, W, _ptr(wh), Cout, KH, KW, stride, pad, _ptr(sc),
                                  _ptr(sh), int(relu), _ptr(rs), _ptr(y)), "conv2d")
        return y

    def group_norm(self, x, gamma, beta, relu=False):
        self._stream()
        x = x.to(self.device, torch.float32).contiguous()
        B, C, H, W = x.shape
        assert C == 256
        y = torch.empty_like(x)
        g, b = gamma.detach().cpu().float().contiguous(), beta.detach().cpu().float().contiguous()
        check(self.L.sylph_group_norm(self._ctx, _ptr(x), B, H, W, _ptr(g), _ptr(b), int(relu), _ptr(y)), "group_norm")
        return y

    def stem_maxpool(self, x, w, scale, shift):
        self._stream()
        x = x.to(self.device, torch.float32).contiguous()
        B, C, H, W = x.shape
        assert C == 3
        H2, W2 = (H - 1) // 2 + 1, (W - 1) // 2 + 1
        H4, W4 = (H2 - 1) // 2 + 1, (W2 - 1) // 2 + 1
        so = torch.empty(B, 64, H2, W2, device=self.device)
        po = torch.empty(B, 64, H4, W4, device=self.device)
        wh, sc, sh = [t.detach().cpu().float().contiguous() for t in (w, scale, shift)]
        check(self.L.sylph_stem_maxpool(self._ctx, _ptr(x), B, H, W, _ptr(wh), _ptr(sc), _ptr(sh), _ptr(so), _ptr(po)), "stem_maxpool")
        return so, po

    def set_debug_taps(self, on: bool = True):
        check(self.L.sylph_set_debug_taps(self._ctx, int(on)), "set_debug_taps")

    def export_stage(self, stage: int) -> torch.Tensor:
        self._stream()
        B, H, W, _ = self._batch
        h, w = (H - 1) // 2 + 1, (W - 1) // 2 + 1
        for _ in range(stage - 1):
            h, w = (h - 1) // 2 + 1, (w - 1) // 2 + 1
        out = torch.empty(B, (64 if self.sc.resnet_depth in (18, 34) else 256) << (stage - 2), h, w, device=self.device)
        check(self.L.sylph_export_stage(self._ctx, stage, _ptr(out)), "export_stage")
        return out

    def export_tower(self, tower: int, layer: int, with_coef: bool = True):
        self._stream()
        B, H, W, _ = self._batch
        ys, cs = [], []
        for l, (h, w) in enumerate(self.level_shapes(H, W)):
            y = torch.empty(B, 256, h, w, device=self.device)
            cf = torch.empty(B, 256, 2, device=self.device) if with_coef else None
            check(self.L.sylph_export_tower(self._ctx, tower, layer, l, _ptr(y), _ptr(cf)), "export_tower")
            ys.append(y); cs.append(cf)
        return ys, cs

    SUPPORT_STAGES = ("roi", "gn_y", "gn_coef", "layer_out", "conv_out", "context", "mscam", "tokens", "cls_tokens")

    def export_support(self, stage: str, index: int = 0) -> torch.Tensor:
        self._stream()
        st = self.SUPPORT_STAGES.index(stage)
        n = c_int64(0)
        check(self.L.sylph_support_tap_numel(self._ctx, st, int(index), ctypes.byref(n)), "support_tap_numel")
        out = torch.empty(n.value, device=self.device)
        check(self.L.sylph_export_support(self._ctx, st, int(index), _ptr(out)), "export_support")
        B = self._batch[0] if stage == "context" else self._sup_rows
        if stage == "gn_coef":
            return out.view(B, 256, 2)
        if stage in ("tokens", "cls_tokens"):
            return out.view(-1, 256)
        return out.view(B, -1, 7, 7)

    def bottleneck(self, x, ws, scales, shifts, stride=1):
        self._stream()
        x = x.to(self.device, torch.float32).contiguous()
        B, Cin, H, W = x.shape
        mid, cout = ws[0].shape[0], ws[2].shape[0]
        n = 4 if len(ws) > 3 and ws[3] is not None else 3
        keep = [[t.detach().cpu().float().contiguous() for t in lst[:n]] for lst in (ws, scales, shifts)]
        arrs = [(c_void_p * 4)(*([t.data_ptr() for t in lst] + [None] * (4 - n))) for lst in keep]
        Ho, Wo = (H - 1) // stride + 1, (W - 1) // stride + 1
        y = torch.empty(B, cout, Ho, Wo, device=self.device)
        check(self.L.sylph_bottleneck(self._ctx, _ptr(x), B, Cin, H, W, stride, mid, cout, arrs[0], arrs[1], arrs[2], _ptr(y)),
              "bottleneck")
        return y

    def bottleneck_even(self, x, ws, scales, shifts):
        self._stream()
        x = x.to(self.device, torch.float32).contiguous()
        B, Cin, H, W = x.shape
        mid, cout = ws[0].shape[0], ws[2].shape[0]
        keep = [[t.detach().cpu().float().contiguous() for t in lst[:3]] for lst in (ws, scales, shifts)]
        arrs = [(c_void_p * 4)(*([t.data_ptr() for t in lst] + [None])) for lst in keep]
        y = torch.empty(B, cout, H // 2, W // 2, device=self.device)
        check(self.L.sylph_bottleneck_even(self._ctx, _ptr(x), B, Cin, H, W, mid, cout, arrs[0], arrs[1], arrs[2], _ptr(y)),
              "bottleneck_even")
        return y

    def bottleneck_grouped(self, x, ws, scales, shifts, stride=1, groups=32):
        self._stream()
        x = x.to(self.device, torch.float32).contiguous()
        B, Cin, H, W = x.shape
        mid, cout = ws[0].shape[0], ws[2].shape[0]
        n = 4 if len(ws) > 3 and ws[3] is not None else 3
        keep = [[t.detach().cpu().float().contiguous() for t in lst[:n]] for lst in (ws, scales, shifts)]
        arrs = [(c_void_p * 4)(*([t.data_ptr() for t in lst] + [None] * (4 - n))) for lst in keep]
        Ho, Wo = (H - 1) // stride + 1, (W - 1) // stride + 1
        y = torch.empty(B, cout, Ho, Wo, device=self.device)
        check(self.L.sylph_bottleneck_grouped(self._ctx, _ptr(x), B, Cin, H, W, stride, mid, cout, groups, arrs[0], arrs[1], arrs[2],
                                              _ptr(y)), "bottleneck_grouped")
        return y

    def group_conv(self, x, w, scale, shift, groups, stride=1, relu=True):
        self._stream()
        x = x.to(self.device, torch.float32).contiguous()
        B, C, H, W = x.shape
        wh = w.detach().cpu().float().contiguous()
        sc, sh = scale.detach().cpu().float().contiguous(), shift.detach().cpu().float().contiguous()
        Ho, Wo = (H - 1) // stride + 1, (W - 1) // stride + 1
        y = torch.empty(B, C, Ho, Wo, device=self.device)
        check(self.L.sylph_group_conv(self._ctx, _ptr(x), B, C, H, W, groups, stride, _ptr(wh), _ptr(sc), _ptr(sh), int(relu), _ptr(y)),
              "group_conv")
        return y

    def conv3x3_c64(self, x, w, scale, shift, relu=True, residual=None):
        self._stream()
        x = x.to(self.device, torch.float32).contiguous()
        B, C, H, W = x.shape
        assert C == 64 and tuple(w.shape) == (64, 64, 3, 3)
        wh, sc, sh = [t.detach().cpu().float().contiguous() for t in (w, scale, shift)]
        rs = residual.to(self.device, torch.float32).contiguous() if residual is not None else None
        assert rs is None or rs.shape == x.shape
        y = torch.empty_like(x)
        check(self.L.sylph_conv3x3_c64(self._ctx, _ptr(x), B, H, W, _ptr(wh), _ptr(sc), _ptr(sh), int(relu), _ptr(rs), _ptr(y)),
              "conv3x3_c64")
        return y

    def basic_block(self, x, ws, scales, shifts, stride=1):
        self._stream()
        x = x.to(self.device, torch.float32).contiguous()
        B, Cin, H, W = x.shape
        cout = ws[0].shape[0]
        n = 3 if len(ws) > 2 and ws[2] is not None else 2
        keep = [[t.detach().cpu().float().contiguous() for t in lst[:n]] for lst in (ws, scales, shifts)]
        arrs = [(c_void_p * 3)(*([t.data_ptr() for t in lst] + [None] * (3 - n))) for lst in keep]
        Ho, Wo = (H - 1) // stride + 1, (W - 1) // stride + 1
        y = torch.empty(B, cout, Ho, Wo, device=self.device)
        check(self.L.sylph_basic_block(self._ctx, _ptr(x), B, Cin, H, W, stride, cout, arrs[0], arrs[1], arrs[2], _ptr(y)), "basic_block")
        return y

    def fpn_lateral(self, x, w, bias, top=None):
        self._stream()
        x = x.to(self.device, torch.float32).contiguous()
        B, C, H, W = x.shape
        wh, bh = w.detach().cpu().float().contiguous(), bias.detach().cpu().float().contiguous()
        tp = top.to(self.device, torch.float32).contiguous() if top is not None else None
        y = torch.empty(B, 256, H, W, device=self.device)
        check(self.L.sylph_fpn_lateral(self._ctx, _ptr(x), B, C, H, W, _ptr(wh), _ptr(bh), _ptr(tp), _ptr(y)), "fpn_lateral")
        return y

    def device_bytes(self) -> int:
        return int(self.L.sylph_device_bytes(self._ctx))

    def bench_conv(self, B, H, W, Cin, Cout, K, stride=1, pad=0, res=False, relu=True, gn=False, iters=10):
        self._stream()
        ms, fl = ctypes.c_float(0), ctypes.c_double(0)
        check(self.L.sylph_bench_conv(self._ctx, B, H, W, Cin, Cout, K, stride, pad, int(res), int(relu), int(gn), iters,
                                      ctypes.byref(ms), ctypes.byref(fl)), "bench_conv")
        return ms.value, fl.value / (ms.value * 1e-3) / 1e12

    def profile_enable(self, on: bool = True):
        check(self.L.sylph_profile_enable(self._ctx, int(on)), "profile_enable")

    def profile_read(self) -> Dict[str, float]:
        mx = 32
        names = ctypes.create_string_buffer(mx * 64)
        ms, fl, ln, n = (ctypes.c_double * mx)(), (ctypes.c_double * mx)(), (c_int64 * mx)(), c_int(0)
        check(self.L.sylph_profile_read_kernels(self._ctx, mx, names, ms, fl, ln, ctypes.byref(n)), "profile_read_kernels")
        kern = {}
        for i in range(n.value):
            kern[names.raw[i * 64:(i + 1) * 64].split(b"\0", 1)[0].decode()] = {"ms": ms[i], "flops": fl[i], "launches": int(ln[i])}
        return {"conv_ms": sum(k["ms"] for k in kern.values()), "conv_flops": sum(k["flops"] for k in kern.values()),
                "conv_launches": sum(k["launches"] for k in kern.values()), "kernels": kern}

    def conv_routes(self, max_routes: int = 1024):
        names, n = ctypes.create_string_buffer(max_routes * 64), c_int(0)
        check(self.L.sylph_conv_routes_read(self._ctx, max_routes, names, ctypes.byref(n)), "conv_routes_read")
        return [names.raw[i * 64:(i + 1) * 64].split(b"\0", 1)[0].decode() for i in range(n.value)]
```

Before: 2272.

## Fuse res3 conv3+residual with next block's conv1 into one persistent pair kernel

Adds a persistent bf16 MFMA kernel for res3 identity blocks (512->128->512). It computes conv3 with scale, shift, residual and ReLU into LDS, stores y, then immediately computes the next block's 1x1 conv1 (512->128) from the same LDS tile. The goal is to avoid re-reading the 512-channel activation from memory and to save a kernel launch per block pair. It uses warp-specialised loader, residual and storer waves with double buffering. The cost is a large, hand-scheduled kernel with a narrow shape gate and a minimum-tile threshold below which it does not run.

```diff
diff --git a/include/sylph_hip.h b/include/sylph_hip.h
--- a/include/sylph_hip.h
+++ b/include/sylph_hip.h
@@ -149,6 +149,9 @@
 int sylph_bottleneck_even(sylph_ctx* ctx, const float* x_nchw_dev, int B, int Cin, int H, int W, int mid, int cout,
                           const float* const* w_host, const float* const* scale_host, const float* const* shift_host,
                           float* y_nchw_dev);
+int sylph_res3_pair(sylph_ctx* ctx, const float* t2_nchw_dev, const float* x_nchw_dev, int B, int H, int W, const float* w3_host,
+                    const float* s3_host, const float* b3_host, const float* w1_host, const float* s1_host, const float* b1_host,
+                    float* y_nchw_dev, float* t1_nchw_dev);
 
 int sylph_fpn_lateral(sylph_ctx* ctx, const float* x_nchw_dev, int B, int C, int H, int W, const float* w_host, const float* bias_host,
                       const float* top_nchw_dev, float* y_nchw_dev);
diff --git a/sylph-few-shot-detection_amd/csrc/api_backbone.hip b/sylph-few-shot-detection_amd/csrc/api_backbone.hip
--- a/sylph-few-shot-detection_amd/csrc/api_backbone.hip
+++ b/sylph-few-shot-detection_amd/csrc/api_backbone.hip
@@ -120,7 +120,23 @@
   return add_conv3x3(c, ops, L, pick_conv3_route(c, L, B, H, W, 1), B, H, W, 1, x, res, y, relu);
 }
 
-BlockRoute pick_block_route(const sylph_ctx* c, const sylph_ctx::Block& blk, int B, int Cin, int Hin, int Win, int stride, int mid, int cout, int flags) {
+static const long PAIR_MIN_MTILES128 = 512;
+
+static bool block_pair_ok(const sylph_ctx* c, const sylph_ctx::Block& blk, const sylph_ctx::Block& next, int B, int Cin, int Hin, int Win, int stride,
+                          int mid, int cout) {
+  const int on = knob::block_pair();
+  if (!on || c->dt != DT_BF16 || blk.basic || next.basic || blk.has_sc || next.has_sc || blk.c2.groups != 1 || next.c2.groups != 1) return false;
+  if (Cin != 512 || cout != 512 || mid != 128 || stride != 1) return false;
+  const ConvLayer &c3 = blk.c3, &c1 = next.c1;
+  if (c3.Cin != 128 || c3.Cout != 512 || c3.Cout_pad != 512 || c3.KH != 1 || c3.KW != 1 || !c3.scale || !c3.shift) return false;
+  if (c1.Cin != 512 || c1.Cout != 128 || c1.Cout_pad != 128 || c1.KH != 1 || c1.KW != 1 || !c1.scale || !c1.shift) return false;
+  const long hw = (long)Hin * Win;
+  if (hw * 1024 >= (1L << 32) || (long)B * hw >= (1L << 31)) return false;
+  return on == 2 || ((long)B * hw + 127) / 128 >= PAIR_MIN_MTILES128;
+}
+
+BlockRoute pick_block_route(const sylph_ctx* c, const sylph_ctx::Block& blk, int B, int Cin, int Hin, int Win, int stride, int mid, int cout, int flags,
+                            const sylph_ctx::Block* next) {
   BlockRoute r;
   r.chunk = B;
   r.s1 = c->cfg.stride_in_1x1 ? stride : 1; r.s3 = c->cfg.stride_in_1x1 ? 1 : stride;
@@ -136,6 +152,17 @@
     r.refuse = "the stride-2-output bottleneck is the fused bf16 identity block (C 256, mid 64) on a map of even height and width";
     return r;
   }
+  r.pair_ok = next && block_pair_ok(c, blk, *next, B, Cin, Hin, Win, stride, mid, cout);
+  r.pair_out = (flags & BK_PAIR_OUT) != 0;
+  r.pair_in = (flags & BK_PAIR_IN) != 0;
+  if (r.pair_out && !r.pair_ok) {
+    r.refuse = "the block pair launch is conv3 + residual of a bf16 identity block 512 -> 128 -> 512 followed by another such block";
+    return r;
+  }
+  if (r.pair_in && (c->dt != DT_BF16 || blk.has_sc || Cin != 512 || mid != 128 || stride != 1 || !dense2)) {
+    r.refuse = "internal: BK_PAIR_IN on a block whose conv1 the pair launch cannot have computed";
+    return r;
+  }
   if (!dense2) {
     const long per_img = std::max({(long)Hin * Win * Cin, (long)r.H1 * r.W1 * mid, (long)r.Ho * r.Wo * mid, (long)r.Ho * r.Wo * cout});
     const int nb = (int)std::min<long>(B, ((1L << 31) - 1) / per_img);
@@ -169,9 +196,26 @@
   return r;
 }
 
+int add_res3_pair(sylph_ctx* c, std::vector<OpFn>& ops, const ConvLayer& c3, const ConvLayer& c1_next, int B, int HW, const void* t2, const void* x, void* y,
+                  void* t1) {
+  const std::vector<PairTile> pt = pair_tiles(B, HW);
+  void* ptd = nullptr;
+  RET(upload(c, &ptd, pt.data(), pt.size() * sizeof(PairTile)));
+  PairArgs pa;
+  memset(&pa, 0, sizeof(pa));
+  pa.t2 = t2; pa.x = x; pa.y = y; pa.t1 = t1;
+  pa.w3 = (const __bf16*)c3.w; pa.w1 = (const __bf16*)c1_next.w;
+  pa.s3 = c3.scale; pa.b3 = c3.shift; pa.s1 = c1_next.scale; pa.b1 = c1_next.shift;
+  pa.tiles = (const PairTile*)ptd; pa.n_tiles = (int)pt.size();
+  const double fl = 2.0 * (double)B * HW * (512.0 * 128 + 128.0 * 512);
+  ops.push_back([=](hipStream_t s) { return timed_op(c, "conv_spw_kernel_pair", fl, s, [=](hipStream_t st) { return launch_conv_spw_pair(pa, st); }); });
+  if (c->prof) c->route_recs.push_back("spw_pair " + std::to_string(PAIR_TILE_ROWS) + "x512+128");
+  return 0;
+}
+
 int add_bottleneck(sylph_ctx* c, std::vector<OpFn>& ops, const sylph_ctx::Block& blk, int B, const void* X, int Cin, int Hin, int Win,
-                          int stride, int mid, int cout, void* Y, const BkScratch& scr, int flags) {
-  const BlockRoute r = pick_block_route(c, blk, B, Cin, Hin, Win, stride, mid, cout, flags);
+                          int stride, int mid, int cout, void* Y, const BkScratch& scr, int flags, const sylph_ctx::Block* next) {
+  const BlockRoute r = pick_block_route(c, blk, B, Cin, Hin, Win, stride, mid, cout, flags, next);
   if (!r.refuse.empty()) return fail(r.refuse);
   const DType dt = c->dt;
   const int H1 = r.H1, W1 = r.W1, Ho = r.Ho, Wo = r.Wo;
@@ -211,8 +255,10 @@
     return add_patch_kernel(c, ops, "bottleneck64p_kernel", fl, launch_bottleneck64p, ba, B, Hin, Win, ph, pw);
   }
   const int route_stride = (flags & BK_IN_COMPACT) ? 2 : 0;
-  ConvOpts o1; o1.stride = r.s1; o1.relu_nch = 1 << 30; o1.route_stride = route_stride;
-  RET(add_conv(c, ops, blk.c1, X, Cin, t1, mid, image_segs(B, Hin, Win, H1, W1), o1));
+  if (!r.pair_in) {
+    ConvOpts o1; o1.stride = r.s1; o1.relu_nch = 1 << 30; o1.route_stride = route_stride;
+    RET(add_conv(c, ops, blk.c1, X, Cin, t1, mid, image_segs(B, Hin, Win, H1, W1), o1));
+  }
   switch (r.conv2) {
     case Conv2Form::grouped: {
       GroupConvArgs ga;
@@ -230,6 +276,7 @@
       RET(add_conv3x3(c, ops, blk.c2, Conv3Route{}, B, H1, W1, r.s3, t1, nullptr, t2, 1));
       break;
   }
+  if (r.pair_out) return add_res3_pair(c, ops, blk.c3, next->c1, B, Ho * Wo, t2, X, Y, t1);
   if (r.fused_sc) {
     std::vector<SegDesc> sg = image_segs(B, Ho, Wo, Ho, Wo);
     for (int b = 0; b < B; ++b) { sg[b].in2_row0 = b * Hin * Win; sg[b].in2_W = Win; }
@@ -340,6 +387,7 @@
     auto& blocks = c->stages[si];
     void* Y = nullptr;
     BkScratch scr{t1, t2, sc, &P->bk_trash};
+    bool pair_in = false;
     for (size_t bi = 0; bi < blocks.size(); ++bi) {
       const int stride = bi == 0 ? first_stride : 1;
       Y = (Y == Ya) ? Yb : Ya;
@@ -347,9 +395,13 @@
       const bool even_tail = knob::bk_strided_tail() && !basic && bi > 0 && bi + 1 == blocks.size() && !fpn_input && si + 1 < 4 && c->cfg.stride_in_1x1 &&
                              !c->stages[si + 1].empty() && !c->stages[si + 1][0].basic &&
                              pick_block_route(c, blocks[bi], B, Cin, Hin, Win, stride, mid, cout, 0).tail_ok;
+      const sylph_ctx::Block* nextb = !basic && bi + 1 < blocks.size() ? &blocks[bi + 1] : nullptr;
+      const bool pair_out = nextb && pick_block_route(c, blocks[bi], B, Cin, Hin, Win, stride, mid, cout, 0, nextb).pair_ok;
       if (basic) RET(add_basic_block(c, ops, blocks[bi], B, X, Cin, Hin, Win, stride, cout, Y, scr));
       else RET(add_bottleneck(c, ops, blocks[bi], B, X, Cin, Hin, Win, stride, mid, cout, Y, scr,
-                              even_tail ? BK_EVEN_OUT : (bi == 0 && in_compact) ? BK_IN_COMPACT : 0));
+                              (even_tail ? BK_EVEN_OUT : (bi == 0 && in_compact) ? BK_IN_COMPACT : 0) | (pair_out ? BK_PAIR_OUT : 0) | (pair_in ? BK_PAIR_IN : 0),
+                              nextb));
+      pair_in = pair_out;
       if (bi == 0) in_compact = false;
       if (even_tail) {
         P->tail_even = true; P->tail_x = X;
diff --git a/sylph-few-shot-detection_amd/csrc/api_internal.h b/sylph-few-shot-detection_amd/csrc/api_internal.h
--- a/sylph-few-shot-detection_amd/csrc/api_internal.h
+++ b/sylph-few-shot-detection_amd/csrc/api_internal.h
@@ -16,6 +16,7 @@
 #include "../../include/sylph_hip.h"
 #include "common.h"
 #include "kernels.h"
+#include "res3_pair_tiles.h"
 
 using namespace sylph;
 namespace sylph_host {
@@ -72,6 +73,7 @@
 SYLPH_KNOB_LIVE(conv_rw64, "SYLPH_CONV_RW64", 1)
 SYLPH_KNOB_ONCE(fuse_bottleneck, "SYLPH_FUSE_BOTTLENECK", 1)
 SYLPH_KNOB_ONCE(bk_strided_tail, "SYLPH_BK_STRIDED_TAIL", 1)
+SYLPH_KNOB_ONCE(block_pair, "SYLPH_BLOCK_PAIR", 1)
 SYLPH_KNOB_ONCE(stem_kernel, "SYLPH_STEM_KERNEL", 1)
 SYLPH_KNOB_ONCE(fuse_stem_pool, "SYLPH_FUSE_STEM_POOL", 1)
 SYLPH_KNOB_ONCE(head_streams, "SYLPH_HEAD_STREAMS", 1)
@@ -384,12 +386,15 @@
   bool fused_sc = false;
   bool tail_ok = false;
   int s1 = 1, s3 = 1, H1 = 0, W1 = 0, Ho = 0, Wo = 0;
+  bool pair_ok = false;
+  bool pair_out = false;
+  bool pair_in = false;
 };
 
 enum class StemRoute { fused_pool, stem_conv, igemm };
 
 struct BkScratch { void *t1, *t2, *sc; void** trash; };
-enum { BK_EVEN_OUT = 1, BK_IN_COMPACT = 2 };
+enum { BK_EVEN_OUT = 1, BK_IN_COMPACT = 2, BK_PAIR_OUT = 4, BK_PAIR_IN = 8 };
 
 namespace sylph_host {
 std::shared_ptr<PilCoeffs> pil_bilinear_coeffs(int in_size, int out_size);
@@ -436,9 +441,12 @@
 std::vector<SegDesc> image_segs(int B, int Hin, int Win, int Hout, int Wout, int resH = 0, int resW = 0);
 int ensure_pyramid(sylph_ctx* c, Plan* P);
 Conv3Route pick_conv3_route(const sylph_ctx* c, const ConvLayer& L, int B, int H, int W, int stride);
-BlockRoute pick_block_route(const sylph_ctx* c, const sylph_ctx::Block& blk, int B, int Cin, int Hin, int Win, int stride, int mid, int cout, int flags);
+BlockRoute pick_block_route(const sylph_ctx* c, const sylph_ctx::Block& blk, int B, int Cin, int Hin, int Win, int stride, int mid, int cout, int flags,
+                            const sylph_ctx::Block* next = nullptr);
 StemRoute pick_stem_route(const sylph_ctx* c);
-int add_bottleneck(sylph_ctx* c, std::vector<OpFn>& ops, const sylph_ctx::Block& blk, int B, const void* X, int Cin, int Hin, int Win, int stride, int mid, int cout, void* Y, const BkScratch& scr, int flags = 0);
+int add_bottleneck(sylph_ctx* c, std::vector<OpFn>& ops, const sylph_ctx::Block& blk, int B, const void* X, int Cin, int Hin, int Win, int stride, int mid, int cout, void* Y, const BkScratch& scr, int flags = 0,
+                   const sylph_ctx::Block* next = nullptr);
+int add_res3_pair(sylph_ctx* c, std::vector<OpFn>& ops, const ConvLayer& c3, const ConvLayer& c1_next, int B, int HW, const void* t2, const void* x, void* y, void* t1);
 int add_conv3x3_c64(sylph_ctx* c, std::vector<OpFn>& ops, const ConvLayer& L, int B, int H, int W, const void* x, const void* res, void* y, int relu);
 int add_basic_block(sylph_ctx* c, std::vector<OpFn>& ops, const sylph_ctx::Block& blk, int B, const void* X, int Cin, int Hin, int Win, int stride, int cout, void* Y, const BkScratch& scr);
 int build_backbone(sylph_ctx* c, Plan* P);
diff --git a/sylph-few-shot-detection_amd/csrc/api_parity.hip b/sylph-few-shot-detection_amd/csrc/api_parity.hip
--- a/sylph-few-shot-detection_amd/csrc/api_parity.hip
+++ b/sylph-few-shot-detection_amd/csrc/api_parity.hip
@@ -165,6 +165,40 @@
   if (Cin != 256 || mid != 64 || cout != 256 || c->dt != DT_BF16) return fail("sylph_bottleneck_even: the fused identity block is C 256, mid 64, bf16");
   if (!w_host[0] || !w_host[1] || !w_host[2] || w_host[3]) return fail("sylph_bottleneck_even: an identity block has three convs and no shortcut");
   return bottleneck_entry(c, x, B, Cin, H, W, 1, mid, cout, 1, w_host, scale_host, shift_host, y, true);
+}
+
+int sylph_res3_pair(sylph_ctx* c, const float* t2, const float* x, int B, int H, int W, const float* w3_host, const float* s3_host,
+                    const float* b3_host, const float* w1_host, const float* s1_host, const float* b1_host, float* y, float* t1) {
+  HIPCHK(hipSetDevice(c->device));
+  if (c->dt != DT_BF16) return fail("sylph_res3_pair: the pair kernel is bf16");
+  if (B < 1 || H < 1 || W < 1 || (long)H * W * 1024 >= (1L << 32) || (long)B * H * W >= (1L << 31)) return fail("sylph_res3_pair: bad shape");
+  if (!t2 || !x || !w3_host || !s3_host || !b3_host || !w1_host || !s1_host || !b1_host || !y || !t1) return fail("sylph_res3_pair: null argument");
+  Scratch tmp(c, Records::to_caller);
+  HostTensor h3, h1;
+  h3.shape = {512, 128, 1, 1}; h3.data.assign(w3_host, w3_host + (size_t)512 * 128);
+  h1.shape = {128, 512, 1, 1}; h1.data.assign(w1_host, w1_host + (size_t)128 * 512);
+  ConvLayer L3, L1;
+  RET(pack_conv(&tmp, {&h3}, &L3));
+  RET(pack_conv(&tmp, {&h1}, &L1));
+  if (L3.Cout_pad != 512 || L1.Cout_pad != 128) return fail("internal: sylph_res3_pair weight padding");
+  RET(upload_vec(&tmp, &L3.scale, std::vector<float>(s3_host, s3_host + 512), 512));
+  RET(upload_vec(&tmp, &L3.shift, std::vector<float>(b3_host, b3_host + 512), 512));
+  RET(upload_vec(&tmp, &L1.scale, std::vector<float>(s1_host, s1_host + 128), 128));
+  RET(upload_vec(&tmp, &L1.shift, std::vector<float>(b1_host, b1_host + 128), 128));
+  const size_t hw = (size_t)H * W, e = tmp.esz();
+  void *t2d, *xd, *yd, *t1d;
+  RET(tmp.dalloc(&t2d, B * hw * 128 * e));
+  RET(tmp.dalloc(&xd, B * hw * 512 * e));
+  RET(tmp.dalloc(&yd, B * hw * 512 * e));
+  RET(tmp.dalloc(&t1d, B * hw * 128 * e));
+  RET(import_nchw(&tmp, t2, t2d, B, 128, (int)hw));
+  RET(import_nchw(&tmp, x, xd, B, 512, (int)hw));
+  std::vector<OpFn> ops;
+  RET(add_res3_pair(&tmp, ops, L3, L1, B, (int)hw, t2d, xd, yd, t1d));
+  RET(run_ops(c, ops, "res3_pair"));
+  tmp.hand_records();
+  RET(export_nchw(&tmp, yd, y, B, 512, (int)hw));
+  return export_nchw(&tmp, t1d, t1, B, 128, (int)hw);
 }
 
 int sylph_bottleneck_grouped(sylph_ctx* c, const float* x, int B, int Cin, int H, int W, int stride, int mid, int cout, int groups,
diff --git a/sylph-few-shot-detection_amd/csrc/common.h b/sylph-few-shot-detection_amd/csrc/common.h
--- a/sylph-few-shot-detection_amd/csrc/common.h
+++ b/sylph-few-shot-detection_amd/csrc/common.h
@@ -87,6 +87,16 @@
   int relu;
 };
 
+struct PairTile;
+struct PairArgs {
+  const void *t2, *x;
+  void *y, *t1;
+  const __bf16 *w3, *w1;
+  const float *s3, *b3, *s1, *b1;
+  const PairTile* tiles;
+  int n_tiles;
+};
+
 template <typename T> struct Cvt;
 template <> struct Cvt<float> {
   static __device__ __forceinline__ float to_f(float v) { return v; }
@@ -170,6 +180,7 @@
 int launch_pw_pack_weights(const void* w_igemm, void* w_pw, int Cout, int K, int BN, hipStream_t s);
 bool conv_spw_ok(DType dt, bool out_f32, const ConvArgs& a);
 int launch_conv_spw(const ConvArgs& a, hipStream_t s);
+int launch_conv_spw_pair(const PairArgs& a, hipStream_t s);
 int launch_pw_pack_table(const float* scale, const float* shift, float* out, int Cout, int BN, hipStream_t s);
 
 }
diff --git a/sylph-few-shot-detection_amd/csrc/conv_spw_pair.hip b/sylph-few-shot-detection_amd/csrc/conv_spw_pair.hip
--- /dev/null
+++ b/sylph-few-shot-detection_amd/csrc/conv_spw_pair.hip
@@ -0,0 +1,285 @@
+#include "gfx950.h"
+#include "res3_pair_tiles.h"
+
+namespace sylph {
+
+namespace {
+constexpr int PT = PAIR_TILE_ROWS;
+constexpr int OFF_A = 0, A_BYTES = PT * 256;
+constexpr int OFF_TAB = OFF_A + A_BYTES;
+constexpr int OFF_Y = OFF_TAB + (2 * 512 + 2 * 128) * 4;
+constexpr int Y_BYTES = PT * 1024;
+constexpr int PAIR_LDS = OFF_Y + 2 * Y_BYTES;
+static_assert(PT == 64, "the wave tiling below is written for 64-row tiles");
+static_assert(PAIR_LDS <= 160 * 1024, "LDS budget");
+typedef int i32x4 __attribute__((ext_vector_type(4)));
+}
+
+__global__ __launch_bounds__(512, 1) void conv_spw_kernel_pair(const PairArgs a) {
+  extern __shared__ __attribute__((aligned(16))) char smem[];
+  const int tid = threadIdx.x, lane = tid & 63;
+  const int wave = __builtin_amdgcn_readfirstlane(tid >> 6);
+  const int l31 = lane & 31, lh = lane >> 5, l15 = lane & 15, kb = lane >> 4;
+  auto opaque_lane = [&]() { int ln = lane; asm volatile("" : "+v"(ln)); return ln; };
+  const bool loader = wave < 2, resw = wave == 2 || wave == 3, storer = wave >= 4;
+  int t = blockIdx.x;
+  const int t_step = gridDim.x;
+  if (t >= a.n_tiles) return;
+  const unsigned lds0 = (unsigned)(size_t)(__attribute__((address_space(3))) char*)smem;
+  auto load_desc = [&](int ti) {
+    const PairTile* p = a.tiles + ti;
+    i32x4 d;
+    asm volatile("s_load_dwordx4 %0, %1, 0x0\n\ts_waitcnt lgkmcnt(0)" : "=&s"(d) : "s"(p));
+    return PairTile{d[0], d[1], d[2], 0};
+  };
+
+  bf16x8 wf[2][8], wg[16];
+  {
+    const bf16_t* wp = a.w3 + (size_t)(wave * 64 + l31) * 128 + lh * 8;
+#pragma unroll
+    for (int j = 0; j < 2; ++j)
+#pragma unroll
+      for (int ks = 0; ks < 8; ++ks) wf[j][ks] = *reinterpret_cast<const bf16x8*>(wp + j * 32 * 128 + ks * 16);
+    const bf16_t* wq = a.w1 + (size_t)(wave * 16 + l15) * 512 + kb * 8;
+#pragma unroll
+    for (int ks = 0; ks < 16; ++ks) wg[ks] = *reinterpret_cast<const bf16x8*>(wq + ks * 32);
+  }
+  {
+    float* tabp = reinterpret_cast<float*>(smem + OFF_TAB);
+    tabp[tid] = a.s3[tid];
+    tabp[512 + tid] = a.b3[tid];
+    if (tid < 256) tabp[1024 + tid] = tid < 128 ? a.s1[tid] : a.b1[tid - 128];
+  }
+  __builtin_amdgcn_s_waitcnt(0x0070);
+  __syncthreads();
+
+  const char* const t2b = reinterpret_cast<const char*>(a.t2);
+  auto issue_a = [&](const PairTile& d) {
+    const int ln = opaque_lane(), r8 = ln >> 3, s8 = ln & 7;
+    const char* base = t2b + (size_t)(unsigned)d.img_row0 * 256 + wave * 128 + ((s8 ^ r8) << 4);
+    char* dst = smem + OFF_A + wave * 8192;
+#pragma unroll
+    for (int k = 0; k < 8; ++k) {
+      const unsigned off = (unsigned)pair_tile_load_row(d, 8 * k + r8) * 256u;
+      __builtin_amdgcn_global_load_lds((gbl_ptr_t)(base + off), (lds_ptr_t)(dst + k * 1024), 16, 0, 0);
+    }
+  };
+  const char* const xb = reinterpret_cast<const char*>(a.x);
+  auto issue_res = [&](const PairTile& d, int buf) {
+    const int ln = opaque_lane(), r8 = ln >> 3, s8 = ln & 7;
+    const char* base = xb + (size_t)(unsigned)d.img_row0 * 1024 + (wave - 2) * 512 + ((s8 ^ r8) << 4);
+    char* dst = smem + OFF_Y + buf * Y_BYTES + (wave - 2) * 4 * 8192;
+#pragma unroll
+    for (int k = 0; k < 8; ++k) {
+      const char* src = base + (unsigned)pair_tile_load_row(d, 8 * k + r8) * 1024u;
+#pragma unroll
+      for (int cg = 0; cg < 4; ++cg)
+        __builtin_amdgcn_global_load_lds((gbl_ptr_t)(src + cg * 128), (lds_ptr_t)(dst + cg * 8192 + k * 1024), 16, 0, 0);
+    }
+  };
+  char* const yb = reinterpret_cast<char*>(a.y);
+  char* const t1b = reinterpret_cast<char*>(a.t1);
+  const int sw = wave - 4;
+  auto store_y = [&](const PairTile& d, int buf) {
+    const int ln = opaque_lane(), r8 = ln >> 3, s8 = ln & 7;
+    char* const gbase = yb + (size_t)(unsigned)d.img_row0 * 1024 + ((s8 ^ r8) << 4);
+#pragma unroll
+    for (int h = 0; h < 4; ++h) {
+      const int cg = 2 * sw + (h >> 1), k0 = (h & 1) * 4;
+      const unsigned region = lds0 + OFF_Y + buf * Y_BYTES + cg * 8192 + ln * 16;
+      u32x4 o[4];
+#pragma unroll
+      for (int k = 0; k < 4; ++k) asm volatile("ds_read_b128 %0, %1" : "=v"(o[k]) : "v"(region + (k0 + k) * 1024));
+      asm volatile("s_waitcnt lgkmcnt(0)" : "+v"(o[0]), "+v"(o[1]), "+v"(o[2]), "+v"(o[3]));
+#pragma unroll
+      for (int k = 0; k < 4; ++k) {
+        const int rc = 8 * (k0 + k) + r8;
+        if (pair_tile_stores(d, rc)) *reinterpret_cast<u32x4*>(gbase + (unsigned)(d.row0 + rc) * 1024u + cg * 128) = o[k];
+      }
+    }
+  };
+  auto store_t1 = [&](const PairTile& d, int buf) {
+    const int ln = opaque_lane(), l15 = ln & 15, kb = ln >> 4;
+    const unsigned region = lds0 + OFF_Y + buf * Y_BYTES + sw * 4096 + ln * 16;
+    u32x4 o[4];
+#pragma unroll
+    for (int k = 0; k < 4; ++k) asm volatile("ds_read_b128 %0, %1" : "=v"(o[k]) : "v"(region + k * 1024));
+    asm volatile("s_waitcnt lgkmcnt(0)" : "+v"(o[0]), "+v"(o[1]), "+v"(o[2]), "+v"(o[3]));
+#pragma unroll
+    for (int k = 0; k < 4; ++k) {
+      const int rc = 16 * sw + 4 * k + kb;
+      if (pair_tile_stores(d, rc))
+        *reinterpret_cast<u32x4*>(t1b + (size_t)(unsigned)d.img_row0 * 256 + (unsigned)(d.row0 + rc) * 256u + ((l15 ^ (rc & 15)) << 4)) = o[k];
+    }
+  };
+
+  unsigned aoff[4];
+#pragma unroll
+  for (int ks = 0; ks < 4; ++ks) aoff[ks] = (unsigned)(l31 * 128 + (((2 * ks + lh) ^ (l31 & 7)) << 4));
+  const unsigned tab = lds0 + OFF_TAB;
+
+  PairTile cur = load_desc(t), prev = cur;
+  bool have_prev = false;
+  int b = 0;
+  if (loader) { issue_a(cur); wait_vmcnt<0>(); }
+  if (resw) issue_res(cur, 0);
+  fenced_barrier();
+
+  while (true) {
+    const int tn = t + t_step;
+    const bool next_valid = tn < a.n_tiles;
+    const unsigned ybuf = lds0 + OFF_Y + b * Y_BYTES;
+    if (storer && have_prev) store_t1(prev, b ^ 1);
+
+    f32x16 acc[2][2];
+    {
+      bf16x8 fa[2][2];
+      auto rd = [&](int s, bf16x8(&f)[2]) {
+        const unsigned ad = lds0 + OFF_A + (s >> 2) * 8192 + aoff[s & 3];
+        asm volatile("ds_read_b128 %0, %1" : "=v"(f[0]) : "v"(ad));
+        asm volatile("ds_read_b128 %0, %1" : "=v"(f[1]) : "v"(ad + 4096));
+      };
+      rd(0, fa[0]);
+#pragma unroll
+      for (int s = 0; s < 8; ++s) {
+        bf16x8(&f)[2] = fa[s & 1];
+        if (s < 7) {
+          rd(s + 1, fa[(s + 1) & 1]);
+          asm volatile("s_waitcnt lgkmcnt(2)" : "+v"(f[0]), "+v"(f[1]));
+        } else {
+          asm volatile("s_waitcnt lgkmcnt(0)" : "+v"(f[0]), "+v"(f[1]));
+        }
+#pragma unroll
+        for (int j = 0; j < 2; ++j)
+#pragma unroll
+          for (int i = 0; i < 2; ++i) {
+            if (s == 0) {
+              f32x16 z;
+#pragma unroll
+              for (int r = 0; r < 16; ++r) z[r] = 0.f;
+              acc[j][i] = __builtin_amdgcn_mfma_f32_32x32x16_bf16(wf[j][0], f[i], z, 0, 0, 0);
+            } else {
+              acc[j][i] = __builtin_amdgcn_mfma_f32_32x32x16_bf16(wf[j][s], f[i], acc[j][i], 0, 0, 0);
+            }
+          }
+      }
+    }
+    if (resw) wait_vmcnt<0>();
+    fenced_barrier();
+    if (next_valid && (loader || resw)) {
+      const PairTile nx = load_desc(tn);
+      if (loader) issue_a(nx);
+      else issue_res(nx, b ^ 1);
+    }
+    const int ln1 = opaque_lane(), l31 = ln1 & 31, lh = ln1 >> 5;
+#pragma unroll
+    for (int j = 0; j < 2; ++j) {
+#pragma unroll
+      for (int i = 0; i < 2; ++i) {
+        const unsigned rg = ybuf + wave * 8192 + (i * 32 + l31) * 128 + lh * 8;
+        u32x2 rv[4];
+#pragma unroll
+        for (int g = 0; g < 4; ++g) asm volatile("ds_read_b64 %0, %1" : "=v"(rv[g]) : "v"(rg + (((4 * j + g) ^ (l31 & 7)) << 4)));
+#pragma unroll
+        for (int g = 0; g < 4; ++g) {
+          f32x4 sc4, sh4;
+          const int chw = wave * 64 + j * 32 + 8 * g + 4 * lh;
+          asm volatile("ds_read_b128 %0, %1" : "=v"(sc4) : "v"(tab + chw * 4));
+          asm volatile("ds_read_b128 %0, %1" : "=v"(sh4) : "v"(tab + (512 + chw) * 4));
+          if (g == 0) asm volatile("s_waitcnt lgkmcnt(0)" : "+v"(sc4), "+v"(sh4), "+v"(rv[0]), "+v"(rv[1]), "+v"(rv[2]), "+v"(rv[3]));
+          else asm volatile("s_waitcnt lgkmcnt(0)" : "+v"(sc4), "+v"(sh4));
+          float v[4];
+#pragma unroll
+          for (int e = 0; e < 4; ++e) v[e] = __builtin_fmaf(acc[j][i][4 * g + e], sc4[e], sh4[e]);
+          const u32x2 rr = rv[g];
+          v[0] += __uint_as_float(rr[0] << 16); v[1] += __uint_as_float(rr[0] & 0xffff0000u);
+          v[2] += __uint_as_float(rr[1] << 16); v[3] += __uint_as_float(rr[1] & 0xffff0000u);
+#pragma unroll
+          for (int e = 0; e < 4; ++e) v[e] = v[e] > 0.f ? v[e] : 0.f;
+          bf16x2 p0, p1;
+          p0[0] = (bf16_t)v[0]; p0[1] = (bf16_t)v[1]; p1[0] = (bf16_t)v[2]; p1[1] = (bf16_t)v[3];
+          const u32x2 pk = {__builtin_bit_cast(unsigned, p0), __builtin_bit_cast(unsigned, p1)};
+          asm volatile("ds_write_b64 %0, %1" ::"v"(rg + (((4 * j + g) ^ (l31 & 7)) << 4)), "v"(pk) : "memory");
+        }
+      }
+    }
+    asm volatile("s_waitcnt lgkmcnt(0)" ::: "memory");
+    fenced_barrier();
+    if (storer) store_y(cur, b);
+
+    f32x4 c2[4];
+#pragma unroll
+    for (int rg = 0; rg < 4; ++rg) c2[rg] = f32x4{0.f, 0.f, 0.f, 0.f};
+    {
+      const int ln3 = opaque_lane(), l15 = ln3 & 15, kb = ln3 >> 4;
+      unsigned boff[2];
+#pragma unroll
+      for (int p = 0; p < 2; ++p) boff[p] = (unsigned)(l15 * 128 + (((4 * p + kb) ^ (l15 & 7)) << 4));
+      bf16x8 fb[2][4];
+      auto rd = [&](int ks, bf16x8(&f)[4]) {
+        const unsigned ad = ybuf + (ks >> 1) * 8192 + boff[ks & 1];
+#pragma unroll
+        for (int rg = 0; rg < 4; ++rg) asm volatile("ds_read_b128 %0, %1" : "=v"(f[rg]) : "v"(ad + rg * 2048));
+      };
+      rd(0, fb[0]);
+#pragma unroll
+      for (int ks = 0; ks < 16; ++ks) {
+        bf16x8(&f)[4] = fb[ks & 1];
+        if (ks < 15) {
+          rd(ks + 1, fb[(ks + 1) & 1]);
+          asm volatile("s_waitcnt lgkmcnt(4)" : "+v"(f[0]), "+v"(f[1]), "+v"(f[2]), "+v"(f[3]));
+        } else {
+          asm volatile("s_waitcnt lgkmcnt(0)" : "+v"(f[0]), "+v"(f[1]), "+v"(f[2]), "+v"(f[3]));
+        }
+#pragma unroll
+        for (int rg = 0; rg < 4; ++rg) c2[rg] = __builtin_amdgcn_mfma_f32_16x16x32_bf16(wg[ks], f[rg], c2[rg], 0, 0, 0);
+      }
+    }
+    asm volatile("s_waitcnt lgkmcnt(0)" ::: "memory");
+    fenced_barrier();
+    const int ln2 = opaque_lane(), l15 = ln2 & 15, kb = ln2 >> 4;
+    f32x4 sc1, sh1;
+    asm volatile("ds_read_b128 %0, %1" : "=v"(sc1) : "v"(tab + (1024 + wave * 16 + 4 * kb) * 4));
+    asm volatile("ds_read_b128 %0, %1" : "=v"(sh1) : "v"(tab + (1152 + wave * 16 + 4 * kb) * 4));
+    asm volatile("s_waitcnt lgkmcnt(0)" : "+v"(sc1), "+v"(sh1));
+#pragma unroll
+    for (int rg = 0; rg < 4; ++rg) {
+      float v[4];
+#pragma unroll
+      for (int e = 0; e < 4; ++e) {
+        v[e] = __builtin_fmaf(c2[rg][e], sc1[e], sh1[e]);
+        v[e] = v[e] > 0.f ? v[e] : 0.f;
+      }
+      bf16x2 p0, p1;
+      p0[0] = (bf16_t)v[0]; p0[1] = (bf16_t)v[1]; p1[0] = (bf16_t)v[2]; p1[1] = (bf16_t)v[3];
+      const u32x2 pk = {__builtin_bit_cast(unsigned, p0), __builtin_bit_cast(unsigned, p1)};
+      const unsigned dst = ybuf + (rg * 16 + l15) * 256 + (((2 * wave + (kb >> 1)) ^ l15) << 4) + (kb & 1) * 8;
+      asm volatile("ds_write_b64 %0, %1" ::"v"(dst), "v"(pk) : "memory");
+    }
+    if (loader) wait_vmcnt<0>();
+    asm volatile("s_waitcnt lgkmcnt(0)" ::: "memory");
+    fenced_barrier();
+    prev = cur;
+    have_prev = true;
+    if (!next_valid) break;
+    t = tn;
+    cur = load_desc(t);
+    b ^= 1;
+  }
+  if (storer) store_t1(prev, b);
+}
+
+int launch_conv_spw_pair(const PairArgs& a, hipStream_t s) {
+  if (a.n_tiles <= 0) return -1;
+  static PerDeviceOnce once;
+  if (!once.run(current_device(), [] {
+        return hipFuncSetAttribute((const void*)conv_spw_kernel_pair, hipFuncAttributeMaxDynamicSharedMemorySize, PAIR_LDS) == hipSuccess;
+      }))
+    return -7;
+  const int n_cu = device_cu_count(current_device());
+  const int grid = a.n_tiles < n_cu ? a.n_tiles : n_cu;
+  hipLaunchKernelGGL(conv_spw_kernel_pair, dim3(grid), dim3(512), PAIR_LDS, s, a);
+  return (int)hipGetLastError();
+}
+
+}
diff --git a/sylph-few-shot-detection_amd/csrc/res3_pair_tiles.h b/sylph-few-shot-detection_amd/csrc/res3_pair_tiles.h
--- /dev/null
+++ b/sylph-few-shot-detection_amd/csrc/res3_pair_tiles.h
@@ -0,0 +1,29 @@
+#pragma once
+#include <vector>
+
+#ifdef __HIPCC__
+#define SYLPH_PAIR_HD __host__ __device__
+#else
+#define SYLPH_PAIR_HD
+#endif
+
+namespace sylph {
+
+constexpr int PAIR_TILE_ROWS = 64;
+
+struct PairTile { int img_row0, row0, seg_rows, pad; };
+
+SYLPH_PAIR_HD inline int pair_tile_load_row(const PairTile& t, int r) {
+  const int p = t.row0 + r;
+  return p < t.seg_rows ? p : t.seg_rows - 1;
+}
+SYLPH_PAIR_HD inline bool pair_tile_stores(const PairTile& t, int r) { return t.row0 + r < t.seg_rows; }
+
+inline std::vector<PairTile> pair_tiles(int B, int HW) {
+  std::vector<PairTile> v;
+  for (int b = 0; b < B; ++b)
+    for (int r0 = 0; r0 < HW; r0 += PAIR_TILE_ROWS) v.push_back(PairTile{b * HW, r0, HW, 0});
+  return v;
+}
+
+}
diff --git a/sylph-few-shot-detection_amd/sylph_amd/_lib.py b/sylph-few-shot-detection_amd/sylph_amd/_lib.py
--- a/sylph-few-shot-detection_amd/sylph_amd/_lib.py
+++ b/sylph-few-shot-detection_amd/sylph_amd/_lib.py
@@ -79,6 +79,7 @@
                                  POINTER(c_void_p), POINTER(c_void_p), c_void_p]),
     "sylph_bottleneck_even": (c_int, [c_void_p, c_void_p, c_int, c_int, c_int, c_int, c_int, c_int, POINTER(c_void_p),
                                       POINTER(c_void_p), POINTER(c_void_p), c_void_p]),
+    "sylph_res3_pair": (c_int, [c_void_p, c_void_p, c_void_p, c_int, c_int, c_int] + [c_void_p] * 8),
     "sylph_allgather_codes": (c_int, [c_void_p, c_void_p, c_void_p, c_int, c_int, c_void_p]),
     "sylph_comm_unique_id": (c_int, [ctypes.c_char_p]),
     "sylph_comm_init_rank": (c_int, [c_void_p, ctypes.c_char_p, c_int, c_int, POINTER(c_void_p)]),
diff --git a/sylph-few-shot-detection_amd/sylph_amd/engine.py b/sylph-few-shot-detection_amd/sylph_amd/engine.py
--- a/sylph-few-shot-detection_amd/sylph_amd/engine.py
+++ b/sylph-few-shot-detection_amd/sylph_amd/engine.py
@@ -786,6 +786,17 @@
               "bottleneck_even")
         return y
 
+    def res3_pair(self, t2, x, w3, s3, b3, w1, s1, b1):
+        self._stream()
+        t2 = t2.to(self.device, torch.float32).contiguous()
+        x = x.to(self.device, torch.float32).contiguous()
+        B, _, H, W = x.shape
+        host = [t.detach().cpu().float().contiguous() for t in (w3, s3, b3, w1, s1, b1)]
+        y = torch.empty(B, 512, H, W, device=self.device)
+        t1 = torch.empty(B, 128, H, W, device=self.device)
+        check(self.L.sylph_res3_pair(self._ctx, _ptr(t2), _ptr(x), B, H, W, *[_ptr(t) for t in host], _ptr(y), _ptr(t1)), "res3_pair")
+        return y, t1
+
     def bottleneck_grouped(self, x, ws, scales, shifts, stride=1, groups=32):
         self._stream()
         x = x.to(self.device, torch.float32).contiguous()
```

Result: faster. 2303 (median of 6 runs) (+1.4%).
